# Lab-LVM/imagenet-models

Measured on AMD Instinct MI355X. Metric: images/sec (whole node) GA-ConvNeXt-T 3x224x224 bf16 training step, higher is better.
Workload: dtype bf16; 1 GPU; ga_convnext_tiny_768 train step (fwd + GA loss lam=-0.8 + bwd + all-reduce + adamw lr=0), batch 256/GPU, drop_path 0.2, synthetic 3x224x224; global_batch=256, parallelism=dp1, dist_backend=none, grad_exchange=torch, allreduce_buckets=0

## Files before the change

### imagenet-models_amd/_lib.py

```python
import ctypes as C
import os

_HERE = os.path.dirname(os.path.abspath(__file__))
LIB_PATH = os.environ.get('GAEXT_LIB') or os.path.join(_HERE, 'csrc', 'libgaext.so')

GA_F32, GA_BF16 = 0, 1
ACT_NONE, ACT_GELU, ACT_RELU = 0, 1, 2
A_PLAIN, A_PATCH2, A_STEM4_NCHW, A_CONV3, A_CONV3S2, A_NEIGH2 = 0, 1, 2, 3, 4, 5
C_PLAIN, C_UNPATCH2 = 0, 1

vp, i32, i64, f32 = C.c_void_p, C.c_int, C.c_int64, C.c_float


class GemmDesc(C.Structure):
    _fields_ = [
        ('M', i32), ('N', i32), ('K', i32), ('batch', i32), ('dtype', i32),
        ('A', vp), ('lda', i64), ('strideA', i64), ('a_batch_mod', i32), ('a_kind', i32),
        ('a_H', i32), ('a_W', i32), ('a_C', i32), ('a_act', i32),
        ('B', vp), ('ldb', i64), ('strideB', i64),
        ('C', vp), ('ldc', i64), ('strideC', i64), ('c_kind', i32),
        ('c_H', i32), ('c_W', i32), ('c_C', i32), ('c_f32', i32), ('C2', vp), ('c2_mode', i32),
        ('alpha', f32), ('bias', vp), ('strideBias', i64), ('act', i32),
        ('H', vp), ('ldh', i64), ('strideH', i64), ('h_is_deriv', i32),
        ('rowscale', vp), ('rows_per_scale', i32),
        ('R', vp), ('ldr', i64), ('strideR', i64), ('relu_after', i32),
        ('colsum', vp), ('colsumsq', vp), ('strideCol', i64),
    ]


class WgradDesc(C.Structure):
    _fields_ = [
        ('M', i32), ('N', i32), ('K', i32), ('batch', i32), ('dtype', i32),
        ('Y', vp), ('ldy', i64), ('strideY', i64),
        ('X', vp), ('ldx', i64), ('strideX', i64), ('x_batch_mod', i32), ('x_kind', i32),
        ('x_H', i32), ('x_W', i32), ('x_C', i32), ('x_act', i32),
        ('dW', vp), ('ldw', i64), ('strideW', i64),
        ('dbias', vp), ('strideDbias', i64),
        ('alpha', f32), ('split_m', i32), ('accumulate', i32), ('workspace', vp), ('ws_bytes', i64),
    ]


class WprepDesc(C.Structure):
    _fields_ = [
        ('w', vp), ('G', i32), ('Co', i32), ('Ci', i32), ('KH', i32), ('KW', i32),
        ('rs', vp), ('cs', vp), ('row_perm', vp), ('dtype', i32),
        ('out', vp), ('ldo', i64), ('outT', vp), ('ldt', i64), ('flip', i32), ('stem', i32), ('t_cols', i32),
    ]


class WunfoldDesc(C.Structure):
    _fields_ = [
        ('G', vp), ('ldg', i64), ('gb', vp), ('W', vp), ('b', vp), ('rs', vp), ('cs', vp), ('v', vp), ('row_perm', vp),
        ('N', i32), ('Ci', i32), ('KH', i32), ('KW', i32), ('stem', i32),
        ('dW', vp), ('db', vp), ('d_rs', vp), ('d_cs', vp), ('d_v', vp),
    ]


class SmallDesc(C.Structure):
    _fields_ = [('kind', i32), ('y', vp), ('x', vp), ('a', f32), ('n', i64), ('R', i32), ('C', i32), ('accumulate', i32),
                ('b', vp), ('rs', vp), ('v', vp), ('row_perm', vp)]


class CswinAttnDesc(C.Structure):
    _fields_ = [('B', i32), ('reso', i32), ('C', i32), ('heads', i32), ('nbranch', i32),
                ('Hs', i32 * 2), ('Ws', i32 * 2), ('lepe_w', vp * 2), ('lepe_b', vp * 2),
                ('scale', f32), ('dtype', i32), ('qkv', vp), ('ldq', i64), ('out', vp), ('ldo', i64)]


class MlpDesc(C.Structure):
    _fields_ = [('X', vp), ('ldx', i64), ('W1', vp), ('ldw1', i64), ('b1', vp), ('W2', vp), ('ldw2', i64), ('b2', vp),
                ('R', vp), ('ldr', i64), ('rowscale', vp), ('rows_per_scale', i32), ('Y', vp), ('ldy', i64),
                ('M', i64), ('C', i32), ('H', i32), ('dtype', i32)]


class MlpBwdDesc(C.Structure):
    _fields_ = [('X', vp), ('ldx', i64), ('DY', vp), ('lddy', i64), ('W1', vp), ('ldw1', i64), ('b1', vp),
                ('W2T', vp), ('ldw2t', i64), ('W1T', vp), ('ldw1t', i64), ('A', vp), ('lda', i64), ('DH', vp), ('lddh', i64),
                ('DX', vp), ('lddx', i64), ('M', i64), ('C', i32), ('H', i32), ('dtype', i32),
                ('dW1', vp), ('ldw', i64), ('db1', vp), ('partials', vp), ('partials_bytes', C.c_size_t), ('max_blocks', i32)]


class SmallLinearDesc(C.Structure):
    _fields_ = [('rows', i32), ('groups', i32), ('Ng', i32), ('Kg', i32), ('A', vp), ('lda', i64), ('a_gstride', i64), ('a_perm', vp),
                ('W', vp), ('bias', vp), ('col_scale', vp), ('rowscale', vp), ('rows_per_scale', i32), ('R', vp), ('ldr', i64),
                ('Y', vp), ('ldy', i64), ('Yraw', vp), ('dtype', i32)]


class AttnDesc(C.Structure):
    _fields_ = [('B', i32), ('N', i32), ('H', i32), ('hd', i32), ('scale', f32), ('dtype', i32), ('qkv', vp), ('ldq', i64),
                ('out', vp), ('ldo', i64), ('lse', vp)]


_SIGS = {
    'ga_version': ([], i32),
    'ga_last_error': ([C.c_char_p, C.c_size_t], i32),
    'ga_device_info': ([C.POINTER(i32), C.POINTER(i32), C.POINTER(i32)], i32),
    'ga_comm_unique_id': ([vp], i32),
    'ga_comm_init': ([C.POINTER(vp), i32, i32, vp], i32),
    'ga_comm_destroy': ([vp], i32),
    'ga_comm_info': ([vp, C.POINTER(i32), C.POINTER(i32)], i32),
    'ga_allreduce_workspace': ([i64, i32], C.c_size_t),
    'ga_allreduce_bucket': ([vp, vp, i64, i32, f32, vp, C.c_size_t, vp], i32),
    'ga_reduce_scatter_bucket': ([vp, vp, vp, i64, f32, vp], i32),
    'ga_allgather_bucket': ([vp, vp, vp, i64, vp], i32),
    'ga_comm_broadcast': ([vp, vp, i64, i32, vp], i32),
    'ga_set_knob': ([C.c_char_p, i32], i32),
    'ga_unset_knob': ([C.c_char_p], i32),
    'ga_config_string': ([C.c_char_p, C.c_size_t], i32),
    'ga_gemm': ([C.POINTER(GemmDesc), vp], i32),
    'ga_wgrad': ([C.POINTER(WgradDesc), vp], i32),
    'ga_weight_prep': ([C.POINTER(WprepDesc), vp], i32),
    'ga_bias_fold': ([vp, vp, vp, vp, vp, vp, i32, i32, vp], i32),
    'ga_weight_unfold': ([C.POINTER(WunfoldDesc), vp], i32),
    'ga_dwconv7_fwd': ([vp, vp, vp, vp, i32, i32, i32, i32, i32, vp], i32),
    'ga_dwconv7_bwd_data': ([vp, vp, vp, vp, i32, i32, i32, i32, i32, vp], i32),
    'ga_dwconv7_bwd_data2': ([vp, vp, vp, vp, vp, vp, i32, i32, i32, i32, i32, vp], i32),
    'ga_dwconv7_bwd_weight': ([vp, vp, vp, vp, i32, i32, i32, i32, i32, vp, C.c_size_t, vp], i32),
    'ga_dwconv7_bwd_weight_workspace': ([i32, i32, i32, i32, i32], C.c_size_t),
    'ga_dwconv3_fwd': ([vp, vp, vp, i32, i32, i32, i32, i32, vp, vp, i32, vp], i32),
    'ga_dwconv3_bwd_data': ([vp, vp, vp, i32, i32, i32, i32, i32, i32, vp], i32),
    'ga_dwconv3_bwd_weight': ([vp, vp, vp, i32, i32, i32, i32, i32, i32, vp, C.c_size_t, vp], i32),
    'ga_dwconv3_bwd_weight_workspace': ([i32, i32, i32, i32, i32, i32], C.c_size_t),
    'ga_maxpool3s2_fwd': ([vp, vp, vp, i32, i32, i32, i32, i32, vp], i32),
    'ga_maxpool3s2_bwd': ([vp, vp, vp, i32, i32, i32, i32, i32, i32, vp], i32),
    'ga_bn_gelu_fwd': ([vp, vp, vp, vp, i64, i32, i32, vp], i32),
    'ga_bn_gelu_bwd_workspace': ([i64, i32], C.c_size_t),
    'ga_bn_gelu_bwd_reduce': ([vp, vp, vp, vp, vp, vp, vp, vp, i64, i32, i32, vp, C.c_size_t, vp], i32),
    'ga_bn_gelu_bwd_apply': ([vp, vp, vp, vp, vp, vp, vp, vp, vp, i64, vp, i64, i32, i32, vp], i32),
    'ga_se_bn_fwd': ([vp, i32, vp, vp, vp, vp, vp, vp, vp, vp, vp, vp, vp, vp, vp, vp, i32, i32, i32, i32, vp], i32),
    'ga_se_bn_bwd': ([vp, vp, vp, vp, vp, vp, vp, vp, i32, vp, vp, vp, vp, vp, vp, vp, vp, vp, vp, vp, vp, vp, vp, vp, vp, vp, vp, vp,
                      vp, vp, i32, i32, i32, vp], i32),
    'ga_se_residual_fwd': ([vp, vp, vp, vp, vp, vp, vp, vp, vp, i32, i32, i32, i32, vp], i32),
    'ga_se_residual_bwd_a': ([vp, vp, vp, vp, vp, vp, vp, vp, i32, i32, i32, i32, vp], i32),
    'ga_se_residual_bwd_b': ([vp, vp, vp, vp, vp, vp, vp, vp, vp, vp, vp, i32, i32, i32, i32, vp], i32),
    'ga_subsample2_fwd': ([vp, vp, i32, i32, i32, i32, i32, vp], i32),
    'ga_subsample2_bwd': ([vp, vp, i32, i32, i32, i32, i32, i32, vp], i32),
    'ga_wgrad_workspace': ([C.POINTER(WgradDesc)], C.c_size_t),
    'ga_gemm_form': ([C.POINTER(GemmDesc), C.c_char_p, C.c_size_t], i32),
    'ga_wgrad_form': ([C.POINTER(WgradDesc), C.c_char_p, C.c_size_t], i32),
    'ga_layernorm_fwd': ([vp, vp, vp, vp, vp, vp, i64, i32, f32, i32, vp], i32),
    'ga_layernorm_bwd': ([vp, vp, vp, vp, vp, vp, vp, vp, vp, i64, i32, i32, i32, vp], i32),
    'ga_layernorm_bwd_dp': ([vp, vp, vp, vp, vp, vp, vp, vp, vp, i64, i32, i32, vp, vp, i64, i32, vp], i32),
    'ga_bn_finalize': ([vp, vp, i64, vp, vp, f32, f32, vp, vp, vp, vp, vp, vp, i32, i32, vp], i32),
    'ga_affine_act': ([vp, vp, vp, vp, vp, i64, vp, i64, i32, i32, i32, i64, vp], i32),
    'ga_bn_bwd_reduce': ([vp, vp, vp, vp, vp, vp, i64, vp, vp, i64, i32, i32, i64, vp], i32),
    'ga_bn_bwd_apply': ([vp, vp, vp, vp, vp, vp, vp, vp, vp, i64, i64, vp, i64, i32, i32, i64, i64, vp], i32),
    'ga_pool_concat_fwd': ([vp, vp, i32, i32, i32, i32, i32, i32, i32, i32, i32, i32, vp], i32),
    'ga_pool_concat_bwd': ([vp, vp, vp, i32, i32, i32, i32, i32, i32, i32, i32, i32, i32, vp], i32),
    'ga_spatial_sum': ([vp, vp, vp, i32, i32, i32, f32, i32, vp], i32),
    'ga_se_mlp_fwd': ([vp, vp, vp, vp, vp, vp, vp, i32, i32, i32, vp], i32),
    'ga_se_mlp_bwd': ([vp, vp, vp, vp, vp, vp, vp, f32, vp, vp, vp, vp, i32, i32, i32, vp], i32),
    'ga_chan_scale': ([vp, vp, vp, vp, i32, i32, i32, i32, vp], i32),
    'ga_gram_pack_fwd': ([vp, vp, vp, i32, i32, i32, i32, i32, vp], i32),
    'ga_gram_pack_bwd': ([vp, vp, vp, vp, i32, i32, i32, i32, i32, vp], i32),
    'ga_gram_f64_fwd_workspace': ([i32, i32], C.c_size_t),
    'ga_gram_f64_bwd_workspace': ([i32, i32], C.c_size_t),
    'ga_gram_f64_fwd': ([vp, vp, vp, vp, C.c_size_t, i32, i32, i32, i32, i32, i32, i32, vp], i32),
    'ga_gram_f64_bwd': ([vp, vp, vp, vp, vp, vp, C.c_size_t, i32, i32, i32, i32, i32, i32, i32, vp], i32),
    'ga_token_cat': ([vp, vp, vp, i32, i32, i32, i32, vp], i32),
    'ga_token_split': ([vp, vp, vp, i32, i32, i32, i32, i32, i32, vp], i32),
    'ga_class_attn_fwd': ([vp, vp, vp, vp, i32, i32, i32, i32, f32, i32, vp], i32),
    'ga_class_attn_bwd': ([vp, vp, vp, vp, vp, vp, i32, i32, i32, i32, f32, i32, vp], i32),
    'ga_class_attn_fwd2': ([vp, vp, vp, i64, vp, vp, i32, i32, i32, i32, f32, i32, vp], i32),
    'ga_class_attn_bwd2': ([vp, vp, vp, vp, i64, vp, vp, vp, vp, i32, i32, i32, i32, f32, i32, vp], i32),
    'ga_loss_fwd_bwd': ([vp, vp, vp, vp, i32, i32, i32, f32, i32, f32, f32, i32, vp], i32),
    'ga_heads_topk': ([vp, i32, i32, i32, i32, vp, vp, vp], i32),
    'ga_sgd_step': ([vp, vp, vp, vp, i64, i32, f32, vp], i32),
    'ga_adamw_step': ([vp, vp, vp, vp, vp, i64, f32, vp], i32),
    'ga_weight_prep_batch': ([vp, i32, vp], i32),
    'ga_weight_unfold_batch': ([vp, i32, vp], i32),
    'ga_small_batch': ([vp, i32, vp], i32),
    'ga_cswin_attn_fwd': ([C.POINTER(CswinAttnDesc), vp], i32),
    'ga_cswin_attn_bwd_workspace': ([C.POINTER(CswinAttnDesc)], C.c_size_t),
    'ga_cswin_attn_bwd': ([C.POINTER(CswinAttnDesc), vp, vp, vp, C.c_size_t, vp], i32),
    'ga_cswin_lepe_wgrad_reduce': ([C.POINTER(CswinAttnDesc), vp, vp, vp, vp, vp, vp], i32),
    'ga_cswin_lepe_wgrad': ([C.POINTER(CswinAttnDesc), vp, vp, vp, vp, vp, vp], i32),
    'ga_layernorm_gelu_fwd': ([vp, vp, vp, vp, vp, vp, i64, i32, f32, i32, vp], i32),
    'ga_layernorm_gelu_bwd': ([vp, vp, vp, vp, vp, vp, vp, vp, vp, i64, i32, i32, vp], i32),
    'ga_nchw3_to_nhwc8': ([vp, vp, i32, i32, i32, i32, vp], i32),
    'ga_convw_pack': ([vp, vp, i32, i32, i32, i32, i64, i32, vp], i32),
    'ga_convw_unpack_grad': ([vp, vp, i32, i32, i32, i32, i64, vp], i32),
    'ga_conv3s2_dgrad_prep': ([vp, vp, i32, i32, i64, i32, vp], i32),
    'ga_gram_pack_fwd2': ([vp, vp, vp, i32, i32, i32, i32, i32, i32, vp], i32),
    'ga_gram_pack_bwd2': ([vp, vp, vp, vp, i32, i32, i32, i32, i32, i32, vp], i32),
    'ga_map_tokens_fwd': ([vp, vp, i32, i32, i32, i32, i32, vp], i32),
    'ga_map_tokens_bwd': ([vp, vp, i32, i32, i32, i32, i32, vp], i32),
    'ga_class_attn_mt_fwd': ([vp, vp, vp, i64, vp, vp, vp, i32, i32, i32, i32, i32, f32, i32, vp], i32),
    'ga_class_attn_mt_bwd': ([vp, vp, vp, vp, i64, vp, vp, vp, vp, vp, i64, i32, i32, i32, i32, i32, f32, i32, vp], i32),
    'ga_class_attn_mt_ia_fwd': ([vp, vp, vp, i64, vp, vp, vp, vp, vp, vp, vp, i32, i32, i32, i32, i32, f32, i32, vp], i32),
    'ga_class_attn_mt_ia_bwd': ([vp, vp, vp, vp, i64, vp, vp, vp, vp, vp, vp, vp, vp, i64, vp, vp, vp, vp, i32, i32, i32, i32, i32, f32, i32,
                                 vp], i32),
    'ga_map_loss_fwd_bwd': ([vp, vp, vp, vp, vp, vp, i32, i32, i32, f32, i32, f32, f32, i32, vp], i32),
    'ga_gelu_fwd': ([vp, vp, i64, i32, vp], i32),
    'ga_gelu_bwd': ([vp, vp, vp, i64, i32, vp], i32),
    'ga_relu_drop': ([vp, vp, vp, vp, i64, i32, vp], i32),
    'ga_mask_mul': ([vp, vp, vp, vp, i64, i32, vp], i32),
    'ga_copy2d': ([vp, i64, vp, i64, i64, i32, i32, i32, vp], i32),
    'ga_dropout_mask_sample': ([vp, i64, f32, C.c_uint64, vp, vp], i32),
    'ga_drop_path_sample': ([vp, vp, i32, i32, C.c_uint64, vp, vp], i32),
    'ga_loss_dense_fwd_bwd': ([vp, vp, vp, vp, vp, vp, vp, i32, i32, i32, f32, i32, f32, f32, f32, i32, vp], i32),
    'ga_u8_normalize': ([vp, vp, i32, i32, i32, i32, C.POINTER(f32), C.POINTER(f32), vp], i32),
    'ga_input_erase': ([vp, i32, vp, i32, i32, i32, i32, C.POINTER(f32), C.POINTER(f32), vp, i32, i32, C.c_uint64, C.c_uint64, vp], i32),
    'ga_input_collate': ([vp, i32, vp, i32, i32, i32, i32, C.POINTER(f32), C.POINTER(f32), vp, vp, i32, i32, C.c_uint64, C.c_uint64, vp],
                         i32),
    'ga_mixup_target_elem': ([vp, vp, i32, i32, vp, C.c_double, vp], i32),
    'ga_rand_augment': ([vp, vp, vp, C.c_size_t, i32, i32, i32, i32, vp, i32, vp, vp], i32),
    'ga_rand_augment_work_bytes': ([i32, i32, i32, i32, i32], C.c_size_t),
    'ga_rand_augment_check_table': ([vp, i32], i32),
    'ga_resize_crop': ([vp, C.c_uint64, vp, vp, vp, C.c_size_t, i32, i32, i32, vp], i32),
    'ga_resize_crop_work_bytes': ([vp, i32, i32, i32], C.c_size_t),
    'ga_resize_crop_check_table': ([vp, i32, i32, i32, C.c_uint64], i32),
    'ga_resample_coeffs': ([i32, i32, i32, vp, vp, i32, vp], i32),
    'ga_jpeg_probe': ([vp, C.c_size_t, vp], i32),
    'ga_jpeg_entropy_decode': ([vp, C.c_size_t, vp, C.c_size_t, vp], i32),
    'ga_jpeg_check_table': ([vp, i32, C.c_uint64, C.c_uint64, C.c_uint64, C.c_uint64], i32),
    'ga_jpeg_work_bytes': ([vp, i32], C.c_size_t),
    'ga_jpeg_reconstruct': ([vp, i32, vp, vp, vp, vp, vp], i32),
    'ga_mixup_batch': ([vp, vp, i32, i32, i32, i32, C.c_double, i32, i32, i32, i32, i32, vp], i32),
    'ga_mixup_target': ([vp, vp, i32, i32, C.c_double, C.c_double, vp], i32),
    'ga_agc_clip': ([vp, vp, vp, i32, f32, f32, vp], i32),
    'ga_small_linear_fwd': ([C.POINTER(SmallLinearDesc), vp], i32),
    'ga_small_linear_bwd': ([C.POINTER(SmallLinearDesc), vp, vp, i32, vp, vp, vp, vp], i32),
    'ga_colstats': ([vp, i64, i32, i32, vp, vp, i32, vp], i32),
    'ga_pad_copy_f32': ([vp, vp, i64, i64, i64, i64, i32, vp], i32),
    'ga_pad_copy': ([vp, vp, i64, i64, i64, i64, i32, i32, vp], i32),
    'ga_stem4_ln_fwd': ([vp, vp, i64, vp, vp, vp, vp, vp, vp, vp, i32, i32, i32, i32, f32, vp], i32),
    'ga_blockdiag_f32': ([vp, vp, i64, i32, i32, i32, i64, i32, i32, vp], i32),
    'ga_pad_groups_f32': ([vp, vp, i64, i64, i32, i32, i32, i32, i32, i32, vp], i32),
    'ga_attn_fwd': ([C.POINTER(AttnDesc), vp], i32),
    'ga_attn_bwd_workspace': ([C.POINTER(AttnDesc)], C.c_size_t),
    'ga_attn_bwd': ([C.POINTER(AttnDesc), vp, vp, vp, C.c_size_t, vp], i32),
    'ga_patchify': ([vp, vp, i32, i32, i32, i32, i32, i32, vp], i32),
    'ga_vit_embed_fwd': ([vp, vp, vp, vp, i32, i32, i32, i32, vp], i32),
    'ga_vit_embed_bwd': ([vp, vp, vp, vp, i32, i32, i32, i32, vp], i32),
    'ga_patchify_strided': ([vp, vp, i32, i32, i32, i32, i32, i32, i32, vp], i32),
    'ga_pos_add_fwd': ([vp, vp, vp, i32, i32, i32, i32, vp], i32),
    'ga_pos_add_bwd': ([vp, vp, i32, i32, i32, i32, vp], i32),
    'ga_dwpool_fwd': ([vp, vp, vp, vp, i32, i32, i32, i32, i32, i32, vp], i32),
    'ga_dwpool_bwd_data': ([vp, vp, vp, i32, i32, i32, i32, i32, i32, vp], i32),
    'ga_dwpool_bwd_weight': ([vp, vp, vp, vp, i32, i32, i32, i32, i32, i32, vp], i32),
    'ga_resize_concat_fwd': ([vp, vp, i32, i32, i32, i32, i32, i32, i64, i32, i32, vp], i32),
    'ga_resize_concat_bwd': ([vp, vp, i32, i32, i32, i32, i32, i32, i64, i32, i32, vp], i32),
    'ga_rows_bcast': ([vp, vp, i32, i32, i32, f32, i32, vp], i32),
    'ga_token_gap_fwd': ([vp, vp, i32, i32, i32, i32, vp], i32),
    'ga_token_gap_bwd': ([vp, vp, i32, i32, i32, i32, vp], i32),
    'ga_mlp_supported': ([i32, i32, i32], i32),
    'ga_mlp_fwd': ([C.POINTER(MlpDesc), vp], i32),
    'ga_mlp_bwd': ([C.POINTER(MlpBwdDesc), vp], i32),
    'ga_mlp_bwd_wgrad_supported': ([i32, i32, i32], i32),
    'ga_mlp_bwd_partials': ([C.POINTER(MlpBwdDesc)], C.c_size_t),
    'ga_memset': ([vp, i32, C.c_size_t, vp], i32),
    'ga_transpose_f32': ([vp, vp, i32, i32, i32, vp], i32),
    'ga_axpy_f32': ([vp, vp, f32, i64, vp], i32),
    'ga_lerp_f32': ([vp, vp, f32, i64, vp], i32),
    'ga_sumsq_f32': ([vp, i64, vp, vp], i32),
    'ga_lamb_stage1': ([vp, vp, vp, vp, vp, vp, vp, vp, i32, vp, vp], i32),
    'ga_lamb_stage2': ([vp, vp, vp, vp, i32, vp, vp], i32),
    'ga_clip_grad_f32': ([vp, i64, vp, f32, i32, vp], i32),
    'ga_rowscale': ([vp, vp, vp, i64, i64, i32, vp], i32),
    'ga_cast_from_f32': ([vp, vp, i64, i32, vp], i32),
    'ga_cast_to_f32': ([vp, vp, i64, i32, vp], i32),
}

_lib = None


def load():
    global _lib
    if _lib is not None:
        return _lib
    if not os.path.exists(LIB_PATH):
        raise RuntimeError(f'libgaext.so not found at {LIB_PATH}: build it with `make -C {os.path.dirname(LIB_PATH)}` '
                           f'(there is no CPU fallback for the product path)')
    lib = C.CDLL(LIB_PATH)
    for name, (argtypes, restype) in _SIGS.items():
        fn = getattr(lib, name)
        fn.argtypes = argtypes
        fn.restype = restype
    _lib = lib
    return lib


def last_error():
    buf = C.create_string_buffer(512)
    load().ga_last_error(buf, 512)
    return buf.value.decode(errors='replace')


def config_string():
    buf = C.create_string_buffer(1024)
    load().ga_config_string(buf, 1024)
    s = buf.value.decode(errors='replace')
    host = sorted(k for k in os.environ if k.startswith(('GAEXT_', 'GA_FUSED_MLP')) and k != 'GAEXT_LIB')
    known = {'GAEXT_ASYNC_WGRAD', 'GAEXT_FWD_SPLIT', 'GAEXT_PAR_BRANCH', 'GAEXT_FWD_SKEW', 'GAEXT_FUSE_DP', 'GAEXT_HEAD_STREAMS',
             'GA_FUSED_MLP', 'GAEXT_SMALL_SINGLE', 'GAEXT_SYNC_DEBUG', 'GAEXT_MLP_WG1'}
    for k in host:
        if k in known:
            s += f' host:{k}={os.environ[k]}'
    if os.environ.get('GAEXT_LIB'):
        s += f' lib={os.environ["GAEXT_LIB"]}'
    return s


class knobs:

    def __init__(self, **kv):
        self.kv = kv

    def __enter__(self):
        lib = load()
        for k, v in self.kv.items():
            check(lib.ga_set_knob(k.encode(), int(v)), f'ga_set_knob({k})')
        return self

    def __exit__(self, *exc):
        lib = load()
        for k in self.kv:
            lib.ga_unset_knob(k.encode())
        return False


def check(rc, what):
    if rc != 0:
        raise RuntimeError(f'libgaext {what} failed (code {rc}): {last_error()}')


def exported_symbols():
    return sorted(_SIGS)
```

### imagenet-models_amd/csrc/gemm.hip

```cpp
#include <stdlib.h>
#include <algorithm>
#include <type_traits>
#include "common.h"
#include "gemm_select.h"

namespace {

constexpr int kThreads = 256;
constexpr int kRowBytes = 128;

__device__ __forceinline__ int xcd_remap(int bid, int nwg) {
    const int q = nwg >> 3, r = nwg & 7, xcd = bid & 7, idx = bid >> 3;
    return (xcd < r ? xcd * (q + 1) : r * (q + 1) + (xcd - r) * q) + idx;
}

struct RowCtx {
    long base;
    int y, x;
    bool valid;
};

__device__ __forceinline__ RowCtx make_row(int kind, long m, long M, long ld, int H, int W, int C) {
    RowCtx r;
    r.valid = m < M;
    r.y = r.x = 0;
    r.base = 0;
    if (!r.valid) return r;
    if (kind == GA_A_PLAIN) {
        r.base = m * ld;
    } else if (kind == GA_A_PATCH2) {
        const int OW = W >> 1, OH = H >> 1;
        const int ox = (int)(m % OW);
        const long t = m / OW;
        const int oy = (int)(t % OH);
        const long b = t / OH;
        r.base = ((b * H + 2 * oy) * W + 2 * ox) * (long)C;
    } else if (kind == GA_A_CONV3 || kind == GA_A_NEIGH2) {
        const int x = (int)(m % W);
        const long t = m / W;
        const int y = (int)(t % H);
        const long b = t / H;
        r.base = b * H * W;
        r.y = y;
        r.x = x;
    } else if (kind == GA_A_CONV3S2) {
        const int OW = (W + 1) >> 1, OH = (H + 1) >> 1;
        const int ox = (int)(m % OW);
        const long t = m / OW;
        const int oy = (int)(t % OH);
        const long b = t / OH;
        r.base = b * H * W;
        r.y = 2 * oy;
        r.x = 2 * ox;
    } else {
        const int OW = W >> 2, OH = H >> 2;
        const int ox = (int)(m % OW);
        const long t = m / OW;
        const int oy = (int)(t % OH);
        const long b = t / OH;
        r.base = ((b * C) * H + 4 * oy) * (long)W + 4 * ox;
    }
    return r;
}

struct KCtx {
    long off;
    int dy, dx;
    bool valid;
};

__device__ __forceinline__ KCtx make_k(int kind, int k, int K, int H, int W, int C) {
    KCtx c;
    c.valid = k < K;
    c.off = 0;
    c.dy = c.dx = 0;
    if (!c.valid) return c;
    if (kind == GA_A_PLAIN) {
        c.off = k;
    } else if (kind == GA_A_PATCH2) {
        const int tap = k / C, ch = k - tap * C;
        c.off = ((long)(tap >> 1) * W + (tap & 1)) * C + ch;
    } else if (kind == GA_A_CONV3 || kind == GA_A_CONV3S2) {
        const int tap = k / C, ch = k - tap * C;
        c.dy = tap / 3 - 1;
        c.dx = tap % 3 - 1;
        c.off = ((long)c.dy * W + c.dx) * C + ch;
    } else if (kind == GA_A_NEIGH2) {
        const int tap = k / C, ch = k - tap * C;
        c.dy = tap >> 1;
        c.dx = tap & 1;
        c.off = ((long)c.dy * W + c.dx) * C + ch;
    } else {
        const int ch = k >> 4, ky = (k >> 2) & 3;
        c.off = ((long)ch * H + ky) * W;
    }
    return c;
}

template <typename T>
__device__ __forceinline__ uint4 load_chunk(int kind, const void* base, const RowCtx& r, const KCtx& k, int H, int W,
                                            int C) {
    uint4 z = make_uint4(0, 0, 0, 0);
    if (!(r.valid && k.valid)) return z;
    if (kind == GA_A_CONV3 || kind == GA_A_CONV3S2 || kind == GA_A_NEIGH2) {
        const int yy = r.y + k.dy, xx = r.x + k.dx;
        if ((unsigned)yy >= (unsigned)H || (unsigned)xx >= (unsigned)W) return z;
        const long pix = r.base + (long)r.y * W + r.x;
        return *reinterpret_cast<const uint4*>(reinterpret_cast<const T*>(base) + pix * C + k.off);
    }
    if (kind == GA_A_STEM4_NCHW) {
        const float* p = reinterpret_cast<const float*>(base) + r.base + k.off;
        const float4 a = *reinterpret_cast<const float4*>(p);
        if constexpr (sizeof(T) == 4) {
            return make_uint4(__float_as_uint(a.x), __float_as_uint(a.y), __float_as_uint(a.z), __float_as_uint(a.w));
        } else {
            const float4 b = *reinterpret_cast<const float4*>(p + W);
            return make_uint4(pack2bf(a.x, a.y), pack2bf(a.z, a.w), pack2bf(b.x, b.y), pack2bf(b.z, b.w));
        }
    }
    return *reinterpret_cast<const uint4*>(reinterpret_cast<const T*>(base) + r.base + k.off);
}

template <typename T> __device__ __forceinline__ uint4 act_chunk(uint4 v, int act) {
    if (act == GA_ACT_NONE) return v;
    if constexpr (sizeof(T) == 4) {
        float f[4] = {__uint_as_float(v.x), __uint_as_float(v.y), __uint_as_float(v.z), __uint_as_float(v.w)};
#pragma unroll
        for (int i = 0; i < 4; ++i) f[i] = act == GA_ACT_GELU ? gelu_f(f[i]) : fmaxf(f[i], 0.f);
        return make_uint4(__float_as_uint(f[0]), __float_as_uint(f[1]), __float_as_uint(f[2]), __float_as_uint(f[3]));
    } else {
        unsigned w[4] = {v.x, v.y, v.z, v.w};
#pragma unroll
        for (int i = 0; i < 4; ++i) {
            float lo = __uint_as_float(w[i] << 16), hi = __uint_as_float(w[i] & 0xffff0000u);
            lo = act == GA_ACT_GELU ? gelu_f(lo) : fmaxf(lo, 0.f);
            hi = act == GA_ACT_GELU ? gelu_f(hi) : fmaxf(hi, 0.f);
            w[i] = pack2bf(lo, hi);
        }
        return make_uint4(w[0], w[1], w[2], w[3]);
    }
}

__device__ __forceinline__ void glds16(const void* gsrc, unsigned lds_dst) {
    unsigned keep;
    asm volatile(
        "s_mov_b32 %0, m0\n\ts_mov_b32 m0, %2\n\ts_nop 0\n\tglobal_load_lds_dwordx4 %1, off\n\ts_mov_b32 m0, %0"
        : "=&s"(keep)
        : "v"(gsrc), "s"(lds_dst)
        : "memory");
}

__device__ __forceinline__ void glds16x2(const void* g0, const void* g1, unsigned lds_dst) {
    unsigned keep;
    const char* g1m = static_cast<const char*>(g1) - 1024;
    asm volatile(
        "s_mov_b32 %0, m0\n\ts_mov_b32 m0, %3\n\ts_nop 0\n\tglobal_load_lds_dwordx4 %1, off\n\t"
        "global_load_lds_dwordx4 %2, off offset:1024\n\ts_mov_b32 m0, %0"
        : "=&s"(keep)
        : "v"(g0), "v"(g1m), "s"(lds_dst)
        : "memory");
}

typedef __attribute__((ext_vector_type(4))) unsigned u32x4_s;
__device__ __forceinline__ void blds16x2(u32x4_s rsrc, unsigned voff0, unsigned voff1, unsigned soff, unsigned lds_dst) {
    unsigned keep;
    const unsigned v1m = voff1 - 1024;
    asm volatile(
        "s_mov_b32 %0, m0\n\ts_mov_b32 m0, %4\n\ts_nop 0\n\tbuffer_load_dwordx4 %1, %3, %5 offen lds\n\t"
        "buffer_load_dwordx4 %2, %3, %5 offen offset:1024 lds\n\ts_mov_b32 m0, %0"
        : "=&s"(keep)
        : "v"(voff0), "v"(v1m), "s"(rsrc), "s"(lds_dst), "s"(soff)
        : "memory");
}
__device__ __forceinline__ void blds16(u32x4_s rsrc, unsigned voff, unsigned soff, unsigned lds_dst) {
    unsigned keep;
    asm volatile("s_mov_b32 %0, m0\n\ts_mov_b32 m0, %3\n\ts_nop 0\n\tbuffer_load_dwordx4 %1, %2, %4 offen lds\n\ts_mov_b32 m0, %0"
                 : "=&s"(keep)
                 : "v"(voff), "s"(rsrc), "s"(lds_dst), "s"(soff)
                 : "memory");
}
__device__ __forceinline__ u32x4_s make_rsrc(const void* base, unsigned bytes) {
    const unsigned long long a = reinterpret_cast<unsigned long long>(base);
    u32x4_s r;
    r[0] = __builtin_amdgcn_readfirstlane((unsigned)a);
    r[1] = __builtin_amdgcn_readfirstlane((unsigned)(a >> 32) & 0xffffu);
    r[2] = bytes;
    r[3] = 0x00020000u;
    return r;
}

__device__ __attribute__((aligned(256))) unsigned char g_zero_page[256];

template <int TNW, int NWM> struct NTCfg {
    static constexpr int NTHR = 128 * NWM;
    static constexpr int BM = 64 * NWM;
    static constexpr int BN = 32 * TNW;
    static constexpr int A_BYTES = BM * kRowBytes;
    static constexpr int RSTEP = NTHR / 8;
    static constexpr int NB = BN * 8 / NTHR > 0 ? BN * 8 / NTHR : 1;
    static constexpr int LDCS = BN + 4;
    static constexpr int SMEM_AB = A_BYTES + BN * kRowBytes;
    static constexpr int SMEM_C = 64 * LDCS * 4;
    static constexpr int SMEM = SMEM_AB > SMEM_C ? SMEM_AB : SMEM_C;
    static constexpr int P8 = BN / 8;
    static constexpr int RG = NTHR / P8;
    static constexpr bool DMA3 = TNW == 4 && NWM == 4;
    static constexpr bool SWZ = TNW == 4 || TNW == 8;
    static constexpr int NS = DMA3 ? 3 : 2;
    static constexpr int PR = TNW == 8 ? 16 : (SWZ ? 32 : 64);
    static constexpr int CSUM_BYTES = 2 * RG * BN * 4;
    static constexpr int STAGE_DMA = SWZ ? PR * BN * 4 : (SMEM_C > CSUM_BYTES ? SMEM_C : CSUM_BYTES);
    static constexpr int RING0 = (STAGE_DMA + 1023) & ~1023;
    static constexpr int SMEM_DMA = RING0 + NS * SMEM_AB;
    static constexpr int NW = 2 * NWM;
    static constexpr int NBP = (4 * TNW + NW - 1) / NW;
};

using gasel::EPI_GENERIC, gasel::EPI_PLAIN, gasel::EPI_FC1, gasel::EPI_FC2, gasel::EPI_DG2;

template <typename T, int TNW, int NWM, bool PLAIN, bool PRE, int EPI, bool DMA = false>
__global__ __launch_bounds__(128 * NWM, (NWM == 2 && !DMA && !PRE && EPI >= 0 && sizeof(T) == 2 && TNW == 3) ? 3 : (NWM == 2 && DMA) ? 2 : 1) void gemm_nt_kernel(const ga_gemm_desc d) {
#define F_GELU (EPI < 0 ? d.act == GA_ACT_GELU : EPI == EPI_FC1)
#define F_RELU (EPI < 0 ? d.act == GA_ACT_RELU : false)
#define F_C2 (EPI < 0 ? d.C2 != nullptr : (EPI == EPI_FC1 && d.C2 != nullptr))
#define F_H (EPI < 0 ? Hb != nullptr : EPI == EPI_DG2)
#define F_HDERIV (EPI < 0 ? d.h_is_deriv != 0 : true)
#define F_RS (EPI < 0 ? d.rowscale != nullptr : (EPI == EPI_FC2 && d.rowscale != nullptr))
#define F_R (EPI < 0 ? Rb != nullptr : EPI == EPI_FC2)
#define F_RELUA (EPI < 0 ? d.relu_after != 0 : false)
#define F_CSUM (EPI < 0 ? d.colsum != nullptr : ((EPI == EPI_DG2 || EPI == EPI_PLAIN) && d.colsum != nullptr))
#define F_UNPATCH (EPI < 0 ? d.c_kind == GA_C_UNPATCH2 : false)
#define F_CF32 (EPI < 0 ? d.c_f32 != 0 : false)
#define F_AACT (EPI < 0 ? d.a_act : GA_ACT_NONE)
    using CF = NTCfg<TNW, NWM>;
    constexpr int EPC = elt<T>::EPC;
    constexpr int BK = kRowBytes / (int)sizeof(T);
    constexpr int BN = CF::BN;
    static_assert(!DMA || (PLAIN && sizeof(T) == 2), "the LDS-DMA form needs plain bf16 operands");
    static_assert(DMA || (CF::BN * 8) % CF::NTHR == 0, "B slab must split evenly over the threads");
    extern __shared__ __attribute__((aligned(16))) unsigned char smem[];
    constexpr int RING0 = DMA ? CF::RING0 : 0;
    unsigned char* As = smem + RING0;
    unsigned char* Bs = As + CF::A_BYTES;

    const int tid = threadIdx.x, lane = tid & 63;
    const int wave = DMA ? __builtin_amdgcn_readfirstlane(tid >> 6) : tid >> 6;
    const int wm = wave >> 1, wn = wave & 1;
    const int tiles_n = (d.N + BN - 1) / BN, tiles_m = (d.M + CF::BM - 1) / CF::BM;
    const int nwg = tiles_n * tiles_m;
    const int z = blockIdx.z;
    const int za = d.a_batch_mod > 0 ? z % d.a_batch_mod : z;

    const unsigned char* Ab = reinterpret_cast<const unsigned char*>(d.A) +
                              (d.a_kind == GA_A_STEM4_NCHW ? 4 : (long)sizeof(T)) * za * d.strideA;
    const T* Bb = reinterpret_cast<const T*>(d.B) + z * d.strideB;

    const int kc = tid & 7, r0 = tid >> 3;
    const int nk = (d.K + BK - 1) / BK;
    RowCtx arow[PLAIN ? 1 : 4];
    int m0 = 0, n0 = 0;
    auto set_tile = [&](int vt) {
        const int bid = xcd_remap(vt, nwg);
        const int tile_m = bid / tiles_n, tile_n = bid - tile_m * tiles_n;
        m0 = tile_m * CF::BM;
        n0 = tile_n * BN;
        if constexpr (!PLAIN) {
#pragma unroll
            for (int i = 0; i < 4; ++i)
                arow[i] = make_row(d.a_kind, (long)m0 + r0 + CF::RSTEP * i, d.M, d.lda, d.a_H, d.a_W, d.a_C);
        }
    };

    uint4 ra[4], rb[CF::NB];
    auto g_load = [&](int kt) {
        const int k = kt * BK + kc * EPC;
        const bool kv = k < d.K;
        if constexpr (PLAIN) {
            const T* Ap = reinterpret_cast<const T*>(Ab) + k;
#pragma unroll
            for (int i = 0; i < 4; ++i) {
                const long m = (long)m0 + r0 + CF::RSTEP * i;
                ra[i] = (kv && m < d.M) ? *reinterpret_cast<const uint4*>(Ap + m * d.lda) : make_uint4(0, 0, 0, 0);
            }
        } else {
            const KCtx kx = make_k(d.a_kind, k, d.K, d.a_H, d.a_W, d.a_C);
#pragma unroll
            for (int i = 0; i < 4; ++i) ra[i] = load_chunk<T>(d.a_kind, Ab, arow[i], kx, d.a_H, d.a_W, d.a_C);
        }
#pragma unroll
        for (int i = 0; i < CF::NB; ++i) {
            const long n = (long)n0 + r0 + CF::RSTEP * i;
            rb[i] = (kv && n < d.N) ? *reinterpret_cast<const uint4*>(Bb + n * d.ldb + k) : make_uint4(0, 0, 0, 0);
        }
    };
    auto s_store = [&]() {
#pragma unroll
        for (int i = 0; i < 4; ++i) {
            const int row = r0 + CF::RSTEP * i;
            *reinterpret_cast<uint4*>(As + row * kRowBytes + ((kc ^ (row & 7)) << 4)) = act_chunk<T>(ra[i], F_AACT);
        }
#pragma unroll
        for (int i = 0; i < CF::NB; ++i) {
            const int row = r0 + CF::RSTEP * i;
            *reinterpret_cast<uint4*>(Bs + row * kRowBytes + ((kc ^ (row & 7)) << 4)) = rb[i];
        }
    };

    unsigned aoff[DMA ? 4 : 1], boff[DMA ? CF::NBP : 1];
    constexpr unsigned kOob = 0x80000000u;
    const int dchunk = ((lane & 7) ^ (lane >> 3)) * 8;
    const unsigned lds_ring = (unsigned)(size_t)(__attribute__((address_space(3))) unsigned char*)smem + RING0;
    const u32x4_s rsA = make_rsrc(Ab, kOob), rsB = make_rsrc(Bb, kOob);
    const int ktail = d.K % BK;
    auto dma_rows = [&](int tm0, int tn0) {
        if constexpr (DMA) {
#pragma unroll
            for (int i = 0; i < 4; ++i) {
                const long m = (long)tm0 + (wave * 4 + i) * 8 + (lane >> 3);
                aoff[i] = m < d.M ? (unsigned)(m * d.lda + dchunk) * 2u : kOob;
            }
#pragma unroll
            for (int i = 0; i < CF::NBP; ++i) {
                const long n = (long)tn0 + (i * CF::NW + wave) * 8 + (lane >> 3);
                boff[i] = n < d.N ? (unsigned)(n * d.ldb + dchunk) * 2u : kOob;
            }
        }
    };
    auto dma_issue = [&](int kt, int slot) {
        if constexpr (DMA) {
            const bool kdead = ktail && kt == nk - 1 && dchunk >= ktail;
            const unsigned soff = (unsigned)kt * (unsigned)kRowBytes;
            const unsigned dst = lds_ring + slot * CF::SMEM_AB;
#pragma unroll
            for (int i = 0; i < 4; ++i) blds16(rsA, kdead ? kOob : aoff[i], soff, dst + (wave * 4 + i) * 1024);
#pragma unroll
            for (int i = 0; i < CF::NBP; ++i) {
                const int p = i * CF::NW + wave;
                if (p < 4 * TNW) blds16(rsB, kdead ? kOob : boff[i], soff, dst + CF::A_BYTES + p * 1024);
            }
        }
    };

    const T* Hb = d.H ? reinterpret_cast<const T*>(d.H) + z * d.strideH : nullptr;
    const T* Rb = d.R ? reinterpret_cast<const T*>(d.R) + z * d.strideR : nullptr;
    float* Cs = reinterpret_cast<float*>(smem);
    const int c8 = tid % CF::P8, rg = tid / CF::P8;
    const bool t_active = rg < CF::RG;

    constexpr int NR = (64 + CF::RG - 1) / CF::RG;
    constexpr bool kPre = PRE && sizeof(T) == 2;
    uint4 pre[kPre ? NWM : 1][kPre ? NR : 1];
    const T* Pb = F_H ? Hb : Rb;
    const long ldp = F_H ? d.ldh : d.ldr;

    auto pre_sel = [&](int hf, int it) -> const uint4& { return pre[kPre ? hf : 0][kPre ? it : 0]; };

    int vt = blockIdx.x;
    set_tile(vt);
    int cslot = 0, ivt = blockIdx.x, ikt = 0, islot = 0, inflight = 0;
    auto issue_next = [&]() {
        if constexpr (DMA) {
            if (ivt >= nwg) return;
            if (ikt == 0) {
                const int bid = xcd_remap(ivt, nwg);
                const int tile_m = bid / tiles_n;
                dma_rows(tile_m * CF::BM, (bid - tile_m * tiles_n) * BN);
            }
            dma_issue(ikt, islot);
            islot = islot + 1 == CF::NS ? 0 : islot + 1;
            if (++ikt == nk) {
                ikt = 0;
                ivt += gridDim.x;
            }
            ++inflight;
        }
    };
    if constexpr (DMA) {
#pragma unroll
        for (int j = 0; j < CF::NS - 1; ++j) issue_next();
    } else {
        g_load(0);
    }
    for (; vt < nwg; ) {
    const int cm0 = m0, cn0 = n0;
    const int n = cn0 + c8 * 8;
    const bool n_ok = t_active && n < d.N;
    const bool full = n + 8 <= d.N;
    const bool use_pre = kPre && Pb != nullptr && n_ok && full;
    f32x4_t acc[TNW][4];
#pragma unroll
    for (int i = 0; i < TNW; ++i)
#pragma unroll
        for (int j = 0; j < 4; ++j) acc[i][j] = f32x4_t{0.f, 0.f, 0.f, 0.f};

    if constexpr (!DMA) {
        s_store();
        __syncthreads();
    }

    for (int kt = 0; kt < nk; ++kt) {
        if constexpr (DMA) {
            if (CF::NS == 3 && inflight >= 2) asm volatile("s_waitcnt vmcnt(6)" ::: "memory");
            else asm volatile("s_waitcnt vmcnt(0)" ::: "memory");
            __builtin_amdgcn_s_barrier();
            issue_next();
            --inflight;
            As = smem + RING0 + cslot * CF::SMEM_AB;
            Bs = As + CF::A_BYTES;
            cslot = cslot + 1 == CF::NS ? 0 : cslot + 1;
        } else {
            if (kt + 1 < nk) g_load(kt + 1);
        }
        if constexpr (kPre) {
            if (kt == nk - 1 && use_pre) {
#pragma unroll
                for (int hf = 0; hf < NWM; ++hf)
#pragma unroll
                    for (int it = 0; it < NR; ++it) {
                        const int row = rg + it * CF::RG;
                        const long m = (long)cm0 + hf * 64 + row;
                        if (row < 64 && m < d.M) pre[hf][it] = load16_nt(Pb + m * ldp + n);
                    }
            }
        }
#pragma unroll
        for (int ks = 0; ks < 2; ++ks) {
            const int chunk = ks * 4 + (lane >> 4);
            uint4 af[4];
#pragma unroll
            for (int t = 0; t < 4; ++t) {
                const int ra_ = wm * 64 + t * 16 + (lane & 15);
                af[t] = *reinterpret_cast<const uint4*>(As + ra_ * kRowBytes + ((chunk ^ (ra_ & 7)) << 4));
            }
#pragma unroll
            for (int tn = 0; tn < TNW; ++tn) {
                const int rb_ = wn * (16 * TNW) + tn * 16 + (lane & 15);
                const uint4 bf = *reinterpret_cast<const uint4*>(Bs + rb_ * kRowBytes + ((chunk ^ (rb_ & 7)) << 4));
                if constexpr (sizeof(T) == 2) {
#pragma unroll
                    for (int tm = 0; tm < 4; ++tm)
                        acc[tn][tm] = __builtin_amdgcn_mfma_f32_16x16x32_bf16(
                            *reinterpret_cast<const bf16x8_t*>(&bf), *reinterpret_cast<const bf16x8_t*>(&af[tm]),
                            acc[tn][tm], 0, 0, 0);
                } else {
#pragma unroll
                    for (int j = 0; j < 4; ++j)
#pragma unroll
                        for (int tm = 0; tm < 4; ++tm)
                            acc[tn][tm] = __builtin_amdgcn_mfma_f32_16x16x4f32(
                                reinterpret_cast<const float*>(&bf)[j], reinterpret_cast<const float*>(&af[tm])[j],
                                acc[tn][tm], 0, 0, 0);
                }
            }
        }
        if constexpr (!DMA) {
            __syncthreads();
            if (kt + 1 < nk) {
                s_store();
                __syncthreads();
            }
        }
    }
    vt += gridDim.x;
    if (vt < nwg) {
        set_tile(vt);
        if constexpr (!DMA) g_load(0);
    }

    float bias[8], csum[8], csq[8];
    {
        const float* bsrc = d.bias ? d.bias + (long)z * d.strideBias : reinterpret_cast<const float*>(Bb);
#pragma unroll
        for (int j = 0; j < 8; ++j) {
            const bool live = d.bias && n_ok && n + j < d.N;
            const float bl = bsrc[live ? n + j : 0];
            bias[j] = live ? bl : 0.f;
            csum[j] = csq[j] = 0.f;
        }
    }
    long c_off = 0;
    if (F_UNPATCH && n_ok) {
        const int tap = n / d.c_C, ch = n - tap * d.c_C;
        c_off = ((long)(tap >> 1) * d.c_W + (tap & 1)) * d.c_C + ch;
    }
    constexpr bool SW = DMA && CF::SWZ;
    constexpr int PRr = SW ? CF::PR : 64, NSUB = 64 / PRr, TMP = PRr / 16, NRP = SW ? PRr / CF::RG : NR;
#pragma unroll
    for (int half = 0; half < NWM; ++half) {
#pragma unroll
    for (int sub = 0; sub < NSUB; ++sub) {
        if (half || sub) __syncthreads();
        if (wm == half) {
#pragma unroll
            for (int tn = 0; tn < TNW; ++tn)
#pragma unroll
                for (int tml = 0; tml < TMP; ++tml) {
                    const int row = tml * 16 + (lane & 15), col = wn * (16 * TNW) + tn * 16 + (lane >> 4) * 4;
                    float* dst = SW ? Cs + row * BN + ((((col >> 2) ^ (row & 15))) << 2) : Cs + row * CF::LDCS + col;
                    *reinterpret_cast<f32x4_t*>(dst) = acc[tn][sub * TMP + tml];
                }
        }
        __syncthreads();
        if (n_ok) {
#pragma unroll
            for (int itp = 0; itp < NRP; ++itp) {
                const int it = sub * NRP + itp;
                const int row = rg + itp * CF::RG;
                if (row >= PRr) break;
                const long m = (long)cm0 + half * 64 + sub * PRr + row;
                if (m >= d.M) break;
                float v[8];
                {
                    const float* pa = SW ? Cs + row * BN + (((2 * c8) ^ (row & 15)) << 2) : Cs + row * CF::LDCS + c8 * 8;
                    const float* pb = SW ? Cs + row * BN + (((2 * c8 + 1) ^ (row & 15)) << 2) : Cs + row * CF::LDCS + c8 * 8 + 4;
                    const f32x4_t a = *reinterpret_cast<const f32x4_t*>(pa);
                    const f32x4_t b = *reinterpret_cast<const f32x4_t*>(pb);
                    v[0] = a[0]; v[1] = a[1]; v[2] = a[2]; v[3] = a[3];
                    v[4] = b[0]; v[5] = b[1]; v[6] = b[2]; v[7] = b[3];
                }
#pragma unroll
                for (int j = 0; j < 8; ++j) v[j] = (EPI < 0 ? v[j] * d.alpha : v[j]) + bias[j];
                if (F_C2) {
                    float w[8];
                    if (EPI >= 0 || (d.c2_mode == 2 && d.act == GA_ACT_GELU)) {
#pragma unroll
                        for (int j = 0; j < 8; ++j) {
                            if constexpr (sizeof(T) == 2 && EPI == EPI_FC1) gelu_both_fast(v[j], v[j], w[j]);
                            else gelu_both_f(v[j], v[j], w[j]);
                        }
                    } else {
#pragma unroll
                        for (int j = 0; j < 8; ++j) w[j] = d.c2_mode == 2 ? gelu_grad_f(v[j]) : v[j];
                        if (d.act == GA_ACT_GELU) {
#pragma unroll
                            for (int j = 0; j < 8; ++j) v[j] = gelu_f(v[j]);
                        }
                    }
                    if (F_RELU) {
#pragma unroll
                        for (int j = 0; j < 8; ++j) v[j] = fmaxf(v[j], 0.f);
                    }
                    T* C2p = reinterpret_cast<T*>(d.C2) + z * d.strideC + m * d.ldc + n;
                    if (full) {
                        store8_nt(C2p, w);
                    } else {
#pragma unroll
                        for (int j = 0; j < 8; ++j)
                            if (n + j < d.N) elt<T>::st(C2p + j, w[j]);
                    }
                } else if (F_GELU) {
#pragma unroll
                    for (int j = 0; j < 8; ++j) {
                        if constexpr (sizeof(T) == 2 && EPI == EPI_FC1) {
                            float unused;
                            gelu_both_fast(v[j], v[j], unused);
                        } else {
                            v[j] = gelu_f(v[j]);
                        }
                    }
                } else if (F_RELU) {
#pragma unroll
                    for (int j = 0; j < 8; ++j) v[j] = fmaxf(v[j], 0.f);
                }
                if (F_H) {
                    float h[8];
                    if (use_pre) {
                        if constexpr (kPre) unpack8(pre_sel(half, it), h);
                    } else if (full) {
                        load8_nt(Hb + m * d.ldh + n, h);
                    } else {
#pragma unroll
                        for (int j = 0; j < 8; ++j) h[j] = n + j < d.N ? elt<T>::ld(Hb + m * d.ldh + n + j) : 0.f;
                    }
                    if (F_HDERIV) {
#pragma unroll
                        for (int j = 0; j < 8; ++j) v[j] *= h[j];
                    } else {
#pragma unroll
                        for (int j = 0; j < 8; ++j) v[j] *= gelu_grad_f(h[j]);
                    }
                }
                if (F_RS) {
                    const float s = d.rowscale[(unsigned)m / (unsigned)d.rows_per_scale];
#pragma unroll
                    for (int j = 0; j < 8; ++j) v[j] *= s;
                }
                if (F_R) {
                    float r[8];
                    if (use_pre && !F_H) {
                        if constexpr (kPre) unpack8(pre_sel(half, it), r);
                    } else if (full) {
                        load8_nt(Rb + m * d.ldr + n, r);
                    } else {
#pragma unroll
                        for (int j = 0; j < 8; ++j) r[j] = n + j < d.N ? elt<T>::ld(Rb + m * d.ldr + n + j) : 0.f;
                    }
#pragma unroll
                    for (int j = 0; j < 8; ++j) v[j] += r[j];
                }
                if (F_RELUA) {
#pragma unroll
                    for (int j = 0; j < 8; ++j) v[j] = fmaxf(v[j], 0.f);
                }
                if (F_CSUM) {
#pragma unroll
                    for (int j = 0; j < 8; ++j) {
                        csum[j] += v[j];
                        csq[j] += v[j] * v[j];
                    }
                }
                long off;
                if (F_UNPATCH) {
                    const unsigned OW = d.c_W >> 1, OH = d.c_H >> 1;
                    const unsigned ox = (unsigned)m % OW;
                    const unsigned t = (unsigned)m / OW;
                    const unsigned oy = t % OH;
                    const long b = t / OH;
                    off = ((b * d.c_H + 2 * oy) * d.c_W + 2 * ox) * (long)d.c_C + c_off;
                } else {
                    off = z * d.strideC + m * d.ldc + n;
                }
                if (F_CF32) {
                    float* Cp = reinterpret_cast<float*>(d.C) + off;
                    if (full) {
                        store8(Cp, v);
                    } else {
#pragma unroll
                        for (int j = 0; j < 8; ++j)
                            if (n + j < d.N) Cp[j] = v[j];
                    }
                } else {
                    T* Cp = reinterpret_cast<T*>(d.C) + off;
                    if (full) {
                        store8_nt(Cp, v);
                    } else {
#pragma unroll
                        for (int j = 0; j < 8; ++j)
                            if (n + j < d.N) elt<T>::st(Cp + j, v[j]);
                    }
                }
            }
        }
    }
    }
    if (F_CSUM) {
        float* red = reinterpret_cast<float*>(smem);
        constexpr int NPASS = SW ? 2 : 1;
#pragma unroll
        for (int pass = 0; pass < NPASS; ++pass) {
            if (SW && pass == 1 && !d.colsumsq) break;
            __syncthreads();
            if (t_active) {
#pragma unroll
                for (int j = 0; j < 8; ++j) {
                    if constexpr (SW) {
                        red[rg * BN + c8 * 8 + j] = pass == 0 ? csum[j] : csq[j];
                    } else {
                        red[rg * BN + c8 * 8 + j] = csum[j];
                        red[CF::RG * BN + rg * BN + c8 * 8 + j] = csq[j];
                    }
                }
            }
            __syncthreads();
            for (int i = tid; i < (SW ? BN : 2 * BN); i += CF::NTHR) {
                const int which = SW ? pass : i / BN, col = SW ? i : i - which * BN;
                if (cn0 + col < d.N && (which == 0 || d.colsumsq)) {
                    float s = 0.f;
                    for (int r = 0; r < CF::RG; ++r) s += red[(SW ? 0 : which * CF::RG * BN) + r * BN + col];
                    atomicAdd((which ? d.colsumsq : d.colsum) + z * d.strideCol + cn0 + col, s);
                }
            }
        }
    }
    __syncthreads();
    }
#undef F_GELU
#undef F_RELU
#undef F_C2
#undef F_H
#undef F_HDERIV
#undef F_RS
#undef F_R
#undef F_RELUA
#undef F_CSUM
#undef F_UNPATCH
#undef F_CF32
#undef F_AACT
}

constexpr int kPPThreads = 512, kPPHalf = 16384, kPPBuf = 4 * kPPHalf, kPPSmem = 2 * kPPBuf + 8 * 4096;

template <int EPI>
__global__ __launch_bounds__(kPPThreads) void gemm_nt_pp_kernel(const ga_gemm_desc d, const int dbg_arg) {
#ifdef GAEXT_DEBUG
    const int dbg = dbg_arg;
#else
    constexpr int dbg = 0;
    (void)dbg_arg;
#endif
    extern __shared__ __attribute__((aligned(16))) unsigned char smem[];
    const int tid = threadIdx.x, lane = tid & 63;
    const int wave = __builtin_amdgcn_readfirstlane(tid >> 6);
    const int wr = wave >> 2, wc = wave & 3;
    const int tiles_n = (d.N + 255) / 256, tiles_m = (d.M + 255) / 256;
    const int nwg = tiles_n * tiles_m;
    const int z = blockIdx.z;
    const int za = d.a_batch_mod > 0 ? z % d.a_batch_mod : z;
    const bf16_t* Ab = reinterpret_cast<const bf16_t*>(d.A) + (long)za * d.strideA;
    const bf16_t* Bb = reinterpret_cast<const bf16_t*>(d.B) + (long)z * d.strideB;
    const int nk = (d.K + 63) / 64;
    const int my_tiles = (nwg - (int)blockIdx.x + (int)gridDim.x - 1) / (int)gridDim.x;
    const int S = my_tiles * nk;

    const int fa = (lane & 15) * 128 + ((((lane >> 4) ^ (lane & 7))) << 4);
    const unsigned char* aF[2] = {smem + wr * kPPHalf + fa, smem + wr * kPPHalf + (fa ^ 64)};
    const unsigned char* bF[2] = {smem + (2 + (wc >> 1)) * kPPHalf + (wc & 1) * 8192 + fa,
                                  smem + (2 + (wc >> 1)) * kPPHalf + (wc & 1) * 8192 + (fa ^ 64)};

    const unsigned lds0 = (unsigned)(size_t)(__attribute__((address_space(3))) unsigned char*)smem;
    const int dchunk = ((lane & 7) ^ (lane >> 3)) * 8;
    struct Cursor { int vt, kt; };
    Cursor cm = {(int)blockIdx.x, 0}, cl = {(int)blockIdx.x, 0};
    int off_a0[2], off_b[2][2], off_a1[2];
    auto rows_of = [&](int t, int h, bool is_a, int (&o)[2]) {
        const int bid = xcd_remap(t, nwg);
        const int tm = bid / tiles_n, tn = bid - tm * tiles_n;
#pragma unroll
        for (int i = 0; i < 2; ++i) {
            const int r = h * 128 + 16 * wave + 8 * i + (lane >> 3);
            o[i] = is_a ? min(tm * 256 + r, d.M - 1) * (int)d.lda : min(tn * 256 + r, d.N - 1) * (int)d.ldb;
        }
    };
    auto set_main = [&]() {
        rows_of(cm.vt, 0, false, off_b[0]);
        rows_of(cm.vt, 1, false, off_b[1]);
    };
    auto set_lag = [&]() {
        rows_of(cl.vt, 0, true, off_a0);
        rows_of(cl.vt, 1, true, off_a1);
    };
    const u32x4_s rsA = make_rsrc(Ab, 0x80000000u), rsB = make_rsrc(Bb, 0x80000000u);
    const int ktail = d.K & 63;
    auto glds_half = [&](const bf16_t* base, const int (&o)[2], int kt_, int half, int buf) {
        if (dbg & 2) return;
        const unsigned dst = lds0 + buf * kPPBuf + half * kPPHalf + 2 * wave * 1024;
        if (dbg & 16) {
            const int k = kt_ * 64 + dchunk;
            const bool kv = k < d.K && !(dbg & 8);
            glds16x2(kv ? static_cast<const void*>(base + o[0] + k) : static_cast<const void*>(g_zero_page),
                     kv ? static_cast<const void*>(base + o[1] + k) : static_cast<const void*>(g_zero_page), dst);
            return;
        }
        unsigned v0 = (unsigned)(o[0] + dchunk) * 2u, v1 = (unsigned)(o[1] + dchunk) * 2u;
        if (ktail && kt_ == nk - 1 && dchunk >= ktail) v0 = v1 = 0x80000400u;
        blds16x2(base == Ab ? rsA : rsB, v0, v1, (unsigned)kt_ * 128u, dst);
    };
    auto issue_B0 = [&](int buf) { glds_half(Bb, off_b[0], cm.kt, 2, buf); };
    auto issue_B1 = [&](int buf) {
        glds_half(Bb, off_b[1], cm.kt, 3, buf);
        if (++cm.kt == nk) {
            cm.kt = 0;
            cm.vt += gridDim.x;
            if (cm.vt < nwg) set_main();
        }
    };
    auto issue_A0 = [&](int buf) { glds_half(Ab, off_a0, cl.kt, 0, buf); };
    auto issue_A1 = [&](int buf) {
        glds_half(Ab, off_a1, cl.kt, 1, buf);
        if (++cl.kt == nk) {
            cl.kt = 0;
            cl.vt += gridDim.x;
            if (cl.vt < nwg) set_lag();
        }
    };

    f32x4_t acc[4][8];
    bf16x8_t af[4][2], bc0[2][2], b1[2][2], bn0[2][2];
    const f32x4_t zero4 = {0.f, 0.f, 0.f, 0.f};
#pragma unroll
    for (int i = 0; i < 4; ++i)
#pragma unroll
        for (int j = 0; j < 8; ++j) acc[i][j] = zero4;

#define PP_READ_A(mh, bufp)                                                                                         \
    _Pragma("unroll") for (int tm = 0; tm < 4; ++tm) _Pragma("unroll") for (int ks = 0; ks < 2; ++ks)               \
        af[tm][ks] = *reinterpret_cast<const bf16x8_t*>(aF[ks] + (bufp) + ((mh) * 4 + tm) * 2048);
#define PP_READ_B(dst, nh, bufp)                                                                                    \
    _Pragma("unroll") for (int tn = 0; tn < 2; ++tn) _Pragma("unroll") for (int ks = 0; ks < 2; ++ks)               \
        dst[tn][ks] = *reinterpret_cast<const bf16x8_t*>(bF[ks] + (bufp) + ((nh) * 2 + tn) * 2048);
#define PP_MMA(bq, mh, nh)                                                                                          \
    __builtin_amdgcn_s_setprio(1);                                                                                  \
    _Pragma("unroll") for (int ks = 0; ks < 2; ++ks) _Pragma("unroll") for (int tn = 0; tn < 2; ++tn)               \
        _Pragma("unroll") for (int tm = 0; tm < 4; ++tm)                                                            \
            acc[(nh) * 2 + tn][(mh) * 4 + tm] = __builtin_amdgcn_mfma_f32_16x16x32_bf16(bq[tn][ks], af[tm][ks],     \
                                                                                      acc[(nh) * 2 + tn][(mh) * 4 + tm], 0, 0, 0); \
    __builtin_amdgcn_s_setprio(0);
#define PP_MMA_RELOAD(bq, mh, nh, mh2, bufp)                                                                        \
    __builtin_amdgcn_s_setprio(1);                                                                                  \
    _Pragma("unroll") for (int tm = 0; tm < 4; ++tm) {                                                              \
        _Pragma("unroll") for (int ks = 0; ks < 2; ++ks) _Pragma("unroll") for (int tn = 0; tn < 2; ++tn)           \
            acc[(nh) * 2 + tn][(mh) * 4 + tm] = __builtin_amdgcn_mfma_f32_16x16x32_bf16(bq[tn][ks], af[tm][ks],     \
                                                                                      acc[(nh) * 2 + tn][(mh) * 4 + tm], 0, 0, 0); \
        __builtin_amdgcn_sched_barrier(0);                                                                          \
        _Pragma("unroll") for (int ks = 0; ks < 2; ++ks)                                                            \
            af[tm][ks] = *reinterpret_cast<const bf16x8_t*>(aF[ks] + (bufp) + ((mh2) * 4 + tm) * 2048);             \
        __builtin_amdgcn_sched_barrier(0);                                                                          \
    }                                                                                                               \
    __builtin_amdgcn_s_setprio(0);
#define PP_LGKM0 asm volatile("s_waitcnt lgkmcnt(0)" ::: "memory")
#define PP_BAR                            \
    __builtin_amdgcn_sched_barrier(0);    \
    __builtin_amdgcn_s_barrier();         \
    __builtin_amdgcn_sched_barrier(0)

    set_main();
    set_lag();
    issue_B0(0);
    issue_B1(0);
    issue_A0(0);
    issue_A1(0);
    if (S > 1) {
        issue_B0(1);
        issue_B1(1);
        asm volatile("s_waitcnt vmcnt(4)" ::: "memory");
    } else {
        asm volatile("s_waitcnt vmcnt(0)" ::: "memory");
    }
    PP_BAR;
    PP_READ_B(bn0, 0, 0);
    PP_LGKM0;

    const bf16_t* Hb = d.H ? reinterpret_cast<const bf16_t*>(d.H) + (long)z * d.strideH : nullptr;
    const bf16_t* Rb = d.R ? reinterpret_cast<const bf16_t*>(d.R) + (long)z * d.strideR : nullptr;
    float* stage = reinterpret_cast<float*>(smem + 2 * kPPBuf + wave * 4096);
    int vt = blockIdx.x, kt = 0;
#pragma unroll 1
    for (int g = 0; g < S; ++g) {
        const int bufp = (g & 1) * kPPBuf, nbufp = kPPBuf - bufp;
        const bool more1 = g + 1 < S, more2 = g + 2 < S;
        if (kt == 0 && wr == 1) { PP_BAR; }
#pragma unroll
        for (int i = 0; i < 2; ++i)
#pragma unroll
            for (int j = 0; j < 2; ++j) bc0[i][j] = bn0[i][j];
        PP_READ_A(0, bufp);
        if (more1) issue_A0((g + 1) & 1);
        PP_LGKM0;
        PP_BAR;
        PP_READ_B(b1, 1, bufp);
        PP_MMA(bc0, 0, 0);
        PP_BAR;
        if (more1) {
            issue_A1((g + 1) & 1);
            if (!(dbg & 4)) asm volatile("s_waitcnt vmcnt(4)" ::: "memory");
        }
        PP_LGKM0;
        PP_BAR;
        PP_MMA_RELOAD(b1, 0, 1, 1, bufp);
        PP_BAR;
        if (more2) issue_B0(g & 1);
        PP_LGKM0;
        PP_BAR;
        if (more1) { PP_READ_B(bn0, 0, nbufp); }
        PP_MMA(b1, 1, 1);
        PP_BAR;
        if (more2) issue_B1(g & 1);
        if (more1 && !(dbg & 4)) {
            if (more2) asm volatile("s_waitcnt vmcnt(4)" ::: "memory");
            else asm volatile("s_waitcnt vmcnt(0)" ::: "memory");
        }
        PP_LGKM0;
        PP_BAR;
        PP_MMA(bc0, 1, 0);
        PP_BAR;
        if (++kt < nk) continue;
        kt = 0;
        if (wr == 0) { PP_BAR; }
        if (dbg & 1) {
            vt += gridDim.x;
            continue;
        }
        {
            const int bid = xcd_remap(vt, nwg);
            const int tile_m = bid / tiles_n, tile_n = bid - tile_m * tiles_n;
            const int q = lane & 7, rr = lane >> 3;
            const int n = tile_n * 256 + wc * 64 + q * 8;
            const bool n_ok = n < d.N;
            float bias[8], csum[8], csq[8];
            {
                const bool live = d.bias && n_ok;
                const float* bsrc = d.bias ? d.bias + (long)z * d.strideBias : reinterpret_cast<const float*>(Bb);
#pragma unroll
                for (int j = 0; j < 8; ++j) {
                    const float bl = bsrc[live ? n + j : 0];
                    bias[j] = live ? bl : 0.f;
                    csum[j] = csq[j] = 0.f;
                }
            }
            const bool do_csum = (EPI == EPI_PLAIN || EPI == EPI_DG2) && d.colsum != nullptr;
            constexpr bool kOp = EPI == EPI_DG2 || EPI == EPI_FC2;
            const bf16_t* Pb = EPI == EPI_DG2 ? Hb : Rb;
            const long ldp = EPI == EPI_DG2 ? d.ldh : d.ldr;
            const long mrow0 = (long)tile_m * 256 + wr * 128 + rr;
            uint4 opn[2] = {make_uint4(0, 0, 0, 0), make_uint4(0, 0, 0, 0)};
            auto fetch_op = [&](int tm) {
                if constexpr (kOp) {
#pragma unroll
                    for (int p = 0; p < 2; ++p) {
                        const long m = mrow0 + tm * 16 + 8 * p;
                        if (n_ok && m < d.M) opn[p] = load16_nt(Pb + m * ldp + n);
                    }
                }
            };
            fetch_op(0);
#pragma unroll
            for (int tm = 0; tm < 8; ++tm) {
                asm volatile("s_waitcnt lgkmcnt(0)" ::: "memory");
#pragma unroll
                for (int tn = 0; tn < 4; ++tn) {
                    const int row = lane & 15, u = tn * 4 + (lane >> 4);
                    *reinterpret_cast<f32x4_t*>(stage + row * 64 + ((u ^ row) << 2)) = acc[tn][tm];
                    acc[tn][tm] = zero4;
                }
                const uint4 opc[2] = {opn[0], opn[1]};
                if (tm + 1 < 8) fetch_op(tm + 1);
                asm volatile("s_waitcnt lgkmcnt(0)" ::: "memory");
#pragma unroll
                for (int p = 0; p < 2; ++p) {
                    const int row = 8 * p + rr;
                    const long m = (long)tile_m * 256 + wr * 128 + tm * 16 + row;
                    const f32x4_t lo = *reinterpret_cast<const f32x4_t*>(stage + row * 64 + (((2 * q) ^ row) << 2));
                    const f32x4_t hi = *reinterpret_cast<const f32x4_t*>(stage + row * 64 + (((2 * q + 1) ^ row) << 2));
                    if (!n_ok || m >= d.M) continue;
                    float v[8] = {lo[0] + bias[0], lo[1] + bias[1], lo[2] + bias[2], lo[3] + bias[3],
                                  hi[0] + bias[4], hi[1] + bias[5], hi[2] + bias[6], hi[3] + bias[7]};
                    if constexpr (EPI == EPI_FC1) {
                        float w[8];
#pragma unroll
                        for (int j = 0; j < 8; ++j) gelu_both_fast(v[j], v[j], w[j]);
                        if (d.C2) store8_nt(reinterpret_cast<bf16_t*>(d.C2) + (long)z * d.strideC + m * d.ldc + n, w);
                    }
                    if constexpr (EPI == EPI_DG2) {
                        float h[8];
                        unpack8(opc[p], h);
#pragma unroll
                        for (int j = 0; j < 8; ++j) v[j] *= h[j];
                    }
                    if constexpr (EPI == EPI_FC2) {
                        if (d.rowscale) {
                            const float sc = d.rowscale[(unsigned)m / (unsigned)d.rows_per_scale];
#pragma unroll
                            for (int j = 0; j < 8; ++j) v[j] *= sc;
                        }
                        float r[8];
                        unpack8(opc[p], r);
#pragma unroll
                        for (int j = 0; j < 8; ++j) v[j] += r[j];
                    }
                    if (do_csum) {
#pragma unroll
                        for (int j = 0; j < 8; ++j) {
                            csum[j] += v[j];
                            csq[j] += v[j] * v[j];
                        }
                    }
                    store8_nt(reinterpret_cast<bf16_t*>(d.C) + (long)z * d.strideC + m * d.ldc + n, v);
                }
            }
            if (do_csum) {
#pragma unroll
                for (int j = 0; j < 8; ++j) {
                    float a = csum[j], b = csq[j];
#pragma unroll
                    for (int o = 8; o < 64; o <<= 1) {
                        a += __shfl_xor(a, o, 64);
                        b += __shfl_xor(b, o, 64);
                    }
                    if (rr == 0 && n_ok) {
                        atomicAdd(d.colsum + (long)z * d.strideCol + n + j, a);
                        if (d.colsumsq) atomicAdd(d.colsumsq + (long)z * d.strideCol + n + j, b);
                    }
                }
            }
        }
        vt += gridDim.x;
    }
#undef PP_READ_A
#undef PP_READ_B
#undef PP_MMA
#undef PP_MMA_RELOAD
#undef PP_LGKM0
#undef PP_BAR
}

constexpr int kR3Threads = 256, kR3Slot = (256 + 128) * 64, kR3Stage = 2048, kR3Smem = 3 * kR3Slot + 4 * kR3Stage;
static_assert(kR3Smem == 81920, "two workgroups per CU need exactly 80 KiB each");

__device__ __forceinline__ u32x4_t r3_bload16(u32x4_s rs, unsigned voff) {
    u32x4_t v;
    asm volatile("buffer_load_dwordx4 %0, %1, %2, 0 offen nt" : "=v"(v) : "v"(voff), "s"(rs) : "memory");
    return v;
}
__device__ __forceinline__ u32x4_t r3_bload16_c(u32x4_s rs, unsigned voff) {
    u32x4_t v;
    asm volatile("buffer_load_dwordx4 %0, %1, %2, 0 offen" : "=v"(v) : "v"(voff), "s"(rs) : "memory");
    return v;
}

__device__ __forceinline__ float r3_bload4(u32x4_s rs, unsigned voff) {
    float v;
    asm volatile("buffer_load_dword %0, %1, %2, 0 offen" : "=v"(v) : "v"(voff), "s"(rs) : "memory");
    return v;
}
__device__ __forceinline__ void r3_bstore16(u32x4_s rs, unsigned voff, u32x4_t v) {
    asm volatile("buffer_store_dwordx4 %0, %1, %2, 0 offen nt\n\ts_nop 1" ::"v"(v), "v"(voff), "s"(rs) : "memory");
}
__device__ __forceinline__ u32x4_t r3_pack8(const float v[8]) {
    u32x4_t a;
    a[0] = pack2bf(v[0], v[1]); a[1] = pack2bf(v[2], v[3]); a[2] = pack2bf(v[4], v[5]); a[3] = pack2bf(v[6], v[7]);
    return a;
}

__device__ int g_r3_ticket[4096];

template <int EPI, int DBG = 0, int AK = 0>
__global__ __launch_bounds__(kR3Threads, 2) void gemm_nt_r3_kernel(const ga_gemm_desc d, const int stagger) {
    constexpr int dbg = DBG;
    extern __shared__ __attribute__((aligned(16))) unsigned char smem[];
    const int tid = threadIdx.x, lane = tid & 63;
    const int wave = __builtin_amdgcn_readfirstlane(tid >> 6);
    const int wm = wave >> 1, wn = wave & 1;
    const int tiles_n = (d.N + 127) / 128, tiles_m = (d.M + 255) / 256;
    const int nwg = tiles_n * tiles_m;
    const int z = blockIdx.z;
    const int za = d.a_batch_mod > 0 ? z % d.a_batch_mod : z;
    const bf16_t* Ab = reinterpret_cast<const bf16_t*>(d.A) + (long)za * d.strideA;
    const bf16_t* Bb = reinterpret_cast<const bf16_t*>(d.B) + (long)z * d.strideB;
    const int nk = (d.K + 31) / 32;
    const int my_tiles = (nwg - (int)blockIdx.x + (int)gridDim.x - 1) / (int)gridDim.x;
    const int S = my_tiles * nk;

    const int frow = lane & 15;
    const unsigned fa = frow * 64 + ((((lane >> 4) ^ ((4 - (frow >> 2)) & 3))) << 4);
    const unsigned char* aF = smem + wm * 8192 + fa;
    const unsigned char* bF = smem + 16384 + wn * 4096 + fa;

    const unsigned lds0 = (unsigned)(size_t)(__attribute__((address_space(3))) unsigned char*)smem;
    const int dchunk = ((lane & 3) ^ ((4 - (lane >> 4)) & 3)) * 8;
    constexpr unsigned kOob = 0x80000000u;
    auto extent = [](long rows, long ld, long cols, int esz) { return (unsigned)(((rows - 1) * ld + cols) * esz); };
    const bool patch2 = d.a_kind == GA_A_PATCH2;
    const bool neigh2 = AK == 1 && EPI == EPI_PLAIN && d.a_kind == GA_A_NEIGH2;
    const bool conv3s2 = AK == 1 && EPI == EPI_PLAIN && d.a_kind == GA_A_CONV3S2;
    const unsigned p2_row = (patch2 || neigh2) ? (unsigned)(d.a_W * d.a_C - 2 * d.a_C) * 2u : 0u;
    const unsigned c3_row = conv3s2 ? (unsigned)((d.a_W - 3) * d.a_C) * 2u : 0u;
    const unsigned c3_shift = conv3s2 ? (unsigned)((d.a_W + 1) * d.a_C) * 2u : 0u;
    const unsigned a_bytes = (patch2 || conv3s2) ? extent(4L * d.M, d.a_C, d.a_C, 2) : neigh2 ? extent(d.M, d.a_C, d.a_C, 2) : extent(d.M, d.lda, d.K, 2);
    const u32x4_s rsA = make_rsrc(reinterpret_cast<const unsigned char*>(Ab) - c3_shift, a_bytes + c3_shift),
                  rsB = make_rsrc(Bb, extent(d.N, d.ldb, d.K, 2));
    unsigned n2_have = 0;
    const int ktail = d.K & 31;
    unsigned aoff[4], boff[2];
    int ivt = blockIdx.x, ikt = 0;
    auto dma_rows = [&]() __attribute__((always_inline)) {
        if (ivt < nwg) {
            const int bid = xcd_remap(ivt, nwg);
            const int tm_ = bid / tiles_n, tn_ = bid - tm_ * tiles_n;
#pragma unroll
            for (int i = 0; i < 4; ++i) {
                const long m = (long)tm_ * 256 + (wave * 4 + i) * 16 + (lane >> 2);
                if (patch2) {
                    const unsigned OW = (unsigned)d.a_W >> 1, OH = (unsigned)d.a_H >> 1;
                    const unsigned ox = (unsigned)m % OW, t = (unsigned)m / OW, oy = t % OH, b = t / OH;
                    aoff[i] = m < d.M ? (unsigned)((((long)b * d.a_H + 2 * oy) * d.a_W + 2 * ox) * d.a_C + dchunk) * 2u : kOob;
                } else if (conv3s2) {
                    const unsigned OW = (unsigned)d.a_W >> 1, OH = (unsigned)d.a_H >> 1;
                    const unsigned ox = (unsigned)m % OW, t = (unsigned)m / OW, oy = t % OH, b = t / OH;
                    aoff[i] = m < d.M ? (unsigned)((((long)b * d.a_H + 2 * oy) * d.a_W + 2 * ox) * d.a_C + dchunk) * 2u : kOob;
                    const unsigned have = (ox > 0 ? 1u : 0u) | (oy > 0 ? 2u : 0u);
                    n2_have = (n2_have & ~(3u << (2 * i))) | (have << (2 * i));
                } else if (neigh2) {
                    const unsigned x = (unsigned)m % (unsigned)d.a_W, y = ((unsigned)m / (unsigned)d.a_W) % (unsigned)d.a_H;
                    aoff[i] = m < d.M ? (unsigned)(m * d.a_C + dchunk) * 2u : kOob;
                    const unsigned have = (x + 1 < (unsigned)d.a_W ? 1u : 0u) | (y + 1 < (unsigned)d.a_H ? 2u : 0u);
                    n2_have = (n2_have & ~(3u << (2 * i))) | (have << (2 * i));
                } else {
                    aoff[i] = m < d.M ? (unsigned)(m * d.lda + dchunk) * 2u : kOob;
                }
            }
#pragma unroll
            for (int i = 0; i < 2; ++i) {
                const long n = (long)tn_ * 128 + (wave * 2 + i) * 16 + (lane >> 2);
                boff[i] = n < d.N ? (unsigned)(n * d.ldb + dchunk) * 2u : kOob;
            }
        } else {
#pragma unroll
            for (int i = 0; i < 4; ++i) aoff[i] = kOob;
            boff[0] = boff[1] = kOob;
        }
    };
    auto dma_part = [&](int slot, int part) __attribute__((always_inline)) {
        const bool kdead = ktail && ikt == nk - 1 && dchunk >= ktail;
        const unsigned soff = (unsigned)ikt * 64u;
        unsigned soffA = soff + (2 * ikt >= nk ? p2_row : 0u);
        const unsigned dst = lds0 + slot * kR3Slot;
        unsigned a0 = aoff[part == 0 ? 0 : 2], a1 = aoff[part == 0 ? 1 : 3];
        if (conv3s2 && part < 2) {
            const int third = nk / 3, spt = nk / 9;
            const int ky = (ikt >= third ? 1 : 0) + (ikt >= 2 * third ? 1 : 0);
            const int r = ikt - ky * third;
            const unsigned need = (r < spt ? 1u : 0u) | (ky == 0 ? 2u : 0u);
            soffA = soff + (unsigned)ky * c3_row;
            if ((need & ~(n2_have >> (4 * part))) & 3u) a0 = kOob;
            if ((need & ~(n2_have >> (4 * part + 2))) & 3u) a1 = kOob;
        }
        if (neigh2 && part < 2) {
            const unsigned need = ((4 * ikt >= nk && 4 * ikt < 2 * nk) || 4 * ikt >= 3 * nk ? 1u : 0u) | (2 * ikt >= nk ? 2u : 0u);
            const unsigned miss = need & ~(n2_have >> (4 * part));
            if (miss & 3u) a0 = kOob;
            if ((need & ~(n2_have >> (4 * part + 2))) & 3u) a1 = kOob;
        }
        if (part == 0) blds16x2(rsA, kdead ? kOob : a0, kdead ? kOob : a1, soffA, dst + (wave * 4) * 1024);
        if (part == 1) blds16x2(rsA, kdead ? kOob : a0, kdead ? kOob : a1, soffA, dst + (wave * 4 + 2) * 1024);
        if (part == 2) {
            blds16x2(rsB, kdead ? kOob : boff[0], kdead ? kOob : boff[1], soff, dst + 16384 + (wave * 2) * 1024);
            if (++ikt == nk) {
                ikt = 0;
                ivt += gridDim.x;
                dma_rows();
            }
        }
    };
    auto dma_issue = [&](int slot) __attribute__((always_inline)) {
        dma_part(slot, 0);
        dma_part(slot, 1);
        dma_part(slot, 2);
    };

    f32x4_t acc[4][8];
    const f32x4_t zero4 = {0.f, 0.f, 0.f, 0.f};
#pragma unroll
    for (int i = 0; i < 4; ++i)
#pragma unroll
        for (int j = 0; j < 8; ++j) acc[i][j] = zero4;

    constexpr bool kOp = EPI == EPI_DG2 || EPI == EPI_FC2;
    const bf16_t* Pb = EPI == EPI_DG2 ? (d.H ? reinterpret_cast<const bf16_t*>(d.H) + (long)z * d.strideH : nullptr)
                                      : (d.R ? reinterpret_cast<const bf16_t*>(d.R) + (long)z * d.strideR : nullptr);
    const long ldp = EPI == EPI_DG2 ? d.ldh : d.ldr;
    const u32x4_s rsP = make_rsrc(Pb, (kOp && Pb && !(dbg & 8)) ? extent(d.M, ldp, d.N, 2) : 0u);
    const u32x4_s rsBias = make_rsrc(d.bias ? d.bias + (long)z * d.strideBias : nullptr, d.bias ? (unsigned)d.N * 4u : 0u);
    u32x4_t opn[kOp ? 4 : 1][2], biasv[2];
    float rsc[EPI == EPI_FC2 ? 4 : 1][2];
    const u32x4_s rsRS = make_rsrc(EPI == EPI_FC2 ? d.rowscale : nullptr,
                                   (EPI == EPI_FC2 && d.rowscale) ? (unsigned)(((d.M - 1) / d.rows_per_scale + 1) * 4) : 0u);
    auto rs_off = [&](long m) -> unsigned { return m < d.M ? ((unsigned)m / (unsigned)d.rows_per_scale) * 4u : kOob; };
    const int q = lane & 7, rr = lane >> 3;
    float* stage = reinterpret_cast<float*>(smem + 3 * kR3Slot + wave * kR3Stage);

    int vt = blockIdx.x, kt = 0, cslot = 0;
    int tile_m = 0, tile_n = 0;
    bool first = true;
    dma_rows();
    dma_issue(0);
    dma_issue(1);
    if (stagger > 0) {
        const unsigned hw = __builtin_amdgcn_s_getreg((31 << 11) | 4);
        const unsigned xcc = __builtin_amdgcn_s_getreg((31 << 11) | 20);
        const unsigned key = ((xcc & 15u) << 8) | ((hw >> 8) & 255u);
        int ticket = 0;
        if (tid == 0) ticket = atomicAdd(&g_r3_ticket[key], 1);
        ticket = __builtin_amdgcn_readfirstlane(ticket);
        if (wave == 0 && (ticket & 1)) {
            for (int i = 0; i < stagger; ++i) __builtin_amdgcn_s_sleep(1);
        }
    }
#pragma unroll 1
    for (int g = 0; g < S; ++g) {
        if (kt == 0) {
            const int bid = xcd_remap(vt, nwg);
            tile_m = bid / tiles_n;
            tile_n = bid - tile_m * tiles_n;
        }
        if ((first || kt >= 2) && !(dbg & 32)) asm volatile("s_waitcnt vmcnt(6)" ::: "memory");
        __builtin_amdgcn_s_barrier();
        const int n = tile_n * 128 + wn * 64 + q * 8;
        const bool n_ok = n < d.N;
        const long mrow0 = (long)tile_m * 256 + wm * 128 + rr;
        if (kt == nk - 1) {
            biasv[0] = r3_bload16_c(rsBias, n_ok ? (unsigned)n * 4u : kOob);
            biasv[1] = r3_bload16_c(rsBias, n_ok ? (unsigned)n * 4u + 16u : kOob);
            if constexpr (kOp) {
#pragma unroll
                for (int tm = 0; tm < 4; ++tm)
#pragma unroll
                    for (int p = 0; p < 2; ++p) {
                        const long m = mrow0 + tm * 16 + 8 * p;
                        opn[tm][p] = r3_bload16(rsP, (n_ok && m < d.M) ? (unsigned)(m * ldp + n) * 2u : kOob);
                        if constexpr (EPI == EPI_FC2) rsc[tm][p] = r3_bload4(rsRS, rs_off(m));
                    }
            }
        }
        const int islot = cslot >= 1 ? cslot - 1 : 2;
        {
            const unsigned sb = cslot * kR3Slot;
            bf16x8_t af[8], bfr[4];
#define R3_RA(i) af[i] = *reinterpret_cast<const bf16x8_t*>(aF + sb + (i) * 1024)
#define R3_MMA(i)                                                                                               \
    _Pragma("unroll") for (int tn = 0; tn < 4; ++tn)                                                             \
        acc[tn][i] = __builtin_amdgcn_mfma_f32_16x16x32_bf16(bfr[tn], af[i], acc[tn][i], 0, 0, 0)
#pragma unroll
            for (int tn = 0; tn < 4; ++tn) bfr[tn] = *reinterpret_cast<const bf16x8_t*>(bF + sb + tn * 1024);
            R3_RA(0); R3_RA(1); R3_RA(2); R3_RA(3);
            __builtin_amdgcn_sched_barrier(0);
            if (!(dbg & 16)) dma_part(islot, 0);
            R3_MMA(0); R3_MMA(1);
            __builtin_amdgcn_sched_barrier(0);
            R3_RA(4); R3_RA(5);
            if (!(dbg & 16)) dma_part(islot, 1);
            __builtin_amdgcn_sched_barrier(0);
            R3_MMA(2); R3_MMA(3);
            __builtin_amdgcn_sched_barrier(0);
            R3_RA(6); R3_RA(7);
            if (!(dbg & 16)) dma_part(islot, 2);
            __builtin_amdgcn_sched_barrier(0);
            R3_MMA(4); R3_MMA(5); R3_MMA(6); R3_MMA(7);
#undef R3_RA
#undef R3_MMA
        }
        cslot = cslot == 2 ? 0 : cslot + 1;
        if (++kt < nk) continue;
        kt = 0;
        first = false;
        if (dbg & 1) {
#pragma unroll
            for (int i = 0; i < 4; ++i)
#pragma unroll
                for (int j = 0; j < 8; ++j) asm volatile("" : "+v"(acc[i][j]));
            if constexpr (kOp)
                asm volatile("s_waitcnt vmcnt(0)"
                             : "+v"(opn[0][0]), "+v"(opn[0][1]), "+v"(opn[1][0]), "+v"(opn[1][1]), "+v"(opn[2][0]), "+v"(opn[2][1]),
                               "+v"(opn[3][0]), "+v"(opn[3][1]), "+v"(biasv[0]), "+v"(biasv[1]), "+v"(rsc[0][0]), "+v"(rsc[0][EPI == EPI_FC2]),
                               "+v"(rsc[EPI == EPI_FC2][0]), "+v"(rsc[EPI == EPI_FC2][EPI == EPI_FC2]), "+v"(rsc[2 * (EPI == EPI_FC2)][0]),
                               "+v"(rsc[2 * (EPI == EPI_FC2)][EPI == EPI_FC2]), "+v"(rsc[3 * (EPI == EPI_FC2)][0]), "+v"(rsc[3 * (EPI == EPI_FC2)][EPI == EPI_FC2])
                             :: "memory");
            else
                asm volatile("s_waitcnt vmcnt(0)" : "+v"(biasv[0]), "+v"(biasv[1])::"memory");
            vt += gridDim.x;
            continue;
        }
        if constexpr (kOp) {
            asm volatile("s_waitcnt vmcnt(0)"
                         : "+v"(opn[0][0]), "+v"(opn[0][1]), "+v"(opn[1][0]), "+v"(opn[1][1]), "+v"(opn[2][0]), "+v"(opn[2][1]),
                           "+v"(opn[3][0]), "+v"(opn[3][1]), "+v"(biasv[0]), "+v"(biasv[1])
                         :: "memory");
            if constexpr (EPI == EPI_FC2) {
#pragma unroll
                for (int tm = 0; tm < 4; ++tm) asm volatile("" : "+v"(rsc[tm][0]), "+v"(rsc[tm][1]));
            }
        } else {
            asm volatile("s_waitcnt vmcnt(0)" : "+v"(biasv[0]), "+v"(biasv[1]) :: "memory");
        }
        {
            float bias[8], csum[8], csq[8];
#pragma unroll
            for (int j = 0; j < 4; ++j) {
                bias[j] = __uint_as_float(biasv[0][j]);
                bias[4 + j] = __uint_as_float(biasv[1][j]);
            }
#pragma unroll
            for (int j = 0; j < 8; ++j) csum[j] = csq[j] = 0.f;
            const bool do_csum = (EPI == EPI_PLAIN || EPI == EPI_DG2) && d.colsum != nullptr;
            const bool unpatch2 = EPI == EPI_PLAIN && d.c_kind == GA_C_UNPATCH2;
            const u32x4_s rsC = make_rsrc(reinterpret_cast<bf16_t*>(d.C) + (long)z * d.strideC,
                                          unpatch2 ? extent(4L * d.M, d.c_C, d.c_C, 2) : extent(d.M, d.ldc, d.N, 2));
            unsigned up_col = 0;
            if (unpatch2 && n_ok) {
                const int tap = n / d.c_C, ch = n - tap * d.c_C;
                up_col = (unsigned)(((tap >> 1) * d.c_W + (tap & 1)) * d.c_C + ch);
            }
            const u32x4_s rsC2 = make_rsrc((EPI == EPI_FC1 && d.C2) ? reinterpret_cast<bf16_t*>(d.C2) + (long)z * d.strideC : nullptr,
                                           (EPI == EPI_FC1 && d.C2) ? extent(d.M, d.ldc, d.N, 2) : 0u);
#pragma unroll
            for (int tm = 0; tm < 8; ++tm) {
                if constexpr (kOp) {
                    if (tm >= 4) {
                        constexpr int L = EPI == EPI_FC2 ? 4 : 2;
                        constexpr int ST = (dbg & 2) ? 0 : 2;
                        constexpr int kYoung[4] = {3 * ST + 3 * L, 3 * ST + 2 * L, 3 * ST + L, 3 * ST};
                        constexpr int R = EPI == EPI_FC2 ? 1 : 0;
                        if (tm == 4) asm volatile("s_waitcnt vmcnt(%4)" : "+v"(opn[0][0]), "+v"(opn[0][1]), "+v"(rsc[0][0]), "+v"(rsc[0][R]) : "n"(kYoung[0]) : "memory");
                        if (tm == 5) asm volatile("s_waitcnt vmcnt(%4)" : "+v"(opn[1][0]), "+v"(opn[1][1]), "+v"(rsc[R][0]), "+v"(rsc[R][R]) : "n"(kYoung[1]) : "memory");
                        if (tm == 6) asm volatile("s_waitcnt vmcnt(%4)" : "+v"(opn[2][0]), "+v"(opn[2][1]), "+v"(rsc[2 * R][0]), "+v"(rsc[2 * R][R]) : "n"(kYoung[2]) : "memory");
                        if (tm == 7) asm volatile("s_waitcnt vmcnt(%4)" : "+v"(opn[3][0]), "+v"(opn[3][1]), "+v"(rsc[3 * R][0]), "+v"(rsc[3 * R][R]) : "n"(kYoung[3]) : "memory");
                    }
                }
#pragma unroll
                for (int p = 0; p < 2; ++p) {
                    if (((lane >> 3) & 1) == p) {
                        const int row = lane & 7;
#pragma unroll
                        for (int tn = 0; tn < 4; ++tn) {
                            const int u = tn * 4 + (lane >> 4);
                            *reinterpret_cast<f32x4_t*>(stage + row * 64 + ((u ^ row) << 2)) = acc[tn][tm];
                        }
                    }
                    const f32x4_t lo = *reinterpret_cast<const f32x4_t*>(stage + rr * 64 + (((2 * q) ^ rr) << 2));
                    const f32x4_t hi = *reinterpret_cast<const f32x4_t*>(stage + rr * 64 + (((2 * q + 1) ^ rr) << 2));
                    const long m = mrow0 + tm * 16 + 8 * p;
                    float v[8] = {lo[0] + bias[0], lo[1] + bias[1], lo[2] + bias[2], lo[3] + bias[3],
                                  hi[0] + bias[4], hi[1] + bias[5], hi[2] + bias[6], hi[3] + bias[7]};
                    const bool live = n_ok && m < d.M;
                    unsigned coff = live ? (unsigned)(m * d.ldc + n) * 2u : kOob;
                    if (unpatch2 && live) {
                        const unsigned OW = (unsigned)d.c_W >> 1, OH = (unsigned)d.c_H >> 1;
                        const unsigned ox = (unsigned)m % OW, t = (unsigned)m / OW, oy = t % OH, b = t / OH;
                        coff = (unsigned)((((long)b * d.c_H + 2 * oy) * d.c_W + 2 * ox) * d.c_C + up_col) * 2u;
                    }
                    if constexpr (EPI == EPI_FC1) {
                        float w[8];
#pragma unroll
                        for (int j = 0; j < 8; ++j) {
                            if (dbg & 4) w[j] = v[j] * 0.5f;
                            else gelu_both_fast(v[j], v[j], w[j]);
                        }
                        if (!(dbg & 2)) r3_bstore16(rsC2, coff, r3_pack8(w));
                        else asm volatile("" ::"v"(w[0]), "v"(w[1]), "v"(w[2]), "v"(w[3]), "v"(w[4]), "v"(w[5]), "v"(w[6]), "v"(w[7]));
                    }
                    if constexpr (EPI == EPI_DG2) {
                        float h[8];
                        unpack8(make_uint4(opn[tm & 3][p][0], opn[tm & 3][p][1], opn[tm & 3][p][2], opn[tm & 3][p][3]), h);
#pragma unroll
                        for (int j = 0; j < 8; ++j) v[j] *= h[j];
                    }
                    if constexpr (EPI == EPI_FC2) {
                        if (d.rowscale) {
                            const float sc = rsc[tm & 3][p];
#pragma unroll
                            for (int j = 0; j < 8; ++j) v[j] *= sc;
                        }
                        float r[8];
                        unpack8(make_uint4(opn[tm & 3][p][0], opn[tm & 3][p][1], opn[tm & 3][p][2], opn[tm & 3][p][3]), r);
#pragma unroll
                        for (int j = 0; j < 8; ++j) v[j] += r[j];
                    }
                    if (do_csum && live) {
#pragma unroll
                        for (int j = 0; j < 8; ++j) {
                            csum[j] += v[j];
                            csq[j] += v[j] * v[j];
                        }
                    }
                    if (!(dbg & 2)) r3_bstore16(rsC, coff, r3_pack8(v));
                    else asm volatile("" ::"v"(v[0]), "v"(v[1]), "v"(v[2]), "v"(v[3]), "v"(v[4]), "v"(v[5]), "v"(v[6]), "v"(v[7]));
                }
                if constexpr (kOp) {
                    if (tm < 4) {
#pragma unroll
                        for (int p = 0; p < 2; ++p) {
                            const long m = mrow0 + (tm + 4) * 16 + 8 * p;
                            opn[tm][p] = r3_bload16(rsP, (n_ok && m < d.M) ? (unsigned)(m * ldp + n) * 2u : kOob);
                            if constexpr (EPI == EPI_FC2) rsc[tm][p] = r3_bload4(rsRS, rs_off(m));
                        }
                    }
                }
#pragma unroll
                for (int tn = 0; tn < 4; ++tn) acc[tn][tm] = zero4;
            }
            if (do_csum) {
#pragma unroll
                for (int j = 0; j < 8; ++j) {
#pragma unroll
                    for (int o = 8; o < 64; o <<= 1) {
                        csum[j] += __shfl_xor(csum[j], o, 64);
                        csq[j] += __shfl_xor(csq[j], o, 64);
                    }
                }
                if (rr == 0) {
#pragma unroll
                    for (int j = 0; j < 8; ++j) {
                        stage[q * 8 + j] = csum[j];
                        stage[64 + q * 8 + j] = csq[j];
                    }
                }
                const float a = stage[lane], b = stage[64 + lane];
                const int nc = tile_n * 128 + wn * 64 + lane;
                if (nc < d.N) {
                    atomicAdd(d.colsum + (long)z * d.strideCol + nc, a);
                    if (d.colsumsq) atomicAdd(d.colsumsq + (long)z * d.strideCol + nc, b);
                }
            }
        }
        vt += gridDim.x;
    }
    asm volatile("s_waitcnt vmcnt(0)" ::: "memory");
}

template <typename T> struct TN {
    static constexpr int EPC = elt<T>::EPC;
    static constexpr int RB = 128 * (int)sizeof(T);
    static constexpr int ROWS = 16384 / RB;
    static constexpr int CPR = RB / 16;
    static constexpr int RSTEP = kThreads / CPR;
};

__device__ __forceinline__ int tn_swz(int row) { return ((row & 3) << 1) | (((row >> 3) & 1) << 3); }

template <typename T>
__global__ __launch_bounds__(kThreads, 2) void gemm_tn_kernel(const ga_wgrad_desc d) {
    using P = TN<T>;
    constexpr int EPC = P::EPC;
    extern __shared__ __attribute__((aligned(16))) unsigned char smem[];
    const int tid = threadIdx.x, lane = tid & 63, wave = tid >> 6;
    const int wn = wave >> 1, wk = wave & 1;
    const int tiles_k = (d.K + 127) / 128, tiles_n = (d.N + 127) / 128;
    const int ntiles = tiles_k * tiles_n;
    const int bid = xcd_remap(blockIdx.x, ntiles * d.split_m);
    const int split = bid / ntiles, tile = bid - split * ntiles;
    const int tile_n = tile / tiles_k, tile_k = tile - tile_n * tiles_k;
    const int n0 = tile_n * 128, k0 = tile_k * 128;
    const int z = blockIdx.z;
    const long slabs = (d.M + P::ROWS - 1) / P::ROWS;
    const long per = (slabs + d.split_m - 1) / d.split_m;
    const long s_begin = (long)split * per;
    const long s_end = s_begin + per < slabs ? s_begin + per : slabs;
    if (s_begin >= s_end) return;

    const T* Yb = reinterpret_cast<const T*>(d.Y) + z * d.strideY;
    const int zx = d.x_batch_mod > 0 ? z % d.x_batch_mod : z;
    const unsigned char* Xb = reinterpret_cast<const unsigned char*>(d.X) +
                              (d.x_kind == GA_A_STEM4_NCHW ? 4 : (long)sizeof(T)) * zx * d.strideX;

    const int cc = tid % P::CPR, rr = tid / P::CPR;
    const int ny = n0 + cc * EPC;
    const bool yv = ny < d.N;
    const KCtx kx = make_k(d.x_kind, k0 + cc * EPC, d.K, d.x_H, d.x_W, d.x_C);

    uint4 ry[4], rx[4];
    float bsum[8];
#pragma unroll
    for (int j = 0; j < 8; ++j) bsum[j] = 0.f;
    const bool do_bias = d.dbias != nullptr && tile_k == 0;

    auto g_load = [&](long slab) {
#pragma unroll
        for (int i = 0; i < 4; ++i) {
            const long m = slab * P::ROWS + rr + P::RSTEP * i;
            ry[i] = (yv && m < d.M) ? *reinterpret_cast<const uint4*>(Yb + m * d.ldy + ny) : make_uint4(0, 0, 0, 0);
            const RowCtx r = make_row(d.x_kind, m, d.M, d.ldx, d.x_H, d.x_W, d.x_C);
            rx[i] = load_chunk<T>(d.x_kind, Xb, r, kx, d.x_H, d.x_W, d.x_C);
        }
    };
    auto s_store = [&](int buf) {
        unsigned char* Ys = smem + buf * 32768;
        unsigned char* Xs = Ys + 16384;
#pragma unroll
        for (int i = 0; i < 4; ++i) {
            const int row = rr + P::RSTEP * i;
            const int off = sizeof(T) == 2 ? row * P::RB + ((cc ^ tn_swz(row)) << 4) : row * P::RB + (cc << 4);
            *reinterpret_cast<uint4*>(Ys + off) = ry[i];
            *reinterpret_cast<uint4*>(Xs + off) = act_chunk<T>(rx[i], d.x_act);
            if (do_bias) {
                if constexpr (sizeof(T) == 2) {
                    const unsigned w[4] = {ry[i].x, ry[i].y, ry[i].z, ry[i].w};
#pragma unroll
                    for (int j = 0; j < 4; ++j) {
                        bsum[2 * j] += __uint_as_float(w[j] << 16);
                        bsum[2 * j + 1] += __uint_as_float(w[j] & 0xffff0000u);
                    }
                } else {
                    bsum[0] += __uint_as_float(ry[i].x); bsum[1] += __uint_as_float(ry[i].y);
                    bsum[2] += __uint_as_float(ry[i].z); bsum[3] += __uint_as_float(ry[i].w);
                }
            }
        }
    };

    f32x4_t acc[4][4];
#pragma unroll
    for (int i = 0; i < 4; ++i)
#pragma unroll
        for (int j = 0; j < 4; ++j) acc[i][j] = f32x4_t{0.f, 0.f, 0.f, 0.f};

    g_load(s_begin);
    s_store(0);
    __syncthreads();
    for (long s = s_begin; s < s_end; ++s) {
        const int cur = (int)((s - s_begin) & 1);
        if (s + 1 < s_end) g_load(s + 1);
        const unsigned char* Ys = smem + cur * 32768;
        const unsigned char* Xs = Ys + 16384;
        if constexpr (sizeof(T) == 2) {
#pragma unroll
            for (int ks = 0; ks < 2; ++ks) {
                s16x4_t yf[4][2], xf[4][2];
#pragma unroll
                for (int hf = 0; hf < 2; ++hf) {
                    const int row = ks * 32 + 8 * (lane >> 4) + 4 * hf + ((lane & 15) >> 2);
                    const int sw = tn_swz(row);
#pragma unroll
                    for (int t = 0; t < 4; ++t) {
                        const int ch_y = ((wn * 64 + t * 16) >> 3) + ((lane & 3) >> 1);
                        const int ch_x = ((wk * 64 + t * 16) >> 3) + ((lane & 3) >> 1);
                        const unsigned ay = row * P::RB + ((ch_y ^ sw) << 4) + 8 * (lane & 1);
                        const unsigned ax = row * P::RB + ((ch_x ^ sw) << 4) + 8 * (lane & 1);
                        yf[t][hf] = __builtin_amdgcn_ds_read_tr16_b64_v4i16(
                            (__attribute__((address_space(3))) s16x4_t*)(Ys + ay));
                        xf[t][hf] = __builtin_amdgcn_ds_read_tr16_b64_v4i16(
                            (__attribute__((address_space(3))) s16x4_t*)(Xs + ax));
                    }
                }
#pragma unroll
                for (int tn = 0; tn < 4; ++tn)
#pragma unroll
                    for (int tk = 0; tk < 4; ++tk)
                        acc[tn][tk] = __builtin_amdgcn_mfma_f32_16x16x32_bf16(
                            *reinterpret_cast<const bf16x8_t*>(&yf[tn][0]), *reinterpret_cast<const bf16x8_t*>(&xf[tk][0]),
                            acc[tn][tk], 0, 0, 0);
            }
        } else {
#pragma unroll
            for (int ks = 0; ks < 8; ++ks) {
                const int row = ks * 4 + (lane >> 4);
                float yf[4], xf[4];
#pragma unroll
                for (int t = 0; t < 4; ++t) {
                    yf[t] = *reinterpret_cast<const float*>(Ys + row * P::RB + (wn * 64 + t * 16 + (lane & 15)) * 4);
                    xf[t] = *reinterpret_cast<const float*>(Xs + row * P::RB + (wk * 64 + t * 16 + (lane & 15)) * 4);
                }
#pragma unroll
                for (int tn = 0; tn < 4; ++tn)
#pragma unroll
                    for (int tk = 0; tk < 4; ++tk)
                        acc[tn][tk] = __builtin_amdgcn_mfma_f32_16x16x4f32(yf[tn], xf[tk], acc[tn][tk], 0, 0, 0);
            }
        }
        if (s + 1 < s_end) s_store(cur ^ 1);
        __syncthreads();
    }

    float* W = d.dW + z * d.strideW;
    const bool atomic = d.accumulate || d.split_m > 1;
#pragma unroll
    for (int tn = 0; tn < 4; ++tn)
#pragma unroll
        for (int tk = 0; tk < 4; ++tk)
#pragma unroll
            for (int r = 0; r < 4; ++r) {
                const int n = n0 + wn * 64 + tn * 16 + (lane >> 4) * 4 + r;
                const int k = k0 + wk * 64 + tk * 16 + (lane & 15);
                if (n < d.N && k < d.K) {
                    const float v = acc[tn][tk][r] * d.alpha;
                    if (atomic) atomicAdd(W + (long)n * d.ldw + k, v);
                    else W[(long)n * d.ldw + k] = v;
                }
            }
    if (do_bias) {
        float* red = reinterpret_cast<float*>(smem);
#pragma unroll
        for (int j = 0; j < EPC; ++j) red[rr * 128 + cc * EPC + j] = bsum[j];
        __syncthreads();
        if (tid < 128 && n0 + tid < d.N) {
            float s = 0.f;
            for (int r = 0; r < P::RSTEP; ++r) s += red[r * 128 + tid];
            atomicAdd(d.dbias + z * d.strideDbias + n0 + tid, s * d.alpha);
        }
    }
}

constexpr int kTn2Threads = 512, kTn2Stage = 32768, kTn2Smem = 4 * kTn2Stage;

template <bool P2>
__global__ __launch_bounds__(kTn2Threads) void gemm_tn2_kernel(const ga_wgrad_desc d, const int split_m,
                                                               float* __restrict__ part) {
    extern __shared__ __attribute__((aligned(16))) unsigned char smem[];
    const int tid = threadIdx.x, lane = tid & 63;
    const int wave = __builtin_amdgcn_readfirstlane(tid >> 6);
    const int wn = wave >> 2, wk = wave & 3;
    const int tiles_k = (d.K + 255) / 256, tiles_n = (d.N + 255) / 256;
    const int ntiles = tiles_k * tiles_n;
    const int bid = xcd_remap(blockIdx.x, ntiles * split_m);
    const int split = bid / ntiles, tile = bid - split * ntiles;
    const int tile_n = tile / tiles_k, tile_k = tile - tile_n * tiles_k;
    const int n0 = tile_n * 256, k0 = tile_k * 256;
    const int z = blockIdx.z;
    const int stages = d.M / 32;
    const int per = (stages + split_m - 1) / split_m;
    const int s_begin = split * per;
    const int s_end = s_begin + per < stages ? s_begin + per : stages;
    if (s_begin >= s_end) return;

    const int sub = wave >> 1;
    const bool is_y = sub < 2;
    const int ncols = is_y ? d.N : d.K;
    const int col0 = (is_y ? n0 : k0) + (sub & 1) * 128;
    const bool sub_live = col0 < ncols;
    const long ld = is_y ? d.ldy : d.ldx;
    const int zx = d.x_batch_mod > 0 ? z % d.x_batch_mod : z;
    const bf16_t* gsrc = is_y ? reinterpret_cast<const bf16_t*>(d.Y) + z * d.strideY
                              : reinterpret_cast<const bf16_t*>(d.X) + zx * d.strideX;
    const int lrow = 16 * (wave & 1) + (lane >> 4);
    const int pc = lane & 15;
    const bool xp2 = P2 && !is_y;
    const int sw_lo = ((lane >> 4) & 3) << 1;
    long goff[2];
#pragma unroll
    for (int b = 0; b < 2; ++b) {
        int c = col0 + ((pc ^ (sw_lo | (b << 3))) << 3);
        if (c >= ncols) c = 0;
        if (xp2) goff[b] = c + (c >= 2 * d.x_C ? (long)(d.x_W - 2) * d.x_C : 0);
        else goff[b] = (long)lrow * ld + c;
    }
    const unsigned lds0 = (unsigned)(size_t)(__attribute__((address_space(3))) unsigned char*)smem;
    const u32x4_s rs = make_rsrc(gsrc, xp2 ? (unsigned)(8L * d.M * d.x_C) : 0xffffffffu);
    unsigned voff[4];
    [[maybe_unused]] unsigned p2_ox[4];
    [[maybe_unused]] unsigned p2_ow = 1, p2_r = 0, p2_step = 0, p2_carry = 0;
    if (xp2) {
        p2_ow = (unsigned)d.x_W >> 1;
        const unsigned q = 32u / p2_ow, rowb = (unsigned)(d.x_W * d.x_C) * 2u;
        p2_r = 32u - q * p2_ow;
        p2_step = 128u * (unsigned)d.x_C + q * rowb;
        p2_carry = rowb;
#pragma unroll
        for (int i = 0; i < 4; ++i) {
            const unsigned m = (unsigned)s_begin * 32u + (unsigned)(lrow + 4 * i), t = m / p2_ow;
            p2_ox[i] = m - t * p2_ow;
            voff[i] = (unsigned)(((long)(2u * m + (unsigned)d.x_W * t)) * d.x_C + goff[(i >> 1) & 1]) * 2u;
        }
    } else {
#pragma unroll
        for (int i = 0; i < 4; ++i) voff[i] = (unsigned)(goff[(i >> 1) & 1] + (long)(4 * i) * ld) * 2u;
    }
    auto stage_load = [&](int s, int buf) __attribute__((always_inline)) {
        if (!sub_live) return;
        const unsigned soff = xp2 ? 0u : (unsigned)s * 64u * (unsigned)ld;
        const unsigned dst = lds0 + buf * kTn2Stage + sub * 8192 + (wave & 1) * 4096;
#pragma unroll
        for (int i = 0; i < 4; ++i) blds16(rs, voff[i], soff, dst + i * 1024);
        if constexpr (P2) {
            if (xp2) {
#pragma unroll
                for (int i = 0; i < 4; ++i) {
                    p2_ox[i] += p2_r;
                    const bool carry = p2_ox[i] >= p2_ow;
                    p2_ox[i] -= carry ? p2_ow : 0u;
                    voff[i] += p2_step + (carry ? p2_carry : 0u);
                }
            }
        }
    };

    int nv = (d.N - n0 - wn * 128 + 15) / 16; nv = nv < 0 ? 0 : (nv > 8 ? 8 : nv);
    int kv = (d.K - k0 - wk * 64 + 15) / 16;  kv = kv < 0 ? 0 : (kv > 4 ? 4 : kv);
    const bool do_bias = d.dbias != nullptr && tile_k == 0 && wk == 0;
    f32x4_t acc[8][4];
    float bsum[8];
#pragma unroll
    for (int i = 0; i < 8; ++i) {
        bsum[i] = 0.f;
#pragma unroll
        for (int j = 0; j < 4; ++j) acc[i][j] = f32x4_t{0.f, 0.f, 0.f, 0.f};
    }
    typedef __attribute__((ext_vector_type(2))) __bf16 bf16x2_t;
    const bf16x2_t ones2 = {(__bf16)1.0f, (__bf16)1.0f};

    const unsigned y_img = wn * 8192, x_img = 16384 + (wk >> 1) * 8192;
    const int xc0 = (wk & 1) * 8;
    unsigned yaddr[8], xaddr[4];
    {
        const int row = 8 * (lane >> 4) + ((lane & 15) >> 2);
        const int sw = tn_swz(row);
        const unsigned rb = row * 256 + 8 * (lane & 1);
#pragma unroll
        for (int t = 0; t < 8; ++t) yaddr[t] = y_img + rb + (((2 * t + ((lane & 3) >> 1)) ^ sw) << 4);
#pragma unroll
        for (int t = 0; t < 4; ++t) xaddr[t] = x_img + rb + (((xc0 + 2 * t + ((lane & 3) >> 1)) ^ sw) << 4);
    }
    auto compute = [&](int cur) {
        const unsigned char* st = smem + cur * kTn2Stage;
        s16x4_t yf[8][2], xf[4][2];
#pragma unroll
        for (int hf = 0; hf < 2; ++hf) {
#pragma unroll
            for (int t = 0; t < 4; ++t)
                xf[t][hf] = __builtin_amdgcn_ds_read_tr16_b64_v4i16(
                    (__attribute__((address_space(3))) s16x4_t*)(st + xaddr[t] + hf * 1024));
#pragma unroll
            for (int t = 0; t < 8; ++t)
                yf[t][hf] = __builtin_amdgcn_ds_read_tr16_b64_v4i16(
                    (__attribute__((address_space(3))) s16x4_t*)(st + yaddr[t] + hf * 1024));
        }
#pragma unroll
        for (int tn = 0; tn < 8; ++tn) {
            const bf16x8_t a = *reinterpret_cast<const bf16x8_t*>(&yf[tn][0]);
#pragma unroll
            for (int tk = 0; tk < 4; ++tk)
                acc[tn][tk] = __builtin_amdgcn_mfma_f32_16x16x32_bf16(
                    a, *reinterpret_cast<const bf16x8_t*>(&xf[tk][0]), acc[tn][tk], 0, 0, 0);
        }
        if (do_bias) {
#pragma unroll
            for (int tn = 0; tn < 8; ++tn) {
                const bf16x8_t a = *reinterpret_cast<const bf16x8_t*>(&yf[tn][0]);
#pragma unroll
                for (int j = 0; j < 4; ++j)
                    bsum[tn] = __builtin_amdgcn_fdot2_f32_bf16(bf16x2_t{a[2 * j], a[2 * j + 1]}, ones2, bsum[tn], false);
            }
        }
    };

    const int nst = s_end - s_begin;
#pragma unroll
    for (int j = 0; j < 3; ++j)
        if (j < nst) stage_load(s_begin + j, j);
    for (int it = 0; it < nst; ++it) {
        const int ahead = nst - 1 - it;
        if (ahead >= 2) asm volatile("s_waitcnt vmcnt(8)" ::: "memory");
        else if (ahead == 1) asm volatile("s_waitcnt vmcnt(4)" ::: "memory");
        else asm volatile("s_waitcnt vmcnt(0)" ::: "memory");
        __builtin_amdgcn_s_barrier();
        if (it + 3 < nst) stage_load(s_begin + it + 3, (it + 3) & 3);
        if (nv > 0 && kv > 0) compute(it & 3);
    }

    float* W = part ? part + ((long)z * split_m + split) * d.N * d.K : d.dW + z * d.strideW;
    const long ldw = part ? d.K : d.ldw;
    const float alpha = part ? 1.f : d.alpha;
    const bool atomic = !part && (d.accumulate || split_m > 1);
#pragma unroll
    for (int tn = 0; tn < 8; ++tn)
#pragma unroll
        for (int tk = 0; tk < 4; ++tk)
#pragma unroll
            for (int r = 0; r < 4; ++r) {
                const int n = n0 + wn * 128 + tn * 16 + (lane >> 4) * 4 + r;
                const int k = k0 + wk * 64 + tk * 16 + (lane & 15);
                if (n < d.N && k < d.K) {
                    const float v = acc[tn][tk][r] * alpha;
                    if (atomic) atomicAdd(W + (long)n * ldw + k, v);
                    else W[(long)n * ldw + k] = v;
                }
            }
    if (do_bias) {
#pragma unroll
        for (int tn = 0; tn < 8; ++tn) {
            float v = bsum[tn];
            v += __shfl_xor(v, 16, 64);
            v += __shfl_xor(v, 32, 64);
            const int n = n0 + wn * 128 + tn * 16 + lane;
            if (lane < 16 && n < d.N) atomicAdd(d.dbias + z * d.strideDbias + n, v * d.alpha);
        }
    }
}

__global__ __launch_bounds__(256) void tn2_reduce_kernel(const float* __restrict__ part, int nsplit, long nk, int K,
                                                         float alpha, float* __restrict__ dW, long ldw, long strideW) {
    const long z = blockIdx.y;
    const float* p = part + z * nsplit * nk;
    for (long i = ((long)blockIdx.x * 256 + threadIdx.x) * 4; i < nk; i += (long)gridDim.x * 1024) {
        float4 a = *reinterpret_cast<const float4*>(p + i);
#pragma unroll 4
        for (int s = 1; s < nsplit; ++s) {
            const float4 b = *reinterpret_cast<const float4*>(p + (long)s * nk + i);
            a.x += b.x; a.y += b.y; a.z += b.z; a.w += b.w;
        }
        const long n = i / K, k = i - n * K;
        float* dst = dW + z * strideW + n * ldw + k;
        dst[0] += alpha * a.x; dst[1] += alpha * a.y; dst[2] += alpha * a.z; dst[3] += alpha * a.w;
    }
}

using namespace gasel;

Knobs current_knobs() {
    Knobs k;
#define GA_SEL_KNOB(NAME) k.NAME = GA_KNOB(#NAME, Knobs{}.NAME)
    GA_SEL_KNOB(NT_R3); GA_SEL_KNOB(NT_R3_NEIGH2); GA_SEL_KNOB(NT_R3_CONV3S2); GA_SEL_KNOB(NT_PP); GA_SEL_KNOB(NT_PP_MINK);
    GA_SEL_KNOB(NT_BIG); GA_SEL_KNOB(NT_DMA); GA_SEL_KNOB(NT_DMA2); GA_SEL_KNOB(NT_DMA2_MINK); GA_SEL_KNOB(NT_T256);
    GA_SEL_KNOB(TN2); GA_SEL_KNOB(TN2_PATCH2); GA_SEL_KNOB(TN2_WGS); GA_SEL_KNOB(TN2_PART_MIN);
    GA_SEL_KNOB(CONV3_DIRECT); GA_SEL_KNOB(CONV0_DIRECT); GA_SEL_KNOB(STEM4_WGRAD_DIRECT);
#undef GA_SEL_KNOB
    return k;
}

int lds_error(int bytes) {
    ga_set_error("ga_gemm: cannot reserve %d bytes of LDS", bytes);
    return GA_ERR_HIP;
}

template <typename T, int TNW, int NWM, bool PLAIN, bool PRE, int EPI, bool DMA = false>
int launch_nt_(const ga_gemm_desc* d, hipStream_t s) {
    using CF = NTCfg<TNW, NWM>;
    constexpr int smem = DMA ? CF::SMEM_DMA : CF::SMEM;
    auto kern = gemm_nt_kernel<T, TNW, NWM, PLAIN, PRE, EPI, DMA>;
    static const int per_cu = [&] {
        int n = 0;
        if (smem > 65536 && hipFuncSetAttribute(reinterpret_cast<const void*>(kern),
                                                hipFuncAttributeMaxDynamicSharedMemorySize, smem) != hipSuccess)
            return 0;
        if (hipOccupancyMaxActiveBlocksPerMultiprocessor(&n, kern, CF::NTHR, smem) != hipSuccess || n < 1) n = 1;
        return n;
    }();
    if (per_cu == 0) return lds_error(smem);
    const int tiles = cdiv(d->M, CF::BM) * cdiv(d->N, CF::BN);
    const int cap = std::max(8, (per_cu * ga_num_cus() / d->batch) / 8 * 8);
    dim3 grid(std::min(tiles, cap), 1, d->batch), block(CF::NTHR);
    hipLaunchKernelGGL(kern, grid, block, smem, s, *d);
    return ga_check_launch("ga_gemm");
}

template <int EPI>
int launch_nt_pp(const ga_gemm_desc* d, hipStream_t s) {
    auto kern = gemm_nt_pp_kernel<EPI>;
    static const bool ok = hipFuncSetAttribute(reinterpret_cast<const void*>(kern), hipFuncAttributeMaxDynamicSharedMemorySize, kPPSmem) == hipSuccess;
    if (!ok) return lds_error(kPPSmem);
    const int tiles = cdiv(d->M, 256) * cdiv(d->N, 256);
    const int cap = std::max(8, (ga_num_cus() / d->batch) / 8 * 8);
    dim3 grid(std::min(tiles, cap), 1, d->batch), block(kPPThreads);
#ifdef GAEXT_DEBUG
    const int dbg = GA_KNOB("PP_DBG", 0);
#else
    const int dbg = 0;
#endif
    hipLaunchKernelGGL(kern, grid, block, kPPSmem, s, *d, dbg);
    return ga_check_launch("ga_gemm");
}

template <int EPI, int DBG = 0, int AK = 0>
int launch_nt_r3_(const ga_gemm_desc* d, hipStream_t s) {
    auto kern = gemm_nt_r3_kernel<EPI, DBG, AK>;
    static const bool ok = hipFuncSetAttribute(reinterpret_cast<const void*>(kern), hipFuncAttributeMaxDynamicSharedMemorySize, kR3Smem) == hipSuccess;
    if (!ok) return lds_error(kR3Smem);
    const int tiles = cdiv(d->M, 256) * cdiv(d->N, 128);
    const int cap = std::max(8, (2 * ga_num_cus() / d->batch) / 8 * 8);
    dim3 grid(std::min(tiles, cap), 1, d->batch), block(kR3Threads);
    const int stagger = std::max(0, GA_KNOB("R3_STAGGER", 0));
    hipLaunchKernelGGL(kern, grid, block, kR3Smem, s, *d, stagger);
    return ga_check_launch("ga_gemm");
}
template <int EPI>
int launch_nt_r3(const ga_gemm_desc* d, hipStream_t s) {
#ifdef GAEXT_DEBUG
    switch (GA_KNOB("R3_DBG", 0)) {
        case 1: return launch_nt_r3_<EPI, 1>(d, s);
        case 2: return launch_nt_r3_<EPI, 2>(d, s);
        case 4: return launch_nt_r3_<EPI, 4>(d, s);
        case 6: return launch_nt_r3_<EPI, 6>(d, s);
        case 8: return launch_nt_r3_<EPI, 8>(d, s);
        case 10: return launch_nt_r3_<EPI, 10>(d, s);
        case 17: return launch_nt_r3_<EPI, 17>(d, s);
        case 33: return launch_nt_r3_<EPI, 33>(d, s);
        default: break;
    }
#endif
    return launch_nt_r3_<EPI, 0>(d, s);
}

template <bool GENERIC, typename F>
int with_epi(int epi, F&& f) {
    switch (epi) {
        case EPI_PLAIN: return f(std::integral_constant<int, EPI_PLAIN>{});
        case EPI_FC1: return f(std::integral_constant<int, EPI_FC1>{});
        case EPI_FC2: return f(std::integral_constant<int, EPI_FC2>{});
        case EPI_DG2: return f(std::integral_constant<int, EPI_DG2>{});
        default: break;
    }
    if constexpr (GENERIC) return f(std::integral_constant<int, EPI_GENERIC>{});
    ga_set_error("ga_gemm: form without a generic epilogue");
    return GA_ERR_BAD_ARG;
}

template <typename T, int TNW, int NWM, bool DMA>
int launch_nt_tile(const ga_gemm_desc* d, const NtSel& sel, hipStream_t s) {
    return with_epi<!DMA>(sel.epi, [&](auto e) {
        constexpr int EPI = decltype(e)::value;
        constexpr bool PRE = sizeof(T) == 2 && TNW != 8 && EPI != EPI_PLAIN && EPI != EPI_FC1;
        if constexpr (EPI == EPI_GENERIC) {
            if (d->a_kind != GA_A_PLAIN) return launch_nt_<T, TNW, NWM, false, false, EPI_GENERIC>(d, s);
            if (!sel.pre) return launch_nt_<T, TNW, NWM, true, false, EPI_GENERIC>(d, s);
        }
        return launch_nt_<T, TNW, NWM, true, PRE, EPI, DMA>(d, s);
    });
}
template <typename T>
int launch_nt_staged(const ga_gemm_desc* d, const NtSel& sel, hipStream_t s) {
    if (sel.tnw == 4) return launch_nt_tile<T, 4, 2, false>(d, sel, s);
    if (sel.tnw == 3) return launch_nt_tile<T, 3, 2, false>(d, sel, s);
    return launch_nt_tile<T, 2, 2, false>(d, sel, s);
}

int launch_nt_form(const ga_gemm_desc* d, const NtSel& sel, hipStream_t s) {
    switch (sel.form) {
        case NT_R3G: return launch_nt_r3_<EPI_PLAIN, 0, 1>(d, s);
        case NT_R3: return with_epi<false>(sel.epi, [&](auto e) { return launch_nt_r3<decltype(e)::value>(d, s); });
        case NT_DMA256:
            return sel.tnw == 4 ? launch_nt_tile<bf16_t, 4, 4, true>(d, sel, s) : launch_nt_tile<bf16_t, 3, 4, true>(d, sel, s);
        case NT_PP: return with_epi<false>(sel.epi, [&](auto e) { return launch_nt_pp<decltype(e)::value>(d, s); });
        case NT_T256: return launch_nt_tile<bf16_t, 8, 4, true>(d, sel, s);
        case NT_DMA128: return launch_nt_tile<bf16_t, 4, 2, true>(d, sel, s);
        case NT_BIG:
            return sel.epi == EPI_FC2 ? launch_nt_<bf16_t, 4, 4, true, true, EPI_FC2>(d, s)
                                      : launch_nt_<bf16_t, 4, 4, true, true, EPI_DG2>(d, s);
        default:
            return d->dtype == GA_BF16 ? launch_nt_staged<bf16_t>(d, sel, s) : launch_nt_staged<float>(d, sel, s);
    }
}

int launch_tn2(const ga_wgrad_desc* d, const TnSel& sel, hipStream_t s) {
    static const bool attr_ok = hipFuncSetAttribute(reinterpret_cast<const void*>(gemm_tn2_kernel<false>),
                                                    hipFuncAttributeMaxDynamicSharedMemorySize, kTn2Smem) == hipSuccess &&
                                hipFuncSetAttribute(reinterpret_cast<const void*>(gemm_tn2_kernel<true>),
                                                    hipFuncAttributeMaxDynamicSharedMemorySize, kTn2Smem) == hipSuccess;
    GA_REQUIRE(attr_ok, "ga_wgrad: cannot reserve %d bytes of LDS", kTn2Smem);
    const int split = sel.split;
    dim3 grid2(cdiv(d->N, 256) * cdiv(d->K, 256) * split, 1, d->batch), block2(kTn2Threads);
    float* part = sel.partials ? reinterpret_cast<float*>(d->workspace) : nullptr;
    GA_REQUIRE(!part || aligned16(part), "ga_wgrad: workspace must be 16-byte aligned");
    const long nk = (long)d->N * d->K;
    if (d->x_kind == GA_A_PATCH2) hipLaunchKernelGGL(gemm_tn2_kernel<true>, grid2, block2, kTn2Smem, s, *d, split, part);
    else hipLaunchKernelGGL(gemm_tn2_kernel<false>, grid2, block2, kTn2Smem, s, *d, split, part);
    if (part)
        hipLaunchKernelGGL(tn2_reduce_kernel, dim3((unsigned)std::min<long>(2048, cdiv(nk, 1024)), d->batch), dim3(256),
                           0, s, part, split, nk, d->K, d->alpha, d->dW, d->ldw, d->strideW);
    return ga_check_launch("ga_wgrad");
}

int launch_tn_direct(const ga_wgrad_desc* d, const TnSel& sel, hipStream_t s) {
    switch (sel.form) {
        case TN_CONV3_DIRECT: return ga_conv3_c64_wgrad_launch(d, sel.split, s);
        case TN_CONV3S2_DIRECT: return ga_conv3s2_c64_wgrad_launch(d, sel.split, s);
        case TN_CONV0_DIRECT: return ga_conv0_c8_wgrad_launch(d, sel.split, s);
        default: return ga_stem4_wgrad_launch(d, sel.split, s);
    }
}

}

extern "C" int ga_gemm(const ga_gemm_desc* d, ga_stream_t stream) {
    if (const int rc = nt_validate(d)) return rc;
    hipStream_t s = reinterpret_cast<hipStream_t>(stream);
    Knobs k = current_knobs();
    NtSel sel = nt_select(d, ga_num_cus(), k);
    if (sel.form == NT_CONV3_DIRECT) {
        if (ga_conv3_c64_launch(d, s)) return ga_check_launch("ga_gemm");
        k.CONV3_DIRECT = 0;
        sel = nt_select(d, ga_num_cus(), k);
    }
    if (sel.form == NT_CONV0_DIRECT) {
        ga_conv0_c8_launch(d, s);
        return ga_check_launch("ga_gemm");
    }
    return launch_nt_form(d, sel, s);
}

extern "C" int ga_gemm_form(const ga_gemm_desc* d, char* buf, size_t n) {
    if (const int rc = nt_validate(d)) return rc;
    if (buf && n) nt_form_name(d, nt_select(d, ga_num_cus(), current_knobs()), buf, n);
    return GA_OK;
}

extern "C" int ga_wgrad(const ga_wgrad_desc* d, ga_stream_t stream) {
    if (const int rc = tn_validate(d)) return rc;
    hipStream_t s = reinterpret_cast<hipStream_t>(stream);
    Knobs k = current_knobs();
    TnSel sel = tn_select(d, ga_num_cus(), k);
    if (sel.form <= TN_STEM4_DIRECT) {
        if (launch_tn_direct(d, sel, s)) return ga_check_launch("ga_wgrad");
        k.CONV3_DIRECT = k.CONV0_DIRECT = k.STEM4_WGRAD_DIRECT = 0;
        sel = tn_select(d, ga_num_cus(), k);
    }
    if (sel.form == TN_TN2) return launch_tn2(d, sel, s);
    dim3 grid(cdiv(d->N, 128) * cdiv(d->K, 128) * d->split_m, 1, d->batch), block(kThreads);
    if (d->dtype == GA_BF16)
        hipLaunchKernelGGL(gemm_tn_kernel<bf16_t>, grid, block, 65536, s, *d);
    else
        hipLaunchKernelGGL(gemm_tn_kernel<float>, grid, block, 65536, s, *d);
    return ga_check_launch("ga_wgrad");
}

extern "C" int ga_wgrad_form(const ga_wgrad_desc* d, char* buf, size_t n) {
    if (const int rc = tn_validate(d)) return rc;
    if (buf && n) tn_form_name(d, tn_select(d, ga_num_cus(), current_knobs()), buf, n);
    return GA_OK;
}

extern "C" size_t ga_wgrad_workspace(const ga_wgrad_desc* d) {
    if (!d || d->M <= 0 || d->N <= 0 || d->K <= 0 || d->batch < 1) return 0;
    return tn_select(d, ga_num_cus(), current_knobs()).ws_bytes;
}
```

### imagenet-models_amd/csrc/gemm_select.h

```cpp
#pragma once
#include <stddef.h>
#include <stdint.h>
#include <stdio.h>
#include <algorithm>
#include "../../include/gaext.h"

void ga_set_error(const char* fmt, ...);
bool ga_conv3_c64_eligible(const ga_gemm_desc* d);
bool ga_conv0_c8_eligible(const ga_gemm_desc* d);
int ga_conv3_c64_wgrad_wgs(const ga_wgrad_desc* d, int num_cus);
int ga_conv3s2_c64_wgrad_wgs(const ga_wgrad_desc* d, int num_cus);
int ga_conv0_c8_wgrad_wgs(const ga_wgrad_desc* d, int num_cus);
int ga_stem4_wgrad_wgs(const ga_wgrad_desc* d, int num_cus);

namespace gasel {

enum { EPI_GENERIC = -1, EPI_PLAIN = 0, EPI_FC1 = 1, EPI_FC2 = 2, EPI_DG2 = 3 };

struct Knobs {
    int NT_R3 = -1, NT_R3_NEIGH2 = 1, NT_R3_CONV3S2 = 1, NT_PP = -1, NT_PP_MINK = 512, NT_BIG = -1, NT_DMA = 1, NT_DMA2 = 10,
        NT_DMA2_MINK = 256, NT_T256 = -1;
    int TN2 = 1, TN2_PATCH2 = 1, TN2_WGS = 0, TN2_PART_MIN = 65536;
    int CONV3_DIRECT = 1, CONV0_DIRECT = 1, STEM4_WGRAD_DIRECT = 1;
};

inline int ceil_div(long a, long b) { return (int)((a + b - 1) / b); }
inline uintptr_t addr(const void* p) { return reinterpret_cast<uintptr_t>(p); }
inline bool aligned16(const void* p) { return (addr(p) & 15) == 0; }

#define GA_SEL_REQUIRE(cond, ...) \
    do { if (!(cond)) { ga_set_error(__VA_ARGS__); return GA_ERR_BAD_ARG; } } while (0)

inline int nt_validate(const ga_gemm_desc* d) {
    GA_SEL_REQUIRE(d && d->A && d->B && d->C, "ga_gemm: null operand");
    GA_SEL_REQUIRE(d->M > 0 && d->N > 0 && d->K > 0 && d->batch >= 1, "ga_gemm: bad shape M=%d N=%d K=%d batch=%d", d->M,
                   d->N, d->K, d->batch);
    GA_SEL_REQUIRE(d->dtype == GA_F32 || d->dtype == GA_BF16, "ga_gemm: bad dtype %d", d->dtype);
    const int epc = d->dtype == GA_BF16 ? 8 : 4;
    GA_SEL_REQUIRE(aligned16(d->A) && aligned16(d->B) && aligned16(d->C), "ga_gemm: operands must be 16-byte aligned");
    GA_SEL_REQUIRE(d->ldb % epc == 0 && d->strideB % epc == 0, "ga_gemm: ldb/strideB must be multiples of %d", epc);
    GA_SEL_REQUIRE(d->K % epc == 0, "ga_gemm: K=%d must be a multiple of %d (pad the operand)", d->K, epc);
    if (d->a_kind == GA_A_PLAIN) {
        GA_SEL_REQUIRE(d->lda % epc == 0 && d->strideA % epc == 0, "ga_gemm: lda/strideA must be multiples of %d", epc);
    } else if (d->a_kind == GA_A_PATCH2) {
        GA_SEL_REQUIRE(d->a_C % epc == 0 && d->a_H % 2 == 0 && d->a_W % 2 == 0 && d->K == 4 * d->a_C &&
                           (long)d->M % ((d->a_H / 2) * (d->a_W / 2)) == 0,
                       "ga_gemm: PATCH2 needs C%%%d==0, even H,W, K==4C", epc);
    } else if (d->a_kind == GA_A_CONV3) {
        GA_SEL_REQUIRE(d->a_C % epc == 0 && d->K == 9 * d->a_C && (long)d->M % (d->a_H * d->a_W) == 0,
                       "ga_gemm: CONV3 needs C%%%d==0, K==9C", epc);
    } else if (d->a_kind == GA_A_CONV3S2) {
        GA_SEL_REQUIRE(d->a_C % epc == 0 && d->K == 9 * d->a_C && (long)d->M % (((d->a_H + 1) / 2) * ((d->a_W + 1) / 2)) == 0,
                       "ga_gemm: CONV3S2 needs C%%%d==0, K==9C", epc);
    } else if (d->a_kind == GA_A_NEIGH2) {
        GA_SEL_REQUIRE(d->a_C % epc == 0 && d->K == 4 * d->a_C && (long)d->M % (d->a_H * d->a_W) == 0,
                       "ga_gemm: NEIGH2 needs C%%%d==0, K==4C", epc);
    } else if (d->a_kind == GA_A_STEM4_NCHW) {
        GA_SEL_REQUIRE(d->a_C == 3 && d->K == 48 && d->a_H % 4 == 0 && d->a_W % 4 == 0, "ga_gemm: STEM4 needs C=3,K=48");
    } else {
        GA_SEL_REQUIRE(false, "ga_gemm: bad a_kind %d", d->a_kind);
    }
    if (d->c_kind == GA_C_UNPATCH2) {
        GA_SEL_REQUIRE(d->c_C % 8 == 0 && d->N == 4 * d->c_C && !d->c_f32, "ga_gemm: UNPATCH2 needs N==4*c_C, c_C%%8==0");
    } else {
        GA_SEL_REQUIRE(d->c_kind == GA_C_PLAIN, "ga_gemm: bad c_kind");
    }
    if (d->H) GA_SEL_REQUIRE(aligned16(d->H) && d->ldh % 8 == 0, "ga_gemm: H alignment");
    if (d->C2) GA_SEL_REQUIRE(aligned16(d->C2) && d->c_kind == GA_C_PLAIN && !d->c_f32 && (d->c2_mode == 1 || d->c2_mode == 2),
                              "ga_gemm: C2 needs a plain, dtype-typed C and c2_mode 1|2");
    if (d->R) GA_SEL_REQUIRE(aligned16(d->R) && d->ldr % 8 == 0, "ga_gemm: R alignment");
    if (d->rowscale) GA_SEL_REQUIRE(d->rows_per_scale > 0, "ga_gemm: rows_per_scale");
    GA_SEL_REQUIRE(d->c_kind != GA_C_PLAIN || d->ldc % 8 == 0, "ga_gemm: ldc=%ld must be a multiple of 8", (long)d->ldc);
    return GA_OK;
}

enum NtForm { NT_CONV3_DIRECT, NT_CONV0_DIRECT, NT_R3G, NT_R3, NT_DMA256, NT_PP, NT_T256, NT_DMA128, NT_BIG, NT_STAGED };

struct NtSel {
    int form, epi, tnw, nwm;
    bool pre;
};

inline int classify_epilogue(const ga_gemm_desc* d) {
    if (d->a_act != GA_ACT_NONE || d->alpha != 1.0f || d->c_f32 || d->relu_after) return EPI_GENERIC;
    const bool act0 = d->act == GA_ACT_NONE;
    if (d->act == GA_ACT_GELU && (!d->C2 || d->c2_mode == 2) && !d->H && !d->R && !d->rowscale && !d->colsum) return EPI_FC1;
    if (act0 && !d->C2 && !d->H && d->R && !d->colsum) return EPI_FC2;
    if (act0 && !d->C2 && d->H && d->h_is_deriv && !d->R && !d->rowscale) return EPI_DG2;
    if (act0 && !d->C2 && !d->H && !d->R && !d->rowscale) return EPI_PLAIN;
    return EPI_GENERIC;
}

inline bool ring_gather_a(const ga_gemm_desc* d) {
    return d->a_kind == GA_A_PATCH2 || d->a_kind == GA_A_NEIGH2 || d->a_kind == GA_A_CONV3S2;
}

inline bool pp_wanted(const ga_gemm_desc* d, int epi, int num_cus, const Knobs& k) {
    const bool e = k.NT_PP >= 0;
    const int mask = e ? k.NT_PP : 7;
    if (!mask || d->dtype != GA_BF16 || d->a_kind != GA_A_PLAIN || epi == EPI_GENERIC || !((mask >> epi) & 1)) return false;
    if (d->N % 8 != 0 || d->K < (e ? 256 : k.NT_PP_MINK) || d->ldc % 8 != 0) return false;
    if ((long)d->M * d->lda >= (1L << 30) || (long)d->N * d->ldb >= (1L << 30) || d->lda < 64 || d->ldb < 64) return false;
    const int tn = ceil_div(d->N, 256);
    if (!e && tn * 256 - d->N > tn * 256 / 8) return false;
    return (long)ceil_div(d->M, 256) * tn * d->batch >= num_cus / 2;
}

inline bool r3_wanted(const ga_gemm_desc* d, int epi, int num_cus, const Knobs& k) {
    const bool forced = k.NT_R3 >= 0;
    const int mask = forced ? k.NT_R3 : 15;
    const bool neigh2 = d->a_kind == GA_A_NEIGH2;
    const bool conv3s2 = d->a_kind == GA_A_CONV3S2;
    const bool patch2 = ring_gather_a(d);
    if (patch2 && (epi != EPI_PLAIN || d->a_C % 16 != 0 || d->K != (conv3s2 ? 9 : 4) * d->a_C || 4L * d->M * d->a_C >= (1L << 30) ||
                   d->a_batch_mod || d->batch != 1))
        return false;
    if (neigh2 && (d->a_C % 32 != 0 || (long)d->M % ((long)d->a_H * d->a_W) != 0 || !k.NT_R3_NEIGH2)) return false;
    if (conv3s2 && (d->a_C % 32 != 0 || d->a_H % 2 != 0 || d->a_W % 2 != 0 || d->a_W < 4 ||
                    (long)d->M % ((long)(d->a_H / 2) * (d->a_W / 2)) != 0 || !k.NT_R3_CONV3S2))
        return false;
    if (!mask || d->dtype != GA_BF16 || (d->a_kind != GA_A_PLAIN && !patch2) || epi == EPI_GENERIC || !((mask >> epi) & 1)) return false;
    if (d->N % 8 != 0 || d->K < 64 || d->ldc % 8 != 0) return false;
    if ((!patch2 && (long)d->M * d->lda >= (1L << 30)) || (long)d->N * d->ldb >= (1L << 30)) return false;
    const bool unpatch2 = d->c_kind == GA_C_UNPATCH2;
    if (unpatch2 && (epi != EPI_PLAIN || d->colsum || d->c_C % 8 != 0 || d->N != 4 * d->c_C || 4L * d->M * d->c_C >= (1L << 30) || d->batch != 1))
        return false;
    if ((!unpatch2 && (long)d->M * d->ldc >= (1L << 30)) || (d->c_kind != GA_C_PLAIN && !unpatch2) || d->c_f32) return false;
    if (epi == EPI_DG2 && (long)d->M * d->ldh >= (1L << 30)) return false;
    if (epi == EPI_FC2 && (long)d->M * d->ldr >= (1L << 30)) return false;
    if (d->bias && (addr(d->bias) & 3)) return false;
    if (forced) return true;
    if (neigh2 || conv3s2) return (long)ceil_div(d->M, 256) * ceil_div(d->N, 128) >= 16;
    if ((long)ceil_div(d->M, 256) * ceil_div(d->N, 128) * d->batch < num_cus / 2) return false;
    const bool pp = pp_wanted(d, epi, num_cus, k);
    if (d->M >= 65536 && pp) return false;
    if (epi != EPI_PLAIN) return true;
    if (d->K <= 512) return true;
    if (pp) return d->N < 2048 && d->K < 3072;
    return d->N >= 384 ? d->K < 3072 : d->K >= 1024;
}

inline bool dma_offsets_fit(const ga_gemm_desc* d) { return (long)d->M * d->lda < (1L << 30) && (long)d->N * d->ldb < (1L << 30); }
inline bool dma_operands(const ga_gemm_desc* d, int epi) {
    return d->dtype == GA_BF16 && d->a_kind == GA_A_PLAIN && epi != EPI_GENERIC && dma_offsets_fit(d);
}

inline bool dma256_wanted(const ga_gemm_desc* d, int epi, int tnw, int num_cus, const Knobs& k) {
    const int mode = k.NT_DMA;
    if (!mode || !dma_operands(d, epi) || (tnw != 4 && tnw != 3)) return false;
    if ((long)ceil_div(d->M, 256) * ceil_div(d->N, 32 * tnw) * d->batch < num_cus) return false;
    return mode == 2 || (epi == EPI_FC2 && tnw == 4 && d->K >= 1024);
}

inline bool t256_wanted(const ga_gemm_desc* d, int epi, int num_cus, const Knobs& k) {
    const int mask = k.NT_T256 >= 0 ? k.NT_T256 : ((d->M >= 65536 && d->N >= 768) ? 15 : 0);
    if (!mask || !dma_operands(d, epi)) return false;
    if (d->N % 256 != 0 || d->K < 256) return false;
    if ((long)ceil_div(d->M, 256) * (d->N / 256) * d->batch < num_cus) return false;
    return (mask >> epi) & 1;
}

inline bool dma128_wanted(const ga_gemm_desc* d, int epi, int tnw, const Knobs& k) {
    if (tnw != 4 || !k.NT_DMA2 || !dma_operands(d, epi)) return false;
    if (d->K < k.NT_DMA2_MINK) return false;
    return (k.NT_DMA2 >> epi) & 1;
}

inline bool big_wanted(const ga_gemm_desc* d, int epi, int tnw, int num_cus, const Knobs& k) {
    if (tnw != 4 || d->dtype != GA_BF16 || d->a_kind != GA_A_PLAIN || (epi != EPI_FC2 && epi != EPI_DG2)) return false;
    if (k.NT_BIG >= 0) return k.NT_BIG != 0;
    return (long)ceil_div(d->M, 256) * ceil_div(d->N, 128) * d->batch >= 2L * num_cus;
}

inline int nt_tile_width(int N) {
    if (N % 128 == 0) return 4;
    if (N % 96 == 0) return 3;
    if (N % 64 == 0) return 2;
    const long w4 = (long)ceil_div(N, 128) * 128, w3 = (long)ceil_div(N, 96) * 96, w2 = (long)ceil_div(N, 64) * 64;
    return (w4 <= w3 && w4 <= w2) ? 4 : (w3 <= w2 ? 3 : 2);
}

inline NtSel nt_select(const ga_gemm_desc* d, int num_cus, const Knobs& k) {
    const int tnw = nt_tile_width(d->N);
    if (k.CONV3_DIRECT && ga_conv3_c64_eligible(d)) return {NT_CONV3_DIRECT, EPI_PLAIN, 0, 0, false};
    if (k.CONV0_DIRECT && ga_conv0_c8_eligible(d)) return {NT_CONV0_DIRECT, EPI_PLAIN, 0, 0, false};
    const int cls = classify_epilogue(d);
    const bool plain_layout = d->a_kind == GA_A_PLAIN && d->c_kind == GA_C_PLAIN;
    const bool ring_layout = !plain_layout && (d->a_kind == GA_A_PLAIN || ring_gather_a(d));
    if (ring_layout && cls == EPI_PLAIN && r3_wanted(d, EPI_PLAIN, num_cus, k))
        return {d->a_kind == GA_A_NEIGH2 || d->a_kind == GA_A_CONV3S2 ? NT_R3G : NT_R3, EPI_PLAIN, 4, 4, false};
    const int epi = plain_layout ? cls : EPI_GENERIC;
    const bool pre = epi == EPI_FC2 || epi == EPI_DG2;
    if (r3_wanted(d, epi, num_cus, k)) return {NT_R3, epi, 4, 4, false};
    if (dma256_wanted(d, epi, tnw, num_cus, k)) return {NT_DMA256, epi, tnw, 4, pre};
    if (pp_wanted(d, epi, num_cus, k)) return {NT_PP, epi, 8, 4, false};
    if (t256_wanted(d, epi, num_cus, k)) return {NT_T256, epi, 8, 4, false};
    if (dma128_wanted(d, epi, tnw, k)) return {NT_DMA128, epi, 4, 2, pre};
    if (big_wanted(d, epi, tnw, num_cus, k)) return {NT_BIG, epi, 4, 4, true};
    const bool bf = d->dtype == GA_BF16;
    if (d->a_kind != GA_A_PLAIN) return {NT_STAGED, EPI_GENERIC, tnw, 2, false};
    return {NT_STAGED, epi, tnw, 2, bf && (pre || (epi == EPI_GENERIC && (d->H || d->R)))};
}

inline void nt_form_name(const ga_gemm_desc* d, const NtSel& s, char* buf, size_t n) {
    const char* const form[] = {"conv3_direct", "conv0_direct", "r3g", "r3", "dma256x", "pp", "t256", "dma128", "big", "staged"};
    const char* const epi[] = {"generic", "plain", "fc1", "fc2", "dg2"};
    if (s.form <= NT_CONV0_DIRECT) snprintf(buf, n, "%s", form[s.form]);
    else if (s.form != NT_DMA256 && s.form != NT_STAGED) snprintf(buf, n, "%s:%s", form[s.form], epi[s.epi + 1]);
    else snprintf(buf, n, "%s%d:%s%s%s%s", form[s.form], 32 * s.tnw, epi[s.epi + 1], s.form == NT_STAGED && s.pre ? "+pre" : "",
                  d->a_kind != GA_A_PLAIN ? "+gather" : "", d->dtype == GA_F32 ? "+f32" : "");
}

inline int tn_validate(const ga_wgrad_desc* d) {
    GA_SEL_REQUIRE(d && d->Y && d->X && d->dW, "ga_wgrad: null operand");
    GA_SEL_REQUIRE(d->M > 0 && d->N > 0 && d->K > 0 && d->batch >= 1 && d->split_m >= 1, "ga_wgrad: bad shape");
    GA_SEL_REQUIRE(d->dtype == GA_F32 || d->dtype == GA_BF16, "ga_wgrad: bad dtype %d", d->dtype);
    const int epc = d->dtype == GA_BF16 ? 8 : 4;
    GA_SEL_REQUIRE(aligned16(d->Y) && aligned16(d->X), "ga_wgrad: operands must be 16-byte aligned");
    GA_SEL_REQUIRE(d->N % epc == 0 && d->ldy % epc == 0 && d->strideY % epc == 0, "ga_wgrad: N/ldy must be multiples of %d",
                   epc);
    if (d->x_kind == GA_A_PLAIN) {
        GA_SEL_REQUIRE(d->ldx % epc == 0 && d->strideX % epc == 0 && d->ldx >= (d->K + epc - 1) / epc * epc,
                       "ga_wgrad: ldx must be a multiple of %d and cover K rounded up", epc);
    } else if (d->x_kind == GA_A_PATCH2 || d->x_kind == GA_A_NEIGH2 || d->x_kind == GA_A_CONV3 || d->x_kind == GA_A_CONV3S2) {
        const int taps = d->x_kind == GA_A_PATCH2 || d->x_kind == GA_A_NEIGH2 ? 4 : 9;
        GA_SEL_REQUIRE(d->x_C % epc == 0 && d->K == taps * d->x_C, "ga_wgrad: %s needs K==%dC",
                       d->x_kind == GA_A_PATCH2 ? "PATCH2" : d->x_kind == GA_A_NEIGH2 ? "NEIGH2" : d->x_kind == GA_A_CONV3 ? "CONV3" : "CONV3S2", taps);
    } else if (d->x_kind == GA_A_STEM4_NCHW) {
        GA_SEL_REQUIRE(d->x_C == 3 && d->K == 48, "ga_wgrad: STEM4 needs C=3,K=48");
    } else {
        GA_SEL_REQUIRE(false, "ga_wgrad: bad x_kind %d", d->x_kind);
    }
    return GA_OK;
}

enum TnForm { TN_CONV3_DIRECT, TN_CONV3S2_DIRECT, TN_CONV0_DIRECT, TN_STEM4_DIRECT, TN_TN2, TN_TN };

struct TnSel {
    int form;
    int split;
    size_t ws_bytes;
    bool partials;
};

inline bool tn2_eligible(const ga_wgrad_desc* d, const Knobs& k) {
    if (!(k.TN2 && d->dtype == GA_BF16 && d->x_act == GA_ACT_NONE && d->M % 32 == 0 && d->M >= 8192 &&
          (d->accumulate || d->split_m > 1) && (long)d->M * d->ldy < (1L << 31)))
        return false;
    if (d->x_kind == GA_A_PLAIN) return (long)d->M * d->ldx < (1L << 31);
    if (d->x_kind == GA_A_PATCH2)
        return k.TN2_PATCH2 && d->x_C > 0 && d->x_C % 8 == 0 && d->K == 4 * d->x_C && d->x_H > 0 && d->x_W > 0 &&
               d->x_H % 2 == 0 && d->x_W % 2 == 0 && d->M % ((long)(d->x_H / 2) * (d->x_W / 2)) == 0 &&
               8L * d->M * d->x_C < (1L << 31);
    return false;
}

inline size_t tn2_plan(const ga_wgrad_desc* d, int num_cus, const Knobs& k, int* split_out) {
    const int tiles = ceil_div(d->N, 256) * ceil_div(d->K, 256) * d->batch;
    const int stages = d->M / 32;
    const int cus = k.TN2_WGS > 0 ? k.TN2_WGS : num_cus * 3 / 4;
    int split = std::max(1, std::min(stages / 8, cus / tiles));
    split = ceil_div(stages, ceil_div(stages, split));
    *split_out = split;
    const long nk = (long)d->N * d->K;
    const long nk_min = k.TN2_PART_MIN;
    return (split > 1 && nk >= nk_min) ? (size_t)d->batch * split * nk * sizeof(float) : 0;
}

inline TnSel tn_select(const ga_wgrad_desc* d, int num_cus, const Knobs& k) {
    const bool has_ws = d->workspace != nullptr;
    int wgs;
    size_t need;
    auto direct = [&](int form, size_t per_wg) -> TnSel {
        need = (size_t)wgs * per_wg * sizeof(float);
        if (has_ws && (size_t)d->ws_bytes >= need) return {form, wgs, need, true};
        return {TN_TN, d->split_m, need, false};
    };
    if (k.CONV3_DIRECT && (wgs = ga_conv3_c64_wgrad_wgs(d, num_cus))) return direct(TN_CONV3_DIRECT, 64 * 576);
    if (k.CONV3_DIRECT && (wgs = ga_conv3s2_c64_wgrad_wgs(d, num_cus))) return direct(TN_CONV3S2_DIRECT, 64 * 576);
    if (k.CONV0_DIRECT && (wgs = ga_conv0_c8_wgrad_wgs(d, num_cus))) return direct(TN_CONV0_DIRECT, 64 * 72);
    if (k.STEM4_WGRAD_DIRECT && (wgs = ga_stem4_wgrad_wgs(d, num_cus))) return direct(TN_STEM4_DIRECT, (size_t)d->N * 49);
    if (tn2_eligible(d, k)) {
        int split;
        need = tn2_plan(d, num_cus, k, &split);
        return {TN_TN2, split, need, need && has_ws && (size_t)d->ws_bytes >= need};
    }
    return {TN_TN, d->split_m, 0, false};
}

inline void tn_form_name(const ga_wgrad_desc* d, const TnSel& s, char* buf, size_t n) {
    const char* const form[] = {"conv3_wgrad_direct", "conv3s2_wgrad_direct", "conv0_wgrad_direct", "stem4_wgrad_direct", "tn2", "tn"};
    if (s.form == TN_TN) snprintf(buf, n, "tn");
    else if (s.form != TN_TN2) snprintf(buf, n, "%s:wgs%d", form[s.form], s.split);
    else snprintf(buf, n, "tn2%s:split%d:%s", d->x_kind == GA_A_PATCH2 ? "p" : "", s.split, s.partials ? "partials" : "atomics");
}

#undef GA_SEL_REQUIRE

}
```

### include/gaext.h

```cpp
#ifndef GAEXT_H
#define GAEXT_H
#include <stddef.h>
#include <stdint.h>

#ifdef __cplusplus
extern "C" {
#endif

typedef void* ga_stream_t;

enum { GA_F32 = 0, GA_BF16 = 1 };
enum { GA_OK = 0, GA_ERR_BAD_ARG = -1, GA_ERR_UNSUPPORTED = -2, GA_ERR_HIP = -3 };

enum { GA_ACT_NONE = 0, GA_ACT_GELU = 1, GA_ACT_RELU = 2 };

enum {
    GA_A_PLAIN = 0,
    GA_A_PATCH2 = 1,
    GA_A_STEM4_NCHW = 2,
    GA_A_CONV3 = 3,
    GA_A_CONV3S2 = 4,
    GA_A_NEIGH2 = 5
};
enum {
    GA_C_PLAIN = 0,
    GA_C_UNPATCH2 = 1
};

int ga_version(void);
int ga_last_error(char* buf, size_t n);
int ga_device_info(int* num_cu, int* lds_bytes, int* wave_size);

int ga_set_knob(const char* name, int value);
int ga_unset_knob(const char* name);
int ga_config_string(char* buf, size_t n);

typedef struct {
    int M, N, K;
    int batch;
    int dtype;
    const void* A;
    int64_t lda, strideA;
    int a_batch_mod;
    int a_kind;
    int a_H, a_W, a_C;
    int a_act;
    const void* B;
    int64_t ldb, strideB;
    void* C;
    int64_t ldc, strideC;
    int c_kind;
    int c_H, c_W, c_C;
    int c_f32;
    void* C2;
    int c2_mode;
    float alpha;
    const float* bias;
    int64_t strideBias;
    int act;
    const void* H;
    int64_t ldh, strideH;
    int h_is_deriv;
    const float* rowscale;
    int rows_per_scale;
    const void* R;
    int64_t ldr, strideR;
    int relu_after;
    float* colsum;
    float* colsumsq;
    int64_t strideCol;
} ga_gemm_desc;
int ga_gemm(const ga_gemm_desc* d, ga_stream_t stream);

typedef struct {
    int M, N, K;
    int batch;
    int dtype;
    const void* Y;
    int64_t ldy, strideY;
    const void* X;
    int64_t ldx, strideX;
    int x_batch_mod;
    int x_kind;
    int x_H, x_W, x_C;
    int x_act;
    float* dW;
    int64_t ldw, strideW;
    float* dbias;
    int64_t strideDbias;
    float alpha;
    int split_m;
    int accumulate;
    void* workspace;
    int64_t ws_bytes;
} ga_wgrad_desc;
int ga_wgrad(const ga_wgrad_desc* d, ga_stream_t stream);
size_t ga_wgrad_workspace(const ga_wgrad_desc* d);

int ga_gemm_form(const ga_gemm_desc* d, char* buf, size_t n);
int ga_wgrad_form(const ga_wgrad_desc* d, char* buf, size_t n);

typedef struct {
    const float* w;
    int G, Co, Ci, KH, KW;
    const float* rs;
    const float* cs;
    const int* row_perm;
    int dtype;
    void* out;  int64_t ldo;
    void* outT; int64_t ldt;
    int flip;
    int stem;
    int t_cols;
} ga_wprep_desc;
int ga_weight_prep(const ga_wprep_desc* d, ga_stream_t stream);
int ga_bias_fold(const float* W, const float* b, const float* rs, const float* v, const int* row_perm, float* be, int N,
                 int C, ga_stream_t stream);
typedef struct {
    const float* G; int64_t ldg;
    const float* gb;
    const float* W; const float* b;
    const float* rs; const float* cs; const float* v;
    const int* row_perm;
    int N, Ci, KH, KW;
    int stem;
    float* dW; float* db; float* d_rs; float* d_cs; float* d_v;
} ga_wunfold_desc;
int ga_weight_unfold(const ga_wunfold_desc* d, ga_stream_t stream);

int ga_dwconv7_fwd(const void* x, const float* w49, const float* bias, void* y, int B, int H, int W, int C,
                   int dtype, ga_stream_t stream);
int ga_dwconv7_bwd_data(const void* dy, const float* w49, const void* res, void* dx, int B, int H, int W, int C,
                        int dtype, ga_stream_t stream);
int ga_dwconv7_bwd_data2(const void* dy, const float* w49, const void* res, void* dx, void* dx2, const float* scale2,
                         int B, int H, int W, int C, int dtype, ga_stream_t stream);
size_t ga_dwconv7_bwd_weight_workspace(int B, int H, int W, int C, int dtype);
int ga_dwconv7_bwd_weight(const void* dy, const void* x, float* dw49, float* dbias, int B, int H, int W, int C,
                          int dtype, void* workspace, size_t ws_bytes, ga_stream_t stream);

int ga_dwconv3_fwd(const void* x, const float* w9, void* y, int B, int H, int W, int C, int stride, float* colsum,
                   float* colsumsq, int dtype, ga_stream_t stream);
int ga_dwconv3_bwd_data(const void* dy, const float* w9, void* dx, int B, int H, int W, int C, int stride, int dtype,
                        ga_stream_t stream);
size_t ga_dwconv3_bwd_weight_workspace(int B, int H, int W, int C, int stride, int dtype);
int ga_dwconv3_bwd_weight(const void* dy, const void* x, float* dw9, int B, int H, int W, int C, int stride, int dtype,
                          void* workspace, size_t ws_bytes, ga_stream_t stream);

int ga_maxpool3s2_fwd(const void* x, void* y, unsigned char* idx, int B, int H, int W, int C, int dtype, ga_stream_t stream);
int ga_maxpool3s2_bwd(const void* dy, const unsigned char* idx, void* dx, int B, int H, int W, int C, int accumulate, int dtype,
                      ga_stream_t stream);
int ga_bn_gelu_fwd(const void* x, const float* scale, const float* shift, void* y, int64_t rows, int C, int dtype, ga_stream_t stream);
size_t ga_bn_gelu_bwd_workspace(int64_t rows, int C);
int ga_bn_gelu_bwd_reduce(const void* dy, const void* x, const float* scale, const float* shift, const float* mean, const float* rstd,
                          float* s1, float* s2, int64_t rows, int C, int dtype, void* workspace, size_t ws_bytes, ga_stream_t stream);
int ga_bn_gelu_bwd_apply(const void* dy, const void* x, const float* scale, const float* shift, const float* mean, const float* rstd,
                         const float* w, const float* s1, const float* s2, int64_t n, void* dx, int64_t rows, int C, int dtype,
                         ga_stream_t stream);
int ga_se_bn_fwd(const float* S, int HW, const float* scale3, const float* shift3, const float* W1, const float* g1, const float* b1,
                 float* rmean, float* rvar, const float* W2, const float* b2, float* hpre, float* mean, float* rstd, float* h, float* gate,
                 int B, int C, int R, int training, ga_stream_t stream);
int ga_se_bn_bwd(const float* P1, const float* P2, const float* rowscale, const float* g3, const float* b3, const float* mean3,
                 const float* rstd3, const float* S, int HW, const float* scale3, const float* shift3, const float* W1, const float* g1,
                 const float* b1, const float* W2, const float* hpre, const float* mean, const float* rstd, const float* h,
                 const float* gate, float* dz, float* dhpre, float* ds, float* s1, float* s2, float* dW1, float* dg1, float* db1,
                 float* dW2, float* db2, int B, int C, int R, ga_stream_t stream);
int ga_se_residual_fwd(const void* x3, const float* scale3, const float* shift3, const float* gate, const float* rowscale, const void* res,
                       const float* rscale, const float* rshift, void* y, int B, int HW, int C, int dtype, ga_stream_t stream);
int ga_se_residual_bwd_a(const void* dy, const void* y, const void* x3, const float* mean3, const float* rstd3, void* dm, float* P1,
                         float* P2, int B, int HW, int C, int dtype, ga_stream_t stream);
int ga_se_residual_bwd_b(const void* dm, const void* x3, const float* mean3, const float* rstd3, const float* g3, const float* gate,
                         const float* rowscale, const float* ds, const float* s1, const float* s2, void* dx3, int B, int HW, int C,
                         int dtype, ga_stream_t stream);
int ga_subsample2_fwd(const void* x, void* y, int B, int H, int W, int C, int dtype, ga_stream_t stream);
int ga_subsample2_bwd(const void* dy, void* dx, int B, int H, int W, int C, int accumulate, int dtype, ga_stream_t stream);

int ga_layernorm_fwd(const void* x, const float* w, const float* b, void* y, float* mean, float* rstd, int64_t rows,
                     int C, float eps, int dtype, ga_stream_t stream);
int ga_layernorm_bwd(const void* g, const void* x, const float* mean, const float* rstd, const float* w,
                     const void* dres, void* dx, float* dw, float* db, int64_t rows, int C, int x_is_normalized,
                     int dtype, ga_stream_t stream);
int ga_layernorm_bwd_dp(const void* g, const void* x, const float* mean, const float* rstd, const float* w, const void* dres,
                        void* dx, float* dw, float* db, int64_t rows, int C, int x_is_normalized, void* dx2, const float* scale2,
                        int64_t rows_per_scale, int dtype, ga_stream_t stream);

int ga_bn_finalize(const float* sum, const float* sumsq, int64_t n, const float* w, const float* b, float eps,
                   float momentum, float* running_mean, float* running_var, float* mean_out, float* rstd_out,
                   float* scale, float* shift, int C, int training, ga_stream_t stream);
int ga_affine_act(const void* x, const float* scale, const float* shift, const void* res, const float* rowscale,
                  int64_t rows_per_scale, void* y, int64_t rows, int C, int relu, int dtype, int64_t ldx, ga_stream_t stream);
int ga_bn_bwd_reduce(const void* dy, const void* y_relu, const void* x, const float* mean, const float* rstd,
                     const float* rowscale, int64_t rows_per_scale, float* s1, float* s2, int64_t rows, int C, int dtype,
                     int64_t ldx, ga_stream_t stream);
int ga_bn_bwd_apply(const void* dy, const void* y_relu, const void* x, const float* mean, const float* rstd,
                    const float* w, const float* s1, const float* s2, const float* rowscale, int64_t rows_per_scale,
                    int64_t n, void* dx, int64_t rows, int C, int dtype, int64_t ldx, int64_t lddx, ga_stream_t stream);

int ga_pool_concat_fwd(const void* src, void* dst, int B, int Hin, int Win, int C, int Hout, int Wout, int ldd,
                       int c_off, int mode, int dtype, ga_stream_t stream);
int ga_pool_concat_bwd(const void* dcat, const void* dres, void* dsrc, int B, int Hin, int Win, int C, int Hout,
                       int Wout, int ldd, int c_off, int mode, int dtype, ga_stream_t stream);

int ga_spatial_sum(const void* a, const void* b2, float* out, int B, int HW, int C, float scale, int dtype,
                   ga_stream_t stream);
int ga_se_mlp_fwd(const float* s, const float* W1, const float* b1, const float* W2, const float* b2, float* hid,
                  float* gate, int B, int C, int R, ga_stream_t stream);
int ga_se_mlp_bwd(const float* dgate, const float* gate, const float* hid, const float* s, const float* W1,
                  const float* W2, float* ds, float ds_scale, float* dW1, float* db1, float* dW2, float* db2, int B,
                  int C, int R, ga_stream_t stream);
int ga_chan_scale(const void* x, const float* g, const float* add, void* y, int B, int HW, int C, int dtype,
                  ga_stream_t stream);

int ga_gram_pack_fwd(const float* G, void* out, float* inv_norm, int B, int C, int groups, int Kp, int dtype,
                     ga_stream_t stream);
int ga_gram_pack_bwd(const void* dvec, const void* vhat, const float* inv_norm, void* S, int B, int C, int groups,
                     int Kp, int dtype, ga_stream_t stream);

size_t ga_gram_f64_fwd_workspace(int B, int C);
size_t ga_gram_f64_bwd_workspace(int B, int C);
int ga_gram_f64_fwd(const void* x, void* vec, double* inv_norm, double* G64, size_t g64_bytes, int B, int HW, int C, int H,
                    int groups, int Kp, int dtype, ga_stream_t stream);
int ga_gram_f64_bwd(const void* dvec, const void* x, const double* G64, const double* inv_norm, void* dx, void* workspace,
                    size_t ws_bytes, int B, int HW, int C, int H, int groups, int Kp, int dtype, ga_stream_t stream);

int ga_token_cat(const void* cls, const void* tok, void* u, int B, int N, int C, int dtype, ga_stream_t stream);
int ga_token_split(const void* du, void* dcls, void* dtok, int B, int N, int C, int acc_cls, int acc_tok, int dtype,
                   ga_stream_t stream);
int ga_class_attn_fwd(const void* q, const void* kv, void* out, float* P, int B, int N, int heads, int hd, float scale,
                      int dtype, ga_stream_t stream);
int ga_class_attn_bwd(const void* dout, const void* q, const void* kv, const float* P, void* dq, void* dkv, int B, int N,
                      int heads, int hd, float scale, int dtype, ga_stream_t stream);
int ga_class_attn_fwd2(const void* q, const void* kv_cls, const void* kv_tok, int64_t tok_ld, void* out, float* P, int B, int N,
                       int heads, int hd, float scale, int dtype, ga_stream_t stream);
int ga_class_attn_bwd2(const void* dout, const void* q, const void* kv_cls, const void* kv_tok, int64_t tok_ld, const float* P,
                       void* dq, void* dkv_cls, void* dkv_tok, int B, int N, int heads, int hd, float scale, int dtype,
                       ga_stream_t stream);

int ga_loss_fwd_bwd(const float* logits, const int64_t* target, float* loss, void* dlogits, int K, int B, int NC,
                    float lam, int kind, float smoothing, float grad_scale, int dtype, ga_stream_t stream);
int ga_heads_topk(const float* logits, int K, int B, int NC, int topk, float* out_sum, int64_t* out_idx,
                  ga_stream_t stream);

int ga_sgd_step(float* p, const float* g, float* buf, const float* hp, int64_t n, int nesterov, float wd_mult,
                ga_stream_t stream);
int ga_adamw_step(float* p, const float* g, float* m, float* v, const float* hp, int64_t n, float wd_mult,
                  ga_stream_t stream);

typedef struct {
    int kind;
    float* y; const float* x; float a; int64_t n;
    int R, C, accumulate;
    const float* b; const float* rs; const float* v; const int* row_perm;
} ga_small_desc;
int ga_weight_prep_batch(const ga_wprep_desc* jobs_dev, int n, ga_stream_t stream);
int ga_weight_unfold_batch(const ga_wunfold_desc* jobs_dev, int n, ga_stream_t stream);
int ga_small_batch(const ga_small_desc* jobs_dev, int n, ga_stream_t stream);

int ga_lamb_stage1(const float* p, const float* g, float* m, float* v, float* u, const float* hp, const float* gsumsq,
                   const int* chunks, int nchunks, float* norms, ga_stream_t stream);
int ga_lamb_stage2(float* p, const float* u, const float* hp, const int* chunks, int nchunks, const float* norms,
                   ga_stream_t stream);

int ga_sumsq_f32(const float* x, int64_t n, float* out, ga_stream_t stream);
int ga_clip_grad_f32(float* g, int64_t n, const float* sumsq, float limit, int mode, ga_stream_t stream);

typedef struct {
    int B, reso, C, heads, nbranch;
    int Hs[2], Ws[2];
    const float* lepe_w[2];
    const float* lepe_b[2];
    float scale;
    int dtype;
    const void* qkv; int64_t ldq;
    void* out; int64_t ldo;
} ga_cswin_attn_desc;
int ga_cswin_attn_fwd(const ga_cswin_attn_desc* d, ga_stream_t stream);
size_t ga_cswin_attn_bwd_workspace(const ga_cswin_attn_desc* d);
int ga_cswin_attn_bwd(const ga_cswin_attn_desc* d, const void* dout, void* dqkv, void* lepe_ws, size_t ws_bytes, ga_stream_t stream);
int ga_cswin_lepe_wgrad_reduce(const ga_cswin_attn_desc* d, const void* lepe_ws, float* dw0, float* db0, float* dw1, float* db1,
                               ga_stream_t stream);
int ga_cswin_lepe_wgrad(const ga_cswin_attn_desc* d, const void* dout, float* dw0, float* db0, float* dw1, float* db1,
                        ga_stream_t stream);
int ga_layernorm_gelu_fwd(const void* x, const float* w, const float* b, void* y, float* mean, float* rstd, int64_t rows,
                          int C, float eps, int dtype, ga_stream_t stream);
int ga_layernorm_gelu_bwd(const void* g, const void* x, const float* mean, const float* rstd, const float* w, const float* b,
                          void* dx, float* dw, float* db, int64_t rows, int C, int dtype, ga_stream_t stream);
int ga_nchw3_to_nhwc8(const float* x, void* y, int B, int H, int W, int dtype, ga_stream_t stream);
int ga_convw_pack(const float* w, void* out, int Co, int Ci, int taps, int Cp, int64_t ldo, int dtype, ga_stream_t stream);
int ga_convw_unpack_grad(const float* G, float* dW, int Co, int Ci, int taps, int Cp, int64_t ldg, ga_stream_t stream);
int ga_conv3s2_dgrad_prep(const float* w, void* out, int Co, int Ci, int64_t ldo, int dtype, ga_stream_t stream);

int ga_gram_pack_fwd2(const float* G, void* out, float* inv_norm, int B, int C, int groups, int Kp, int ntok, int dtype,
                      ga_stream_t stream);
int ga_gram_pack_bwd2(const void* dvec, const void* vhat, const float* inv_norm, void* S, int B, int C, int groups, int Kp,
                      int ntok, int dtype, ga_stream_t stream);
int ga_map_tokens_fwd(const void* e, void* tok, int B, int C, int T, int add_mean, int dtype, ga_stream_t stream);
int ga_map_tokens_bwd(const void* dtok, void* de, int B, int C, int T, int add_mean, int dtype, ga_stream_t stream);
int ga_class_attn_mt_fwd(const void* q, const void* kv_cls, const void* kv_tok, int64_t tok_ld, void* out, float* P,
                         const float* mask, int B, int T, int N, int heads, int hd, float scale, int dtype, ga_stream_t stream);
int ga_class_attn_mt_bwd(const void* dout, const void* q, const void* kv_cls, const void* kv_tok, int64_t tok_ld, const float* P,
                         const float* mask, void* dq, void* dkv_cls, void* dkv_tok, int64_t dtok_ld, int B, int T, int N,
                         int heads, int hd, float scale, int dtype, ga_stream_t stream);
int ga_class_attn_mt_ia_fwd(const void* q, const void* kv_cls, const void* kv_tok, int64_t tok_ld, void* out, float* P,
                            const float* mask, const float* W1, const float* b1, const float* W2, const float* b2, int B, int T, int N,
                            int heads, int hd, float scale, int dtype, ga_stream_t stream);
int ga_class_attn_mt_ia_bwd(const void* dout, const void* q, const void* kv_cls, const void* kv_tok, int64_t tok_ld, const float* P,
                            const float* mask, const float* W1, const float* W2, const float* b2, void* dq, void* dkv_cls,
                            void* dkv_tok, int64_t dtok_ld, float* dW1, float* db1, float* dW2, float* db2, int B, int T, int N,
                            int heads, int hd, float scale, int dtype, ga_stream_t stream);
int ga_map_loss_fwd_bwd(const float* org, const float* avg, const int64_t* target, float* loss, void* dorg, void* davg, int K,
                        int B, int NC, float lam, int kind, float smoothing, float grad_scale, int dtype, ga_stream_t stream);
int ga_loss_dense_fwd_bwd(const float* org, const float* avg, const int64_t* target, const float* dense, float* loss, void* dorg,
                          void* davg, int K, int B, int NC, float lam, int kind, float smoothing, float bce_threshold,
                          float grad_scale, int dtype, ga_stream_t stream);
int ga_mixup_batch(const float* x, float* out, int B, int CH, int H, int W, double lam, int cutmix, int yl, int yh, int xl, int xh,
                   ga_stream_t stream);
int ga_mixup_target(const int64_t* target, float* out, int B, int NC, double lam, double smoothing, ga_stream_t stream);
int ga_u8_normalize(const void* x, float* out, int B, int CH, int H, int W, const float* mean, const float* std, ga_stream_t stream);
int ga_input_erase(const void* x, int x_is_u8, float* out, int B, int CH, int H, int W, const float* mean, const float* std,
                   const int32_t* boxes, int max_count, int mode, uint64_t seed, uint64_t offset, ga_stream_t stream);
int ga_input_collate(const void* x, int x_is_u8, float* out, int B, int CH, int H, int W, const float* mean, const float* std,
                     const int32_t* mix, const int32_t* boxes, int max_count, int mode, uint64_t seed, uint64_t offset,
                     ga_stream_t stream);
int ga_mixup_target_elem(const int64_t* target, float* out, int B, int NC, const float* lam, double smoothing, ga_stream_t stream);
int ga_rand_augment(const void* x, void* out, void* work, size_t work_bytes, int B, int CH, int H, int W, const void* ops, int n_layers,
                    const uint8_t* fill, ga_stream_t stream);
size_t ga_rand_augment_work_bytes(int B, int CH, int H, int W, int n_layers);
int ga_rand_augment_check_table(const void* ops_host, int rows);
int ga_resize_crop(const void* src, uint64_t src_bytes, const void* rows, void* out, void* work, size_t work_bytes, int B, int OH, int OW,
                   ga_stream_t stream);
size_t ga_resize_crop_work_bytes(const void* rows_host, int B, int OH, int OW);
int ga_resize_crop_check_table(const void* rows_host, int B, int OH, int OW, uint64_t src_bytes);
int ga_resample_coeffs(int in_size, int out_size, int interp, int32_t* bounds, int32_t* coeffs, int ksize, ga_stream_t stream);
int ga_jpeg_probe(const uint8_t* bytes, size_t n, int64_t* info);
int ga_jpeg_entropy_decode(const uint8_t* bytes, size_t n, int16_t* coef, size_t coef_capacity, uint16_t* qt);
int ga_jpeg_check_table(const void* rows_host, int n_images, uint64_t coef_count, uint64_t qt_count, uint64_t work_bytes,
                        uint64_t dst_bytes);
size_t ga_jpeg_work_bytes(const void* rows_host, int n_images);
int ga_jpeg_reconstruct(const void* table, int n_images, const int16_t* coef, const uint16_t* qt, void* work, void* dst,
                        ga_stream_t stream);
int ga_agc_clip(const float* params, float* grads, const int64_t* units, int nunits, float clip_factor, float eps, ga_stream_t stream);
int ga_gelu_fwd(const void* x, void* y, int64_t n, int dtype, ga_stream_t stream);
int ga_gelu_bwd(const void* dy, const void* x, void* dx, int64_t n, int dtype, ga_stream_t stream);
int ga_relu_drop(const void* a, const float* mask, void* out, void* deriv, int64_t n, int dtype, ga_stream_t stream);
int ga_mask_mul(const void* x, const float* mask, const void* res, void* y, int64_t n, int dtype, ga_stream_t stream);
int ga_copy2d(const void* src, int64_t lds, void* dst, int64_t ldd, int64_t rows, int cols, int accumulate, int dtype,
              ga_stream_t stream);

int ga_drop_path_sample(float* out, const float* keep, int sites, int B, uint64_t seed, uint64_t* counter, ga_stream_t stream);

int ga_dropout_mask_sample(float* out, int64_t n, float keep, uint64_t seed, uint64_t* counter, ga_stream_t stream);

typedef struct {
    const void* X; int64_t ldx;
    const void* W1; int64_t ldw1; const float* b1;
    const void* W2; int64_t ldw2; const float* b2;
    const void* R; int64_t ldr;
    const float* rowscale; int rows_per_scale;
    void* Y; int64_t ldy;
    int64_t M; int C, H, dtype;
} ga_mlp_desc;
typedef struct {
    const void* X; int64_t ldx;
    const void* DY; int64_t lddy;
    const void* W1; int64_t ldw1; const float* b1;
    const void* W2T; int64_t ldw2t;
    const void* W1T; int64_t ldw1t;
    void* A; int64_t lda;
    void* DH; int64_t lddh;
    void* DX; int64_t lddx;
    int64_t M; int C, H, dtype;
    float* dW1; int64_t ldw;
    float* db1;
    float* partials; size_t partials_bytes;
    int max_blocks;
} ga_mlp_bwd_desc;
int ga_mlp_supported(int C, int H, int dtype);
int ga_mlp_fwd(const ga_mlp_desc* d, ga_stream_t stream);
int ga_mlp_bwd(const ga_mlp_bwd_desc* d, ga_stream_t stream);
int ga_mlp_bwd_wgrad_supported(int C, int H, int dtype);
size_t ga_mlp_bwd_partials(const ga_mlp_bwd_desc* d);

typedef struct {
    int rows, groups, Ng, Kg;
    const void* A; int64_t lda; int64_t a_gstride; const int* a_perm;
    const float* W; const float* bias; const float* col_scale;
    const float* rowscale; int rows_per_scale;
    const void* R; int64_t ldr;
    void* Y; int64_t ldy; void* Yraw;
    int dtype;
} ga_small_linear_desc;
int ga_small_linear_fwd(const ga_small_linear_desc* d, ga_stream_t stream);
int ga_small_linear_bwd(const ga_small_linear_desc* d, const void* dY, void* dA, int accumulate_dA, float* dW, float* dbias,
                        float* dcol_scale, ga_stream_t stream);
int ga_colstats(const void* x, int64_t ld, int rows, int C, float* sum, float* sumsq, int dtype, ga_stream_t stream);
int ga_pad_copy_f32(const float* src, float* dst, int64_t rows, int64_t cols, int64_t lds, int64_t ldd, int accumulate, ga_stream_t stream);
int ga_stem4_ln_fwd(const float* x, const void* W, int64_t ldw, const float* bias, const float* gamma, const float* beta, void* pre,
                    void* y, float* mean, float* rstd, int B, int H, int W_, int C, float eps, ga_stream_t stream);
int ga_blockdiag_f32(const float* src, float* dst, int64_t R, int rg, int ng, int cg, int64_t ld, int to_diag, int accumulate,
                     ga_stream_t stream);
int ga_pad_groups_f32(const float* src, float* dst, int64_t R, int64_t C, int RG, int RGp, int CG, int CGp, int unpad, int accumulate,
                      ga_stream_t stream);
int ga_pad_copy(const void* src, void* dst, int64_t rows, int64_t cols, int64_t lds, int64_t ldd, int accumulate, int dtype,
                ga_stream_t stream);

typedef struct {
    int B, N, H, hd;
    float scale;
    int dtype;
    const void* qkv; int64_t ldq;
    void* out; int64_t ldo;
    float* lse;
} ga_attn_desc;
int ga_attn_fwd(const ga_attn_desc* d, ga_stream_t stream);
size_t ga_attn_bwd_workspace(const ga_attn_desc* d);
int ga_attn_bwd(const ga_attn_desc* d, const void* dout, void* dqkv, void* workspace, size_t ws_bytes, ga_stream_t stream);
int ga_patchify(const float* x, void* out, int B, int CH, int H, int W, int P, int dtype, ga_stream_t stream);
int ga_vit_embed_fwd(const void* tok, const float* cls, const float* pos, void* x0, int B, int Np, int C, int dtype, ga_stream_t stream);
int ga_vit_embed_bwd(const void* dx0, void* dtok, float* dcls, float* dpos, int B, int Np, int C, int dtype, ga_stream_t stream);

int ga_patchify_strided(const float* x, void* out, int B, int CH, int H, int W, int P, int S, int dtype, ga_stream_t stream);
int ga_pos_add_fwd(const void* tok, const float* pos, void* x0, int B, int Np, int C, int dtype, ga_stream_t stream);
int ga_pos_add_bwd(const void* dx0, float* dpos, int B, int Np, int C, int dtype, ga_stream_t stream);
int ga_dwpool_fwd(const void* x, const float* w, const float* bias, void* y, int B, int H, int W, int Cin, int mult, int dtype,
                  ga_stream_t stream);
int ga_dwpool_bwd_data(const void* dy, const float* w, void* dx, int B, int H, int W, int Cin, int mult, int dtype, ga_stream_t stream);
int ga_dwpool_bwd_weight(const void* dy, const void* x, float* dw, float* db, int B, int H, int W, int Cin, int mult, int dtype,
                         ga_stream_t stream);
int ga_resize_concat_fwd(const void* src, void* dst, int B, int Hin, int Win, int C, int Hout, int Wout, int64_t ldd, int c_off,
                         int dtype, ga_stream_t stream);
int ga_resize_concat_bwd(const void* dcat, void* dsrc, int B, int Hin, int Win, int C, int Hout, int Wout, int64_t ldd, int c_off,
                         int dtype, ga_stream_t stream);
int ga_rows_bcast(const void* src, void* dst, int B, int HW, int C, float scale, int dtype, ga_stream_t stream);
int ga_token_gap_fwd(const void* x, void* y, int B, int N, int C, int dtype, ga_stream_t stream);
int ga_token_gap_bwd(const void* dy, void* dx, int B, int N, int C, int dtype, ga_stream_t stream);

int ga_memset(void* p, int value, size_t bytes, ga_stream_t stream);
int ga_transpose_f32(const float* in, float* out, int R, int C, int accumulate, ga_stream_t stream);
int ga_axpy_f32(float* y, const float* x, float a, int64_t n, ga_stream_t stream);
int ga_lerp_f32(float* y, const float* x, float w, int64_t n, ga_stream_t stream);
int ga_rowscale(const void* x, const float* s, void* y, int64_t n, int64_t elems_per_scale, int dtype,
                ga_stream_t stream);
int ga_cast_from_f32(const float* src, void* dst, int64_t n, int dtype, ga_stream_t stream);
int ga_cast_to_f32(const void* src, float* dst, int64_t n, int dtype, ga_stream_t stream);

typedef struct ga_comm* ga_comm_t;
int ga_comm_unique_id(void* id128);
int ga_comm_init(ga_comm_t* comm, int rank, int world, const void* id128);
int ga_comm_destroy(ga_comm_t comm);
int ga_comm_info(ga_comm_t comm, int* rank, int* world);
size_t ga_allreduce_workspace(int64_t n, int wire_dtype);
int ga_allreduce_bucket(ga_comm_t comm, float* grads, int64_t n, int wire_dtype, float scale, void* workspace, size_t ws_bytes,
                        ga_stream_t stream);
int ga_reduce_scatter_bucket(ga_comm_t comm, const float* grads, float* shard, int64_t n_per_rank, float scale, ga_stream_t stream);
int ga_allgather_bucket(ga_comm_t comm, const float* shard, float* full, int64_t n_per_rank, ga_stream_t stream);
int ga_comm_broadcast(ga_comm_t comm, void* buf, int64_t n_f32, int root, ga_stream_t stream);

#ifdef __cplusplus
}
#endif
#endif
```

Before: 11050 images/sec.

## Add deeper register-staged prefetch for staged NT and TN GEMMs on small grids

Adds an AHEAD template depth to the register-staged NT GEMM and the TN wgrad kernel. It prefetches several K slabs ahead through buffer loads into multiple register sets, and for NT it double-buffers LDS. Selection heuristics enable it only for plain bf16 operands when the grid underfills the CUs and K has enough slabs, so that more memory latency is hidden per workgroup. The cost is more registers and LDS, and a lower launch-bounds occupancy hint.

```diff
diff --git a/imagenet-models_amd/_lib.py b/imagenet-models_amd/_lib.py
--- a/imagenet-models_amd/_lib.py
+++ b/imagenet-models_amd/_lib.py
@@ -138,6 +138,8 @@
     'ga_wgrad_workspace': ([C.POINTER(WgradDesc)], C.c_size_t),
     'ga_gemm_form': ([C.POINTER(GemmDesc), C.c_char_p, C.c_size_t], i32),
     'ga_wgrad_form': ([C.POINTER(WgradDesc), C.c_char_p, C.c_size_t], i32),
+    'ga_gemm_ahead': ([C.POINTER(GemmDesc)], i32),
+    'ga_wgrad_ahead': ([C.POINTER(WgradDesc)], i32),
     'ga_layernorm_fwd': ([vp, vp, vp, vp, vp, vp, i64, i32, f32, i32, vp], i32),
     'ga_layernorm_bwd': ([vp, vp, vp, vp, vp, vp, vp, vp, vp, i64, i32, i32, i32, vp], i32),
     'ga_layernorm_bwd_dp': ([vp, vp, vp, vp, vp, vp, vp, vp, vp, i64, i32, i32, vp, vp, i64, i32, vp], i32),
@@ -293,7 +295,7 @@
     s = buf.value.decode(errors='replace')
     host = sorted(k for k in os.environ if k.startswith(('GAEXT_', 'GA_FUSED_MLP')) and k != 'GAEXT_LIB')
     known = {'GAEXT_ASYNC_WGRAD', 'GAEXT_FWD_SPLIT', 'GAEXT_PAR_BRANCH', 'GAEXT_FWD_SKEW', 'GAEXT_FUSE_DP', 'GAEXT_HEAD_STREAMS',
-             'GA_FUSED_MLP', 'GAEXT_SMALL_SINGLE', 'GAEXT_SYNC_DEBUG', 'GAEXT_MLP_WG1'}
+             'GA_FUSED_MLP', 'GAEXT_SMALL_SINGLE', 'GAEXT_SYNC_DEBUG', 'GAEXT_MLP_WG1', 'GAEXT_STAGED_AHEAD'}
     for k in host:
         if k in known:
             s += f' host:{k}={os.environ[k]}'
diff --git a/imagenet-models_amd/csrc/gemm.hip b/imagenet-models_amd/csrc/gemm.hip
--- a/imagenet-models_amd/csrc/gemm.hip
+++ b/imagenet-models_amd/csrc/gemm.hip
@@ -218,8 +218,8 @@
 
 using gasel::EPI_GENERIC, gasel::EPI_PLAIN, gasel::EPI_FC1, gasel::EPI_FC2, gasel::EPI_DG2;
 
-template <typename T, int TNW, int NWM, bool PLAIN, bool PRE, int EPI, bool DMA = false>
-__global__ __launch_bounds__(128 * NWM, (NWM == 2 && !DMA && !PRE && EPI >= 0 && sizeof(T) == 2 && TNW == 3) ? 3 : (NWM == 2 && DMA) ? 2 : 1) void gemm_nt_kernel(const ga_gemm_desc d) {
+template <typename T, int TNW, int NWM, bool PLAIN, bool PRE, int EPI, bool DMA = false, int AHEAD = 1>
+__global__ __launch_bounds__(128 * NWM, (AHEAD == 1 && NWM == 2 && !DMA && !PRE && EPI >= 0 && sizeof(T) == 2 && TNW == 3) ? 3 : (NWM == 2 && DMA) ? 2 : 1) void gemm_nt_kernel(const ga_gemm_desc d) {
 #define F_GELU (EPI < 0 ? d.act == GA_ACT_GELU : EPI == EPI_FC1)
 #define F_RELU (EPI < 0 ? d.act == GA_ACT_RELU : false)
 #define F_C2 (EPI < 0 ? d.C2 != nullptr : (EPI == EPI_FC1 && d.C2 != nullptr))
@@ -238,6 +238,7 @@
     constexpr int BN = CF::BN;
     static_assert(!DMA || (PLAIN && sizeof(T) == 2), "the LDS-DMA form needs plain bf16 operands");
     static_assert(DMA || (CF::BN * 8) % CF::NTHR == 0, "B slab must split evenly over the threads");
+    static_assert(AHEAD == 1 || (!DMA && PLAIN && sizeof(T) == 2 && AHEAD <= 4), "deep staging: register-staged form, plain bf16 operands");
     extern __shared__ __attribute__((aligned(16))) unsigned char smem[];
     constexpr int RING0 = DMA ? CF::RING0 : 0;
     unsigned char* As = smem + RING0;
@@ -271,8 +272,8 @@
         }
     };
 
-    uint4 ra[4], rb[CF::NB];
-    auto g_load = [&](int kt) {
+    uint4 ra[AHEAD][4], rb[AHEAD][CF::NB];
+    auto g_load = [&](int kt, int set) {
         const int k = kt * BK + kc * EPC;
         const bool kv = k < d.K;
         if constexpr (PLAIN) {
@@ -280,29 +281,29 @@
 #pragma unroll
             for (int i = 0; i < 4; ++i) {
                 const long m = (long)m0 + r0 + CF::RSTEP * i;
-                ra[i] = (kv && m < d.M) ? *reinterpret_cast<const uint4*>(Ap + m * d.lda) : make_uint4(0, 0, 0, 0);
+                ra[set][i] = (kv && m < d.M) ? *reinterpret_cast<const uint4*>(Ap + m * d.lda) : make_uint4(0, 0, 0, 0);
             }
         } else {
             const KCtx kx = make_k(d.a_kind, k, d.K, d.a_H, d.a_W, d.a_C);
 #pragma unroll
-            for (int i = 0; i < 4; ++i) ra[i] = load_chunk<T>(d.a_kind, Ab, arow[i], kx, d.a_H, d.a_W, d.a_C);
+            for (int i = 0; i < 4; ++i) ra[set][i] = load_chunk<T>(d.a_kind, Ab, arow[i], kx, d.a_H, d.a_W, d.a_C);
         }
 #pragma unroll
         for (int i = 0; i < CF::NB; ++i) {
             const long n = (long)n0 + r0 + CF::RSTEP * i;
-            rb[i] = (kv && n < d.N) ? *reinterpret_cast<const uint4*>(Bb + n * d.ldb + k) : make_uint4(0, 0, 0, 0);
+            rb[set][i] = (kv && n < d.N) ? *reinterpret_cast<const uint4*>(Bb + n * d.ldb + k) : make_uint4(0, 0, 0, 0);
         }
     };
-    auto s_store = [&]() {
+    auto s_store = [&](int set) {
 #pragma unroll
         for (int i = 0; i < 4; ++i) {
             const int row = r0 + CF::RSTEP * i;
-            *reinterpret_cast<uint4*>(As + row * kRowBytes + ((kc ^ (row & 7)) << 4)) = act_chunk<T>(ra[i], F_AACT);
+            *reinterpret_cast<uint4*>(As + row * kRowBytes + ((kc ^ (row & 7)) << 4)) = act_chunk<T>(ra[set][i], F_AACT);
         }
 #pragma unroll
         for (int i = 0; i < CF::NB; ++i) {
             const int row = r0 + CF::RSTEP * i;
-            *reinterpret_cast<uint4*>(Bs + row * kRowBytes + ((kc ^ (row & 7)) << 4)) = rb[i];
+            *reinterpret_cast<uint4*>(Bs + row * kRowBytes + ((kc ^ (row & 7)) << 4)) = rb[set][i];
         }
     };
 
@@ -338,6 +339,37 @@
                 const int p = i * CF::NW + wave;
                 if (p < 4 * TNW) blds16(rsB, kdead ? kOob : boff[i], soff, dst + CF::A_BYTES + p * 1024);
             }
+        }
+    };
+
+    unsigned zaoff[AHEAD > 1 ? 4 : 1], zboff[AHEAD > 1 ? CF::NB : 1];
+    auto deep_rows = [&]() {
+        if constexpr (AHEAD > 1) {
+#pragma unroll
+            for (int i = 0; i < 4; ++i) {
+                const long m = (long)m0 + r0 + CF::RSTEP * i;
+                zaoff[i] = m < d.M ? (unsigned)(m * d.lda + kc * EPC) * 2u : kOob;
+            }
+#pragma unroll
+            for (int i = 0; i < CF::NB; ++i) {
+                const long n = (long)n0 + r0 + CF::RSTEP * i;
+                zboff[i] = n < d.N ? (unsigned)(n * d.ldb + kc * EPC) * 2u : kOob;
+            }
+        }
+    };
+    auto deep_load = [&](int kt, int set) {
+        if constexpr (AHEAD > 1) {
+            const __amdgpu_buffer_rsrc_t brA = __builtin_amdgcn_make_buffer_rsrc(const_cast<unsigned char*>(Ab), 0, (int)kOob, 0x00020000);
+            const __amdgpu_buffer_rsrc_t brB = __builtin_amdgcn_make_buffer_rsrc(const_cast<T*>(Bb), 0, (int)kOob, 0x00020000);
+            const unsigned kdead = (unsigned)(kt >= nk) | ((unsigned)(ktail != 0) & (unsigned)(kt == nk - 1) & (unsigned)(kc * EPC >= ktail));
+            const unsigned dead = kdead * kOob;
+            const unsigned soff = (unsigned)kt * (unsigned)kRowBytes;
+#pragma unroll
+            for (int i = 0; i < 4; ++i)
+                ra[set][i] = __builtin_bit_cast(uint4, __builtin_amdgcn_raw_buffer_load_b128(brA, zaoff[i] | dead, soff, 0));
+#pragma unroll
+            for (int i = 0; i < CF::NB; ++i)
+                rb[set][i] = __builtin_bit_cast(uint4, __builtin_amdgcn_raw_buffer_load_b128(brB, zboff[i] | dead, soff, 0));
         }
     };
 
@@ -378,8 +410,8 @@
     if constexpr (DMA) {
 #pragma unroll
         for (int j = 0; j < CF::NS - 1; ++j) issue_next();
-    } else {
-        g_load(0);
+    } else if constexpr (AHEAD == 1) {
+        g_load(0, 0);
     }
     for (; vt < nwg; ) {
     const int cm0 = m0, cn0 = n0;
@@ -393,13 +425,29 @@
 #pragma unroll
         for (int j = 0; j < 4; ++j) acc[i][j] = f32x4_t{0.f, 0.f, 0.f, 0.f};
 
+    if constexpr (AHEAD > 1) {
+        deep_rows();
+#pragma unroll
+        for (int j = 0; j < AHEAD; ++j) deep_load(j, j);
+        As = smem;
+        Bs = As + CF::A_BYTES;
+    }
     if constexpr (!DMA) {
-        s_store();
+        s_store(0);
         __syncthreads();
     }
 
-    for (int kt = 0; kt < nk; ++kt) {
-        if constexpr (DMA) {
+    for (int kt0 = 0; kt0 < nk; kt0 += AHEAD) {
+#pragma unroll
+    for (int j = 0; j < AHEAD; ++j) {
+        const int kt = kt0 + j;
+        const bool live = AHEAD == 1 || kt < nk;
+        if constexpr (AHEAD > 1) {
+            deep_load(kt + AHEAD, j);
+            __builtin_amdgcn_sched_barrier(0);
+            As = smem + (kt & 1) * CF::SMEM_AB;
+            Bs = As + CF::A_BYTES;
+        } else if constexpr (DMA) {
             if (CF::NS == 3 && inflight >= 2) asm volatile("s_waitcnt vmcnt(6)" ::: "memory");
             else asm volatile("s_waitcnt vmcnt(0)" ::: "memory");
             __builtin_amdgcn_s_barrier();
@@ -409,8 +457,9 @@
             Bs = As + CF::A_BYTES;
             cslot = cslot + 1 == CF::NS ? 0 : cslot + 1;
         } else {
-            if (kt + 1 < nk) g_load(kt + 1);
-        }
+            if (kt + 1 < nk) g_load(kt + 1, 0);
+        }
+        if (live) {
         if constexpr (kPre) {
             if (kt == nk - 1 && use_pre) {
 #pragma unroll
@@ -453,18 +502,27 @@
                 }
             }
         }
-        if constexpr (!DMA) {
+        }
+        if constexpr (AHEAD > 1) {
+            if (kt + 1 < nk) {
+                As = smem + ((kt + 1) & 1) * CF::SMEM_AB;
+                Bs = As + CF::A_BYTES;
+                s_store((j + 1) % AHEAD);
+            }
+            __syncthreads();
+        } else if constexpr (!DMA) {
             __syncthreads();
             if (kt + 1 < nk) {
-                s_store();
+                s_store(0);
                 __syncthreads();
             }
         }
+    }
     }
     vt += gridDim.x;
     if (vt < nwg) {
         set_tile(vt);
-        if constexpr (!DMA) g_load(0);
+        if constexpr (!DMA && AHEAD == 1) g_load(0, 0);
     }
 
     float bias[8], csum[8], csq[8];
@@ -1406,8 +1464,9 @@
 
 __device__ __forceinline__ int tn_swz(int row) { return ((row & 3) << 1) | (((row >> 3) & 1) << 3); }
 
-template <typename T>
-__global__ __launch_bounds__(kThreads, 2) void gemm_tn_kernel(const ga_wgrad_desc d) {
+template <typename T, int AHEAD = 1>
+__global__ __launch_bounds__(kThreads, AHEAD > 1 ? 1 : 2) void gemm_tn_kernel(const ga_wgrad_desc d) {
+    static_assert(AHEAD == 1 || (sizeof(T) == 2 && AHEAD <= 4), "deep staging: bf16");
     using P = TN<T>;
     constexpr int EPC = P::EPC;
     extern __shared__ __attribute__((aligned(16))) unsigned char smem[];
@@ -1436,7 +1495,7 @@
     const bool yv = ny < d.N;
     const KCtx kx = make_k(d.x_kind, k0 + cc * EPC, d.K, d.x_H, d.x_W, d.x_C);
 
-    uint4 ry[4], rx[4];
+    uint4 ry[AHEAD][4], rx[AHEAD][4];
     float bsum[8];
 #pragma unroll
     for (int j = 0; j < 8; ++j) bsum[j] = 0.f;
@@ -1446,31 +1505,47 @@
 #pragma unroll
         for (int i = 0; i < 4; ++i) {
             const long m = slab * P::ROWS + rr + P::RSTEP * i;
-            ry[i] = (yv && m < d.M) ? *reinterpret_cast<const uint4*>(Yb + m * d.ldy + ny) : make_uint4(0, 0, 0, 0);
+            ry[0][i] = (yv && m < d.M) ? *reinterpret_cast<const uint4*>(Yb + m * d.ldy + ny) : make_uint4(0, 0, 0, 0);
             const RowCtx r = make_row(d.x_kind, m, d.M, d.ldx, d.x_H, d.x_W, d.x_C);
-            rx[i] = load_chunk<T>(d.x_kind, Xb, r, kx, d.x_H, d.x_W, d.x_C);
+            rx[0][i] = load_chunk<T>(d.x_kind, Xb, r, kx, d.x_H, d.x_W, d.x_C);
         }
     };
-    auto s_store = [&](int buf) {
+    auto deep_load = [&](long slab, int set) {
+        if constexpr (AHEAD > 1) {
+            constexpr unsigned kOob = 0x80000000u;
+            const __amdgpu_buffer_rsrc_t brY = __builtin_amdgcn_make_buffer_rsrc(const_cast<T*>(Yb), 0, (int)kOob, 0x00020000);
+            const __amdgpu_buffer_rsrc_t brX = __builtin_amdgcn_make_buffer_rsrc(const_cast<unsigned char*>(Xb), 0, (int)kOob, 0x00020000);
+#pragma unroll
+            for (int i = 0; i < 4; ++i) {
+                const long m = slab * P::ROWS + rr + P::RSTEP * i;
+                const unsigned mdead = (unsigned)(slab >= s_end) | (unsigned)(m >= d.M);
+                const unsigned oy = ((unsigned)(m * d.ldy + ny) * 2u) | ((mdead | (unsigned)!yv) * kOob);
+                const unsigned ox = ((unsigned)(m * d.ldx + kx.off) * 2u) | ((mdead | (unsigned)!kx.valid) * kOob);
+                ry[set][i] = __builtin_bit_cast(uint4, __builtin_amdgcn_raw_buffer_load_b128(brY, oy, 0, 0));
+                rx[set][i] = __builtin_bit_cast(uint4, __builtin_amdgcn_raw_buffer_load_b128(brX, ox, 0, 0));
+            }
+        }
+    };
+    auto s_store = [&](int buf, int set) {
         unsigned char* Ys = smem + buf * 32768;
         unsigned char* Xs = Ys + 16384;
 #pragma unroll
         for (int i = 0; i < 4; ++i) {
             const int row = rr + P::RSTEP * i;
             const int off = sizeof(T) == 2 ? row * P::RB + ((cc ^ tn_swz(row)) << 4) : row * P::RB + (cc << 4);
-            *reinterpret_cast<uint4*>(Ys + off) = ry[i];
-            *reinterpret_cast<uint4*>(Xs + off) = act_chunk<T>(rx[i], d.x_act);
+            *reinterpret_cast<uint4*>(Ys + off) = ry[set][i];
+            *reinterpret_cast<uint4*>(Xs + off) = act_chunk<T>(rx[set][i], d.x_act);
             if (do_bias) {
                 if constexpr (sizeof(T) == 2) {
-                    const unsigned w[4] = {ry[i].x, ry[i].y, ry[i].z, ry[i].w};
+                    const unsigned w[4] = {ry[set][i].x, ry[set][i].y, ry[set][i].z, ry[set][i].w};
 #pragma unroll
                     for (int j = 0; j < 4; ++j) {
                         bsum[2 * j] += __uint_as_float(w[j] << 16);
                         bsum[2 * j + 1] += __uint_as_float(w[j] & 0xffff0000u);
                     }
                 } else {
-                    bsum[0] += __uint_as_float(ry[i].x); bsum[1] += __uint_as_float(ry[i].y);
-                    bsum[2] += __uint_as_float(ry[i].z); bsum[3] += __uint_as_float(ry[i].w);
+                    bsum[0] += __uint_as_float(ry[set][i].x); bsum[1] += __uint_as_float(ry[set][i].y);
+                    bsum[2] += __uint_as_float(ry[set][i].z); bsum[3] += __uint_as_float(ry[set][i].w);
                 }
             }
         }
@@ -1482,14 +1557,27 @@
 #pragma unroll
         for (int j = 0; j < 4; ++j) acc[i][j] = f32x4_t{0.f, 0.f, 0.f, 0.f};
 
-    g_load(s_begin);
-    s_store(0);
+    if constexpr (AHEAD > 1) {
+#pragma unroll
+        for (int j = 0; j < AHEAD; ++j) deep_load(s_begin + j, j);
+    } else {
+        g_load(s_begin);
+    }
+    s_store(0, 0);
     __syncthreads();
-    for (long s = s_begin; s < s_end; ++s) {
+    for (long s0 = s_begin; s0 < s_end; s0 += AHEAD) {
+#pragma unroll
+    for (int j = 0; j < AHEAD; ++j) {
+        const long s = s0 + j;
+        const bool live = AHEAD == 1 || s < s_end;
         const int cur = (int)((s - s_begin) & 1);
-        if (s + 1 < s_end) g_load(s + 1);
+        if constexpr (AHEAD > 1) {
+            deep_load(s + AHEAD, j);
+            __builtin_amdgcn_sched_barrier(0);
+        } else if (s + 1 < s_end) g_load(s + 1);
         const unsigned char* Ys = smem + cur * 32768;
         const unsigned char* Xs = Ys + 16384;
+        if (live) {
         if constexpr (sizeof(T) == 2) {
 #pragma unroll
             for (int ks = 0; ks < 2; ++ks) {
@@ -1535,8 +1623,10 @@
                         acc[tn][tk] = __builtin_amdgcn_mfma_f32_16x16x4f32(yf[tn], xf[tk], acc[tn][tk], 0, 0, 0);
             }
         }
-        if (s + 1 < s_end) s_store(cur ^ 1);
+        }
+        if (s + 1 < s_end) s_store(cur ^ 1, (j + 1) % AHEAD);
         __syncthreads();
+    }
     }
 
     float* W = d.dW + z * d.strideW;
@@ -1779,7 +1869,7 @@
     GA_SEL_KNOB(NT_R3); GA_SEL_KNOB(NT_R3_NEIGH2); GA_SEL_KNOB(NT_R3_CONV3S2); GA_SEL_KNOB(NT_PP); GA_SEL_KNOB(NT_PP_MINK);
     GA_SEL_KNOB(NT_BIG); GA_SEL_KNOB(NT_DMA); GA_SEL_KNOB(NT_DMA2); GA_SEL_KNOB(NT_DMA2_MINK); GA_SEL_KNOB(NT_T256);
     GA_SEL_KNOB(TN2); GA_SEL_KNOB(TN2_PATCH2); GA_SEL_KNOB(TN2_WGS); GA_SEL_KNOB(TN2_PART_MIN);
-    GA_SEL_KNOB(CONV3_DIRECT); GA_SEL_KNOB(CONV0_DIRECT); GA_SEL_KNOB(STEM4_WGRAD_DIRECT);
+    GA_SEL_KNOB(CONV3_DIRECT); GA_SEL_KNOB(CONV0_DIRECT); GA_SEL_KNOB(STEM4_WGRAD_DIRECT); GA_SEL_KNOB(STAGED_AHEAD);
 #undef GA_SEL_KNOB
     return k;
 }
@@ -1789,11 +1879,11 @@
     return GA_ERR_HIP;
 }
 
-template <typename T, int TNW, int NWM, bool PLAIN, bool PRE, int EPI, bool DMA = false>
+template <typename T, int TNW, int NWM, bool PLAIN, bool PRE, int EPI, bool DMA = false, int AHEAD = 1>
 int launch_nt_(const ga_gemm_desc* d, hipStream_t s) {
     using CF = NTCfg<TNW, NWM>;
-    constexpr int smem = DMA ? CF::SMEM_DMA : CF::SMEM;
-    auto kern = gemm_nt_kernel<T, TNW, NWM, PLAIN, PRE, EPI, DMA>;
+    constexpr int smem = DMA ? CF::SMEM_DMA : AHEAD > 1 ? std::max(2 * CF::SMEM_AB, CF::SMEM) : CF::SMEM;
+    auto kern = gemm_nt_kernel<T, TNW, NWM, PLAIN, PRE, EPI, DMA, AHEAD>;
     static const int per_cu = [&] {
         int n = 0;
         if (smem > 65536 && hipFuncSetAttribute(reinterpret_cast<const void*>(kern),
@@ -1872,25 +1962,35 @@
 }
 
 template <typename T, int TNW, int NWM, bool DMA>
-int launch_nt_tile(const ga_gemm_desc* d, const NtSel& sel, hipStream_t s) {
+int launch_nt_tile(const ga_gemm_desc* d, const NtSel& sel, hipStream_t s, int ahead = 1) {
     return with_epi<!DMA>(sel.epi, [&](auto e) {
         constexpr int EPI = decltype(e)::value;
         constexpr bool PRE = sizeof(T) == 2 && TNW != 8 && EPI != EPI_PLAIN && EPI != EPI_FC1;
         if constexpr (EPI == EPI_GENERIC) {
             if (d->a_kind != GA_A_PLAIN) return launch_nt_<T, TNW, NWM, false, false, EPI_GENERIC>(d, s);
+        }
+        if constexpr (!DMA && NWM == 2 && sizeof(T) == 2) {
+            if (ahead > 1) {
+                if constexpr (EPI == EPI_GENERIC) {
+                    if (!sel.pre) return launch_nt_<T, TNW, NWM, true, false, EPI_GENERIC, false, kAheadDepth>(d, s);
+                }
+                return launch_nt_<T, TNW, NWM, true, PRE, EPI, false, kAheadDepth>(d, s);
+            }
+        }
+        if constexpr (EPI == EPI_GENERIC) {
             if (!sel.pre) return launch_nt_<T, TNW, NWM, true, false, EPI_GENERIC>(d, s);
         }
         return launch_nt_<T, TNW, NWM, true, PRE, EPI, DMA>(d, s);
     });
 }
 template <typename T>
-int launch_nt_staged(const ga_gemm_desc* d, const NtSel& sel, hipStream_t s) {
-    if (sel.tnw == 4) return launch_nt_tile<T, 4, 2, false>(d, sel, s);
-    if (sel.tnw == 3) return launch_nt_tile<T, 3, 2, false>(d, sel, s);
-    return launch_nt_tile<T, 2, 2, false>(d, sel, s);
-}
-
-int launch_nt_form(const ga_gemm_desc* d, const NtSel& sel, hipStream_t s) {
+int launch_nt_staged(const ga_gemm_desc* d, const NtSel& sel, hipStream_t s, int ahead) {
+    if (sel.tnw == 4) return launch_nt_tile<T, 4, 2, false>(d, sel, s, ahead);
+    if (sel.tnw == 3) return launch_nt_tile<T, 3, 2, false>(d, sel, s, ahead);
+    return launch_nt_tile<T, 2, 2, false>(d, sel, s, ahead);
+}
+
+int launch_nt_form(const ga_gemm_desc* d, const NtSel& sel, hipStream_t s, int ahead) {
     switch (sel.form) {
         case NT_R3G: return launch_nt_r3_<EPI_PLAIN, 0, 1>(d, s);
         case NT_R3: return with_epi<false>(sel.epi, [&](auto e) { return launch_nt_r3<decltype(e)::value>(d, s); });
@@ -1903,7 +2003,7 @@
             return sel.epi == EPI_FC2 ? launch_nt_<bf16_t, 4, 4, true, true, EPI_FC2>(d, s)
                                       : launch_nt_<bf16_t, 4, 4, true, true, EPI_DG2>(d, s);
         default:
-            return d->dtype == GA_BF16 ? launch_nt_staged<bf16_t>(d, sel, s) : launch_nt_staged<float>(d, sel, s);
+            return d->dtype == GA_BF16 ? launch_nt_staged<bf16_t>(d, sel, s, ahead) : launch_nt_staged<float>(d, sel, s, 1);
     }
 }
 
@@ -1951,7 +2051,13 @@
         ga_conv0_c8_launch(d, s);
         return ga_check_launch("ga_gemm");
     }
-    return launch_nt_form(d, sel, s);
+    return launch_nt_form(d, sel, s, nt_ahead(d, sel, ga_num_cus(), k));
+}
+
+extern "C" int ga_gemm_ahead(const ga_gemm_desc* d) {
+    if (const int rc = nt_validate(d)) return rc;
+    const Knobs k = current_knobs();
+    return nt_ahead(d, nt_select(d, ga_num_cus(), k), ga_num_cus(), k);
 }
 
 extern "C" int ga_gemm_form(const ga_gemm_desc* d, char* buf, size_t n) {
@@ -1972,7 +2078,9 @@
     }
     if (sel.form == TN_TN2) return launch_tn2(d, sel, s);
     dim3 grid(cdiv(d->N, 128) * cdiv(d->K, 128) * d->split_m, 1, d->batch), block(kThreads);
-    if (d->dtype == GA_BF16)
+    if (tn_ahead(d, sel, ga_num_cus(), k) > 1)
+        hipLaunchKernelGGL((gemm_tn_kernel<bf16_t, kAheadDepth>), grid, block, 65536, s, *d);
+    else if (d->dtype == GA_BF16)
         hipLaunchKernelGGL(gemm_tn_kernel<bf16_t>, grid, block, 65536, s, *d);
     else
         hipLaunchKernelGGL(gemm_tn_kernel<float>, grid, block, 65536, s, *d);
@@ -1985,6 +2093,12 @@
     return GA_OK;
 }
 
+extern "C" int ga_wgrad_ahead(const ga_wgrad_desc* d) {
+    if (const int rc = tn_validate(d)) return rc;
+    const Knobs k = current_knobs();
+    return tn_ahead(d, tn_select(d, ga_num_cus(), k), ga_num_cus(), k);
+}
+
 extern "C" size_t ga_wgrad_workspace(const ga_wgrad_desc* d) {
     if (!d || d->M <= 0 || d->N <= 0 || d->K <= 0 || d->batch < 1) return 0;
     return tn_select(d, ga_num_cus(), current_knobs()).ws_bytes;
diff --git a/imagenet-models_amd/csrc/gemm_select.h b/imagenet-models_amd/csrc/gemm_select.h
--- a/imagenet-models_amd/csrc/gemm_select.h
+++ b/imagenet-models_amd/csrc/gemm_select.h
@@ -22,6 +22,7 @@
         NT_DMA2_MINK = 256, NT_T256 = -1;
     int TN2 = 1, TN2_PATCH2 = 1, TN2_WGS = 0, TN2_PART_MIN = 65536;
     int CONV3_DIRECT = 1, CONV0_DIRECT = 1, STEM4_WGRAD_DIRECT = 1;
+    int STAGED_AHEAD = 1;
 };
 
 inline int ceil_div(long a, long b) { return (int)((a + b - 1) / b); }
@@ -211,6 +212,19 @@
                   d->a_kind != GA_A_PLAIN ? "+gather" : "", d->dtype == GA_F32 ? "+f32" : "");
 }
 
+#ifndef GA_STAGED_AHEAD_DEPTH
+#define GA_STAGED_AHEAD_DEPTH 2
+#endif
+constexpr int kAheadDepth = GA_STAGED_AHEAD_DEPTH;
+constexpr int kAheadMinSlabs = 4;
+inline int nt_ahead(const ga_gemm_desc* d, const NtSel& s, int num_cus, const Knobs& k) {
+    if (!k.STAGED_AHEAD || s.form != NT_STAGED || s.nwm != 2 || d->dtype != GA_BF16 || d->a_kind != GA_A_PLAIN) return 1;
+    if (!dma_offsets_fit(d)) return 1;
+    if (k.STAGED_AHEAD >= 2) return kAheadDepth;
+    const long wgs = (long)ceil_div(d->M, 128) * ceil_div(d->N, 32 * s.tnw) * d->batch;
+    return (ceil_div(d->K, 64) >= kAheadMinSlabs && wgs < num_cus) ? kAheadDepth : 1;
+}
+
 inline int tn_validate(const ga_wgrad_desc* d) {
     GA_SEL_REQUIRE(d && d->Y && d->X && d->dW, "ga_wgrad: null operand");
     GA_SEL_REQUIRE(d->M > 0 && d->N > 0 && d->K > 0 && d->batch >= 1 && d->split_m >= 1, "ga_wgrad: bad shape");
@@ -295,6 +309,15 @@
     else snprintf(buf, n, "tn2%s:split%d:%s", d->x_kind == GA_A_PATCH2 ? "p" : "", s.split, s.partials ? "partials" : "atomics");
 }
 
+inline int tn_ahead(const ga_wgrad_desc* d, const TnSel& s, int num_cus, const Knobs& k) {
+    if (!k.STAGED_AHEAD || s.form != TN_TN || d->dtype != GA_BF16 || d->x_kind != GA_A_PLAIN) return 1;
+    if ((long)d->M * d->ldy >= (1L << 30) || (long)d->M * d->ldx >= (1L << 30)) return 1;
+    if (k.STAGED_AHEAD >= 2) return kAheadDepth;
+    const int slabs = ceil_div(ceil_div(d->M, 64), d->split_m);
+    const long wgs = (long)ceil_div(d->N, 128) * ceil_div(d->K, 128) * d->split_m * d->batch;
+    return (slabs >= kAheadMinSlabs && 2 * wgs <= num_cus) ? kAheadDepth : 1;
+}
+
 #undef GA_SEL_REQUIRE
 
 }
diff --git a/include/gaext.h b/include/gaext.h
--- a/include/gaext.h
+++ b/include/gaext.h
@@ -99,6 +99,9 @@
 
 int ga_gemm_form(const ga_gemm_desc* d, char* buf, size_t n);
 int ga_wgrad_form(const ga_wgrad_desc* d, char* buf, size_t n);
+
+int ga_gemm_ahead(const ga_gemm_desc* d);
+int ga_wgrad_ahead(const ga_wgrad_desc* d);
 
 typedef struct {
     const float* w;
```

Result: no change. 11130 images/sec (median of 3 runs) (+0.7%).
